# CityU-AIM-Group/HTD

Measured on AMD Instinct MI355X. Metric: images/sec (1333x800) HTD-R50 train step, higher is better.
Workload: dtype f32; 1 GPU; HTD ResNet-50 FPN fp32 train step fwd+bwd+SGD, batch 4/GPU @ 1333x800 (padded 1344x800), random-init weights, 2000 RPN proposals/img, 512 RoIs/img/stage; global_batch=4, parallelism=dp1, stage2_positives=158, proposals=random-init RPN (few positives: the regression branch is nearly idle)

## Files before the change

### htd_amd/csrc/conv_wgrad.hip

```cpp
#include <algorithm>

#include "common.h"

namespace {

using f32x16 = __attribute__((ext_vector_type(16))) float;

__device__ __forceinline__ float4 keep4(bool ok, float4 v)
{
    return make_float4(ok ? v.x : 0.f, ok ? v.y : 0.f, ok ? v.z : 0.f, ok ? v.w : 0.f);
}

struct WgradParams {
    const float *x, *gy;
    float *out;
    float *bias_out;
    int B, H, W, Ci, Co, kh, kw, stride, pad, dil, Ho, Wo;
    int64_t K;
    int Ntot;
    int mt, nt, splits;
    int64_t slices_per_split;
    const float *amax_x, *amax_g;
};

constexpr int BKW = 32;

enum : int {
    PIX_POINTWISE = 0,
    PIX_WIDE = 1,
    PIX_GENERAL = 2
};

template <int WGM, int WGN, int TM, int TN, int PIX, bool COVEC>
__global__ __launch_bounds__(256, 3) void conv_wgrad_kernel(WgradParams p)
{
    static_assert(WGM * WGN == 4, "4 waves per block");
    constexpr int BM = WGM * TM * 32, BN = WGN * TN * 32;
    constexpr int SA = BM + 4, SB = BN + 4;
    constexpr int VA = BM / 4, VB = BN / 4;
    constexpr int PA = (BKW * VA + 255) / 256, PB = (BKW * VB + 255) / 256;
    __shared__ __attribute__((aligned(16))) float lds[1][BKW * (SA + SB)];

    int tile, split;
    {
        const int tiles = p.mt * p.nt, L = blockIdx.x;
        if (p.splits % 8 == 0) {
            const int xcd = L % 8, idx = L / 8;
            tile = idx % tiles;
            split = (idx / tiles) * 8 + xcd;
        } else {
            tile = L % tiles;
            split = L / tiles;
        }
    }
    const int tile_m = tile % p.mt, tile_n = tile / p.mt;
    const int m0 = tile_m * BM, n0 = tile_n * BN;
    const int tid = threadIdx.x, lane = tid & 63, wave = tid >> 6;
    const int wm = wave / WGN, wn = wave % WGN;

    int a_col[PA], a_row[PA];
    bool a_cok[PA];
#pragma unroll
    for (int i = 0; i < PA; ++i) {
        const int v = tid + i * 256;
        a_row[i] = v / VA;
        a_col[i] = (v % VA) * 4;
        a_cok[i] = (v < BKW * VA) && (m0 + a_col[i] < p.Co);
    }
    int b_col[PB], b_row[PB], b_dy[PB], b_dx[PB], b_ci[PB];
    bool b_cok[PB];
#pragma unroll
    for (int i = 0; i < PB; ++i) {
        const int v = tid + i * 256;
        b_row[i] = v / VB;
        b_col[i] = (v % VB) * 4;
        const int n = n0 + b_col[i];
        b_cok[i] = (v < BKW * VB) && (n < p.Ntot);
        const int tap = b_cok[i] ? n / p.Ci : 0;
        b_ci[i] = b_cok[i] ? n - tap * p.Ci : 0;
        b_dy[i] = (tap / p.kw) * p.dil - p.pad;
        b_dx[i] = (tap % p.kw) * p.dil - p.pad;
    }

    const int64_t total_slices = (p.K + BKW - 1) / BKW;
    const int64_t s_begin = (int64_t)split * p.slices_per_split;
    const int64_t s_end = min(total_slices, s_begin + p.slices_per_split);

    unsigned a_k[PA];
#pragma unroll
    for (int i = 0; i < PA; ++i) a_k[i] = (unsigned)(s_begin * BKW) + a_row[i];
    unsigned b_k[PB];
    int b_b[PB], b_ho[PB], b_wo[PB];
    auto decode = [&](int i) {
        const unsigned kk = b_k[i] < (unsigned)p.K ? b_k[i] : 0u;
        b_wo[i] = (int)(kk % (unsigned)p.Wo);
        const unsigned t = kk / (unsigned)p.Wo;
        b_ho[i] = (int)(t % (unsigned)p.Ho);
        b_b[i] = (int)(t / (unsigned)p.Ho);
    };
#pragma unroll
    for (int i = 0; i < PB; ++i) {
        b_k[i] = (unsigned)(s_begin * BKW) + b_row[i];
        if constexpr (PIX != PIX_POINTWISE) decode(i);
    }

    float4 ra[PA], rb[PB];
    unsigned ra_ok = 0u, rb_ok = 0u;
    auto load_slice = [&]() {
#pragma unroll
        for (int i = 0; i < PA; ++i) {
            const bool ok = a_cok[i] && a_k[i] < (unsigned)p.K;
            const unsigned off = ok ? a_k[i] * (unsigned)p.Co + m0 + a_col[i] : 0u;
            if constexpr (COVEC) {
                ra[i] = *reinterpret_cast<const float4 *>(p.gy + off);
            } else {
                const int rem = ok ? p.Co - (m0 + a_col[i]) : 1;
                const float *g = p.gy + off;
                ra[i] = make_float4(g[0], g[rem > 1 ? 1 : 0], g[rem > 2 ? 2 : 0], g[rem > 3 ? 3 : 0]);
                ra[i].y = rem > 1 ? ra[i].y : 0.f;
                ra[i].z = rem > 2 ? ra[i].z : 0.f;
                ra[i].w = rem > 3 ? ra[i].w : 0.f;
            }
            ra_ok = ok ? (ra_ok | (1u << i)) : (ra_ok & ~(1u << i));
            a_k[i] += BKW;
        }
#pragma unroll
        for (int i = 0; i < PB; ++i) {
            bool ok = b_cok[i] && b_k[i] < (unsigned)p.K;
            unsigned off;
            if constexpr (PIX == PIX_POINTWISE) {
                off = b_k[i] * (unsigned)p.Ci + b_ci[i];
            } else {
                const int hi = b_ho[i] * p.stride + b_dy[i], wi = b_wo[i] * p.stride + b_dx[i];
                ok = ok && (unsigned)hi < (unsigned)p.H && (unsigned)wi < (unsigned)p.W;
                off = (((unsigned)b_b[i] * p.H + hi) * p.W + wi) * (unsigned)p.Ci + b_ci[i];
            }
            rb[i] = *reinterpret_cast<const float4 *>(p.x + (ok ? off : 0u));
            rb_ok = ok ? (rb_ok | (1u << i)) : (rb_ok & ~(1u << i));
            b_k[i] += BKW;
            if constexpr (PIX == PIX_WIDE) {
                const int wo = b_wo[i] + BKW;
                const bool c1 = wo >= p.Wo;
                b_wo[i] = c1 ? wo - p.Wo : wo;
                const int ho = b_ho[i] + (c1 ? 1 : 0);
                const bool c2 = ho == p.Ho;
                b_ho[i] = c2 ? 0 : ho;
                b_b[i] += c2 ? 1 : 0;
            } else if constexpr (PIX == PIX_GENERAL) {
                decode(i);
            }
        }
    };
    const bool do_bias = p.bias_out != nullptr && tile_n == 0;
    float4 bsum = make_float4(0.f, 0.f, 0.f, 0.f);
    auto store_slice = [&](int buf) {
        float *la = lds[buf], *lb = lds[buf] + BKW * SA;
#pragma unroll
        for (int i = 0; i < PA; ++i)
            if ((BKW * VA) % 256 == 0 || tid + i * 256 < BKW * VA) {
                const float4 v = keep4((ra_ok >> i) & 1u, ra[i]);
                *reinterpret_cast<float4 *>(la + a_row[i] * SA + a_col[i]) = v;
                if (do_bias) { bsum.x += v.x; bsum.y += v.y; bsum.z += v.z; bsum.w += v.w; }
            }
#pragma unroll
        for (int i = 0; i < PB; ++i)
            if ((BKW * VB) % 256 == 0 || tid + i * 256 < BKW * VB) *reinterpret_cast<float4 *>(lb + b_row[i] * SB + b_col[i]) = keep4((rb_ok >> i) & 1u, rb[i]);
    };

    f32x16 acc[TM][TN];
#pragma unroll
    for (int i = 0; i < TM; ++i)
#pragma unroll
        for (int j = 0; j < TN; ++j)
#pragma unroll
            for (int r = 0; r < 16; ++r) acc[i][j][r] = 0.f;
// ... 647 lines not shown
        if (v < 0) { x = Wv - 1; y = -1; }
    };
#pragma unroll
    for (int i = 0; i < 4; ++i) decode(s_begin * XH_KS + a_row0 + 8 * i, ax[i], ay[i], ab[i]);
#pragma unroll
    for (int i = 0; i < 3; ++i) decode(s_begin * XH_KS - 1 + b_row0 + 16 * i, bx[i], by[i], bb[i]);
    auto advance = [&](int &x, int &y, int &b) {
        if constexpr (WIDE) {
            x += XH_KS;
            const bool c1 = x >= Wv;
            x = c1 ? x - Wv : x;
            y += c1 ? 1 : 0;
            const bool c2 = y >= p.H;
            y = c2 ? y - p.H : y;
            b += c2 ? 1 : 0;
        } else {
            const int64_t v = ((int64_t)b * p.H + y) * Wv + x + XH_KS;
            x = (int)(v % Wv);
            const int64_t t = v / Wv;
            y = (int)(t % p.H);
            b = (int)(t / p.H);
        }
    };

    float4 ra[4], rb[3];
    unsigned ok_a = 0u, ok_b = 0u;
    auto load_slice = [&]() {
#pragma unroll
        for (int i = 0; i < 4; ++i) {
            const bool ok = a_cok && ab[i] < p.B && ax[i] < p.W;
            const unsigned off = (((unsigned)ab[i] * p.H + ay[i]) * (unsigned)p.W + ax[i]) * (unsigned)p.Co + m0 + a_col;
            ra[i] = *reinterpret_cast<const float4 *>(p.gy + (ok ? off : 0u));
            ok_a = ok ? (ok_a | (1u << i)) : (ok_a & ~(1u << i));
            advance(ax[i], ay[i], ab[i]);
        }
#pragma unroll
        for (int i = 0; i < 3; ++i) {
            const int yy = by[i] + dy;
            const bool ok = b_cok && (i < 2 || b_row0 < 2) && bb[i] < p.B && bx[i] < p.W && (unsigned)yy < (unsigned)p.H;
            const unsigned off = (((unsigned)bb[i] * p.H + yy) * (unsigned)p.W + bx[i]) * (unsigned)p.Ci + ci0 + b_col;
            rb[i] = *reinterpret_cast<const float4 *>(p.x + (ok ? off : 0u));
            ok_b = ok ? (ok_b | (1u << i)) : (ok_b & ~(1u << i));
            advance(bx[i], by[i], bb[i]);
        }
    };
    const bool do_bias = p.bias_out != nullptr && tile_nc == 0 && ky == 1;
    float4 bsum = make_float4(0.f, 0.f, 0.f, 0.f);
    auto put = [&](unsigned short *img, int plane, int rowpitch, int row, int col, float4 v) {
        unsigned h0, m0_, l0, h1, m1, l1;
        split3x2w(v.x, v.y, h0, m0_, l0);
        split3x2w(v.z, v.w, h1, m1, l1);
        unsigned short *d = img + row * rowpitch + col;
        *reinterpret_cast<uint2 *>(d) = make_uint2(h0, h1);
        *reinterpret_cast<uint2 *>(d + plane) = make_uint2(m0_, m1);
        *reinterpret_cast<uint2 *>(d + 2 * plane) = make_uint2(l0, l1);
    };
    auto store_slice = [&]() {
#pragma unroll
        for (int i = 0; i < 4; ++i) {
            const float4 v = keep4((ok_a >> i) & 1u, ra[i]);
            put(la, XH_PLANE_A, X3_ROW, a_row0 + 8 * i, a_col, v);
            if (do_bias) { bsum.x += v.x; bsum.y += v.y; bsum.z += v.z; bsum.w += v.w; }
        }
#pragma unroll
        for (int i = 0; i < 3; ++i)
            if (i < 2 || b_row0 < 2) put(lb, XH_PLANE_B, XH_ROWB, b_row0 + 16 * i, b_col, keep4((ok_b >> i) & 1u, rb[i]));
    };

    f32x16 acc[3][2];
#pragma unroll
    for (int t = 0; t < 3; ++t)
#pragma unroll
        for (int i = 0; i < 2; ++i)
#pragma unroll
            for (int r = 0; r < 16; ++r) acc[t][i][r] = 0.f;

    if (s_begin < s_end) {
        load_slice();
        store_slice();
    }
    __syncthreads();
    for (int64_t s = s_begin; s < s_end; ++s) {
        if (s + 1 < s_end) load_slice();
#pragma unroll
        for (int kk = 0; kk < XH_KS / 16; ++kk) {
            bf16x8w fa[2][3];
#pragma unroll
            for (int i = 0; i < 2; ++i)
#pragma unroll
                for (int q = 0; q < 3; ++q) fa[i][q] = tr_frag_row<X3_ROW>(la + q * XH_PLANE_A, kk * 16, wm * 64 + i * 32, lane);
#pragma unroll
            for (int t = 0; t < 3; ++t) {
                bf16x8w fb[3];
#pragma unroll
                for (int q = 0; q < 3; ++q) fb[q] = tr_frag_row<XH_ROWB>(lb + q * XH_PLANE_B, kk * 16 + t, wn * 32, lane);
#pragma unroll
                for (int i = 0; i < 2; ++i) {
                    acc[t][i] = __builtin_amdgcn_mfma_f32_32x32x16_bf16(fa[i][2], fb[0], acc[t][i], 0, 0, 0);
                    acc[t][i] = __builtin_amdgcn_mfma_f32_32x32x16_bf16(fa[i][0], fb[2], acc[t][i], 0, 0, 0);
                    acc[t][i] = __builtin_amdgcn_mfma_f32_32x32x16_bf16(fa[i][1], fb[1], acc[t][i], 0, 0, 0);
                    acc[t][i] = __builtin_amdgcn_mfma_f32_32x32x16_bf16(fa[i][1], fb[0], acc[t][i], 0, 0, 0);
                    acc[t][i] = __builtin_amdgcn_mfma_f32_32x32x16_bf16(fa[i][0], fb[1], acc[t][i], 0, 0, 0);
                    acc[t][i] = __builtin_amdgcn_mfma_f32_32x32x16_bf16(fa[i][0], fb[0], acc[t][i], 0, 0, 0);
                }
            }
        }
        if (s + 1 < s_end) {
            __syncthreads();
            store_slice();
        }
        __syncthreads();
    }

    if (do_bias) {
        float4 *red = reinterpret_cast<float4 *>(lds);
        red[tid] = bsum;
        __syncthreads();
        if (tid < 32) {
            float4 t = red[tid];
            for (int r = 1; r < 8; ++r) {
                const float4 v = red[r * 32 + tid];
                t.x += v.x; t.y += v.y; t.z += v.z; t.w += v.w;
            }
            float *dst = p.bias_out + (int64_t)split * p.Co;
            const int m = m0 + tid * 4;
            if (m < p.Co) dst[m] = t.x;
            if (m + 1 < p.Co) dst[m + 1] = t.y;
            if (m + 2 < p.Co) dst[m + 2] = t.z;
            if (m + 3 < p.Co) dst[m + 3] = t.w;
        }
    }
    float *out = p.out + (int64_t)split * p.Co * p.Ntot;
    const int fcol = lane & 31, fhalf = lane >> 5;
    const int ci = ci0 + wn * 32 + fcol;
    if (ci < p.Ci) {
#pragma unroll
        for (int t = 0; t < 3; ++t) {
            const int n = (ky * 3 + t) * p.Ci + ci;
#pragma unroll
            for (int i = 0; i < 2; ++i)
#pragma unroll
                for (int r = 0; r < 16; ++r) {
                    const int m = m0 + wm * 64 + i * 32 + (r & 3) + 8 * (r >> 2) + 4 * fhalf;
                    if (m < p.Co) out[(int64_t)m * p.Ntot + n] = acc[t][i][r];
                }
        }
    }
}

constexpr int XHD_KS = 16;
constexpr int XHD_RUN = XHD_KS + 2;
constexpr int XHD_PLANE_A = XHD_KS * X3_ROW, XHD_PLANE_B = XHD_RUN * XH_ROWB;
constexpr int XHD_BUF = 3 * XHD_PLANE_A + 3 * XHD_PLANE_B;
template <int TM, bool H2 = false>
__global__ __launch_bounds__(256, 2) void conv_wgrad_x3hd_kernel(WgradParams p)
{
    float sg = 1.f, sx = 1.f, sg_inv = 1.f, sx_inv = 1.f;
    if constexpr (H2) {
        const H2ScaleW a = h2w_scale(p.amax_g), b = h2w_scale(p.amax_x);
        sg = a.s; sg_inv = a.inv; sx = b.s; sx_inv = b.inv;
    }
    constexpr int BM = 2 * TM * 32, BNC = 64;
    constexpr int VA = BM / 4, RA = 256 / VA, PA = XHD_KS / RA;
    __shared__ __attribute__((aligned(16))) unsigned short lds[2 * XHD_BUF];
    const int ntc = (p.Ci + BNC - 1) / BNC;
    const int tiles = p.mt * ntc * 3;
    int tile, split;
    {
        const int L = blockIdx.x;
        if (p.splits % 8 == 0) {
            const int xcd = L % 8, idx = L / 8;
            tile = idx % tiles;
            split = (idx / tiles) * 8 + xcd;
        } else {
            tile = L % tiles;
            split = L / tiles;
        }
    }
    const int tile_m = tile % p.mt, rest = tile / p.mt;
    const int tile_nc = rest % ntc, ky = rest / ntc;
    const int m0 = tile_m * BM, ci0 = tile_nc * BNC, dy = ky - 1;
    const int tid = threadIdx.x, lane = tid & 63, wave = tid >> 6;
    const int wm = wave >> 1, wn = wave & 1;

    const int Wv = p.W + 1;
    const int64_t V = (int64_t)p.B * p.H * Wv;
    const int64_t v_begin = (int64_t)split * p.slices_per_split * XH_KS;
    const int64_t v_end = min((V + XH_KS - 1) / XH_KS * XH_KS, v_begin + p.slices_per_split * XH_KS);
    const int n_slices = v_begin < v_end ? (int)((v_end - v_begin) / XHD_KS) : 0;

    constexpr unsigned OOB = 0x80000000u;
    const int64_t px_end = min((int64_t)p.B * p.H * p.W, v_end - v_end / Wv);
    const __amdgpu_buffer_rsrc_t gy_desc = __builtin_amdgcn_make_buffer_rsrc(
        const_cast<float *>(p.gy), 0, (int)((unsigned)px_end * (unsigned)p.Co * 4u), 0x00020000);
    const __amdgpu_buffer_rsrc_t x_desc = __builtin_amdgcn_make_buffer_rsrc(
        const_cast<float *>(p.x), 0, (int)((unsigned)p.B * p.H * p.W * p.Ci * 4u), 0x00020000);

    const int a_col = (tid % VA) * 4, a_row0 = tid / VA;
    const int b_col = (tid & 15) * 4, b_row0 = tid >> 4;
    const bool a_cok = m0 + a_col < p.Co, b_cok = ci0 + b_col < p.Ci;
    const bool ragged = tid < 32;
    auto decode = [&](int64_t v, int &x, int &y, int64_t &real) {
        const int64_t vv = v < 0 ? 0 : v;
        x = (int)(vv % Wv);
        const int64_t t = vv / Wv;
        y = (int)(t % p.H);
        real = vv - t;
        if (v < 0) { x = Wv - 1; y = -1; real = 0; }
    };
    int ax[PA], bx[2], by[2];
    unsigned a_off[PA], b_off[2];
    const unsigned a_px = a_cok ? (unsigned)p.Co * 4u : 0u, b_px = b_cok ? (unsigned)p.Ci * 4u : 0u;
#pragma unroll
    for (int i = 0; i < PA; ++i) {
        int y;
        int64_t real;
        decode(v_begin + a_row0 + RA * i, ax[i], y, real);
        a_off[i] = a_cok ? (unsigned)(real * p.Co + m0 + a_col) * 4u : OOB;
    }
#pragma unroll
    for (int i = 0; i < 2; ++i) {
        int64_t real;
        decode(v_begin - 1 + b_row0 + 16 * i, bx[i], by[i], real);
        b_off[i] = b_cok && (i == 0 || ragged) ? (unsigned)((real + (int64_t)dy * p.W) * p.Ci + ci0 + b_col) * 4u : OOB;
    }
    const unsigned b_px1 = ragged ? b_px : 0u;
    const int adv_rows = XHD_KS / Wv, adv_x = XHD_KS - adv_rows * Wv;

    using u32x4w = __attribute__((ext_vector_type(4))) unsigned;
    auto load16 = [&](__amdgpu_buffer_rsrc_t d, unsigned off) {
        union { u32x4w u; float4 f; } c;
        c.u = __builtin_amdgcn_raw_buffer_load_b128(d, (int)off, 0, 0);
        return c.f;
    };
    float4 ra[2][PA], rb[2][2];
    auto load_slice = [&](float4 (&qa)[PA], float4 (&qb)[2]) {
#pragma unroll
        for (int i = 0; i < PA; ++i) {
            qa[i] = load16(gy_desc, ax[i] < p.W ? a_off[i] : OOB);
            ax[i] += adv_x;
            const bool c1 = ax[i] >= Wv;
            ax[i] -= c1 ? Wv : 0;
            a_off[i] += XHD_KS * a_px - (unsigned)(adv_rows + (c1 ? 1 : 0)) * a_px;
        }
#pragma unroll
        for (int i = 0; i < 2; ++i) {
            const unsigned px = i == 0 ? b_px : b_px1;
            qb[i] = load16(x_desc, bx[i] < p.W && (unsigned)(by[i] + dy) < (unsigned)p.H ? b_off[i] : OOB);
            bx[i] += adv_x;
            const bool c1 = bx[i] >= Wv;
            bx[i] -= c1 ? Wv : 0;
            const int rows = adv_rows + (c1 ? 1 : 0);
            by[i] += rows;
            by[i] -= by[i] >= p.H ? p.H : 0;
            b_off[i] += XHD_KS * px - (unsigned)rows * px;
        }
    };
    const bool do_bias = p.bias_out != nullptr && tile_nc == 0 && ky == 1;
    float4 bsum = make_float4(0.f, 0.f, 0.f, 0.f);
    auto put = [&](unsigned short *d, int plane, float4 v, float sc) {
        if constexpr (H2) {
            unsigned h0, l0, h1, l1;
            split2w(v.x * sc, v.y * sc, h0, l0);
            split2w(v.z * sc, v.w * sc, h1, l1);
            *reinterpret_cast<uint2 *>(d) = make_uint2(h0, h1);
            *reinterpret_cast<uint2 *>(d + plane) = make_uint2(l0, l1);
        } else {
            unsigned h0, m0_, l0, h1, m1, l1;
            split3x2w(v.x, v.y, h0, m0_, l0);
            split3x2w(v.z, v.w, h1, m1, l1);
            *reinterpret_cast<uint2 *>(d) = make_uint2(h0, h1);
            *reinterpret_cast<uint2 *>(d + plane) = make_uint2(m0_, m1);
            *reinterpret_cast<uint2 *>(d + 2 * plane) = make_uint2(l0, l1);
        }
    };
    const int a_lds0 = a_row0 * X3_ROW + a_col, a_lds1 = (a_row0 + RA) * X3_ROW + a_col;
    const int b_lds0 = 3 * XHD_PLANE_A + b_row0 * XH_ROWB + b_col, b_lds1 = 3 * XHD_PLANE_A + (16 + b_row0) * XH_ROWB + b_col;

    f32x16 acc[3][TM];
#pragma unroll
    for (int t = 0; t < 3; ++t)
#pragma unroll
        for (int i = 0; i < TM; ++i)
#pragma unroll
            for (int r = 0; r < 16; ++r) acc[t][i][r] = 0.f;

    auto half = [&](const unsigned short *rd, unsigned short *wr, float4 (&qa)[PA], float4 (&qb)[2]) {
        constexpr int NPL = H2 ? 2 : 3;
        bf16x8w fa[TM][3], fb[3][3];
#pragma unroll
        for (int i = 0; i < TM; ++i)
#pragma unroll
            for (int q = 0; q < NPL; ++q) fa[i][q] = tr_frag_row<X3_ROW>(rd + q * XHD_PLANE_A, 0, wm * TM * 32 + i * 32, lane);
#pragma unroll
        for (int t = 0; t < 3; ++t)
#pragma unroll
            for (int q = 0; q < NPL; ++q) fb[t][q] = tr_frag_row<XH_ROWB>(rd + 3 * XHD_PLANE_A + q * XHD_PLANE_B, t, wn * 32, lane);
        __builtin_amdgcn_sched_barrier(0);
        constexpr int QA[6] = {H2 ? 1 : 2, 0, H2 ? 0 : 1, 1, 0, 0}, QB[6] = {0, H2 ? 1 : 2, H2 ? 0 : 1, 0, 1, 0};
        unsigned h[2], m[2], l[2];
        constexpr int NC = 2 * (PA + 1), NM = (H2 ? 9 : 18) * TM;
#pragma unroll
        for (int c = 0; c < NC; ++c) {
            const int u = c >> 1;
            const float4 v = u < PA ? qa[u < PA ? u : 0] : qb[0];
            const float sc = u < PA ? sg : sx;
            if ((c & 1) == 0) {
                if constexpr (H2) split2w(v.x * sc, v.y * sc, h[0], l[0]);
                else split3x2w(v.x, v.y, h[0], m[0], l[0]);
            } else {
                if constexpr (H2) split2w(v.z * sc, v.w * sc, h[1], l[1]);
                else split3x2w(v.z, v.w, h[1], m[1], l[1]);
                unsigned short *d = wr + (u >= PA ? b_lds0 : u == 0 ? a_lds0 : a_lds1);
                const int plane = u < PA ? XHD_PLANE_A : XHD_PLANE_B;
                *reinterpret_cast<uint2 *>(d) = make_uint2(h[0], h[1]);
                if constexpr (H2) {
                    *reinterpret_cast<uint2 *>(d + plane) = make_uint2(l[0], l[1]);
                } else {
                    *reinterpret_cast<uint2 *>(d + plane) = make_uint2(m[0], m[1]);
                    *reinterpret_cast<uint2 *>(d + 2 * plane) = make_uint2(l[0], l[1]);
                }
                if (u < PA) { bsum.x += v.x; bsum.y += v.y; bsum.z += v.z; bsum.w += v.w; }
            }
#pragma unroll
            for (int e = c * NM / NC; e < (c + 1) * NM / NC; ++e) {
                const int q = e / (3 * TM), t = (e % (3 * TM)) / TM, i = e % TM;
                acc[t][i] = mfma_x3w<H2>(fa[i][QA[q]], fb[t][QB[q]], acc[t][i]);
            }
            __builtin_amdgcn_sched_barrier(0);
        }
        if (__builtin_amdgcn_readfirstlane(wave) == 0) {
            if (ragged) put(wr + b_lds1, XHD_PLANE_B, qb[1], sx);
        }
        load_slice(qa, qb);
        __syncthreads();
    };
    auto store_slice = [&](unsigned short *wr, const float4 (&qa)[PA], const float4 (&qb)[2]) {
        put(wr + a_lds0, XHD_PLANE_A, qa[0], sg);
        if constexpr (PA > 1) put(wr + a_lds1, XHD_PLANE_A, qa[PA - 1], sg);
#pragma unroll
        for (int i = 0; i < PA; ++i) { bsum.x += qa[i].x; bsum.y += qa[i].y; bsum.z += qa[i].z; bsum.w += qa[i].w; }
        put(wr + b_lds0, XHD_PLANE_B, qb[0], sx);
        if (ragged) put(wr + b_lds1, XHD_PLANE_B, qb[1], sx);
    };

    unsigned short *buf0 = lds, *buf1 = lds + XHD_BUF;
    load_slice(ra[0], rb[0]);
    load_slice(ra[1], rb[1]);
    store_slice(buf0, ra[0], rb[0]);
    load_slice(ra[0], rb[0]);
    __syncthreads();
    for (int s = 0; s < n_slices; s += 2) {
        half(buf0, buf1, ra[1], rb[1]);
        half(buf1, buf0, ra[0], rb[0]);
    }

    if (do_bias) {
        float4 *red = reinterpret_cast<float4 *>(lds);
        __syncthreads();
        red[tid] = bsum;
        __syncthreads();
        if (tid < VA) {
            float4 t = red[tid];
            for (int r = 1; r < RA; ++r) {
                const float4 v = red[r * VA + tid];
                t.x += v.x; t.y += v.y; t.z += v.z; t.w += v.w;
            }
            float *dst = p.bias_out + (int64_t)split * p.Co;
            const int m = m0 + tid * 4;
            if (m < p.Co) dst[m] = t.x;
            if (m + 1 < p.Co) dst[m + 1] = t.y;
            if (m + 2 < p.Co) dst[m + 2] = t.z;
            if (m + 3 < p.Co) dst[m + 3] = t.w;
        }
    }
    float *out = p.out + (int64_t)split * p.Co * p.Ntot;
    const int fcol = lane & 31, fhalf = lane >> 5;
    const int ci = ci0 + wn * 32 + fcol;
    if (ci < p.Ci) {
#pragma unroll
        for (int t = 0; t < 3; ++t) {
            const int n = (ky * 3 + t) * p.Ci + ci;
#pragma unroll
            for (int i = 0; i < TM; ++i)
#pragma unroll
                for (int r = 0; r < 16; ++r) {
                    const int m = m0 + wm * TM * 32 + i * 32 + (r & 3) + 8 * (r >> 2) + 4 * fhalf;
                    if (m < p.Co) out[(int64_t)m * p.Ntot + n] = H2 ? acc[t][i][r] * sg_inv * sx_inv : acc[t][i][r];
                }
        }
    }
}

__global__ __launch_bounds__(256) void splitk_reduce_kernel(const float *__restrict__ ws, float *__restrict__ out,
                                                            int64_t n, int splits, const float *__restrict__ ws2 = nullptr,
                                                            float *__restrict__ out2 = nullptr, int n2 = 0, int acc = 0)
{
    const int extra = out2 ? (n2 + 255) / 256 : 0;
    if ((int)blockIdx.x >= (int)gridDim.x - extra) {
        const int i = ((int)blockIdx.x - ((int)gridDim.x - extra)) * 256 + threadIdx.x;
        if (i < n2) {
            float s = acc ? out2[i] : 0.f;
            int k = 0;
            for (; k + 3 < splits; k += 4) {
                const float a = ws2[(int64_t)k * n2 + i], b = ws2[(int64_t)(k + 1) * n2 + i];
                const float c = ws2[(int64_t)(k + 2) * n2 + i], d = ws2[(int64_t)(k + 3) * n2 + i];
                s += a; s += b; s += c; s += d;
            }
            for (; k < splits; ++k) s += ws2[(int64_t)k * n2 + i];
            out2[i] = s;
        }
        return;
    }
    const unsigned main_blocks = gridDim.x - extra;
    const int64_t n4 = (n & 3) == 0 ? (n >> 2) : 0;
    for (int64_t i = (int64_t)blockIdx.x * blockDim.x + threadIdx.x; i < n4; i += (int64_t)main_blocks * blockDim.x) {
        float4 s = acc ? *reinterpret_cast<const float4 *>(out + i * 4) : make_float4(0.f, 0.f, 0.f, 0.f);
        int k = 0;
        for (; k + 3 < splits; k += 4) {
            float4 v[4];
#pragma unroll
            for (int u = 0; u < 4; ++u) v[u] = *reinterpret_cast<const float4 *>(ws + (int64_t)(k + u) * n + i * 4);
#pragma unroll
            for (int u = 0; u < 4; ++u) { s.x += v[u].x; s.y += v[u].y; s.z += v[u].z; s.w += v[u].w; }
        }
        for (; k < splits; ++k) {
            const float4 v = *reinterpret_cast<const float4 *>(ws + (int64_t)k * n + i * 4);
            s.x += v.x; s.y += v.y; s.z += v.z; s.w += v.w;
        }
        *reinterpret_cast<float4 *>(out + i * 4) = s;
    }
    if (blockIdx.x == 0)
        for (int64_t i = n4 * 4 + threadIdx.x; i < n; i += blockDim.x) {
            float s = acc ? out[i] : 0.f;
            for (int k = 0; k < splits; ++k) s += ws[(int64_t)k * n + i];
            out[i] = s;
        }
}

__global__ __launch_bounds__(256) void reduce_rows_kernel(const float *__restrict__ ws, float *__restrict__ out, int n,
                                                          int rows)
{
    __shared__ float red[16][17];
    const int col = threadIdx.x & 15, grp = threadIdx.x >> 4;
    const int c = blockIdx.x * 16 + col;
    float s = 0.f;
    if (c < n)
        for (int k = grp; k < rows; k += 16) s += ws[(int64_t)k * n + c];
    red[grp][col] = s;
    __syncthreads();
    if (grp == 0 && c < n) {
        float t = red[0][col];
#pragma unroll
        for (int g = 1; g < 16; ++g) t += red[g][col];
        out[c] = t;
    }
}

using htd::mag_bits;
using htd::wave_mag_out;

__global__ __launch_bounds__(256) void colsum_mask_kernel(const float *__restrict__ g, const float *__restrict__ y,
                                                          float *__restrict__ gm, float *__restrict__ partial,
                                                          int64_t rows, int C, int64_t rows_per_block, float *__restrict__ amax_out)
{
    const int c = blockIdx.y * 256 + threadIdx.x;
    const int64_t r0 = (int64_t)blockIdx.x * rows_per_block, r1 = min(rows, r0 + rows_per_block);
    float s = 0.f;
    unsigned mx = 0u;
    if (c < C)
        for (int64_t r = r0; r < r1; ++r) {
            float v = g[r * C + c];
            if (y) {
                v = y[r * C + c] > 0.f ? v : 0.f;
                gm[r * C + c] = v;
            }
            mx = max(mx, mag_bits(v));
            s += v;
        }
    if (amax_out) wave_mag_out(mx, amax_out);
    if (partial && c < C) partial[(int64_t)blockIdx.x * C + c] = s;
}

__global__ __launch_bounds__(256) void colsum_mask_vec_kernel(const float *__restrict__ g, const float *__restrict__ y,
                                                              float *__restrict__ gm, float *__restrict__ partial,
                                                              int64_t rows, int C, int64_t rows_per_block,
                                                              float *__restrict__ amax_out)
{
    __shared__ float4 red[256];
    unsigned mx = 0u;
    const int C4 = C >> 2;
    const int cbase = blockIdx.y * 256;
    const int cw = min(256, C4 - cbase);
    const int R = 256 / cw;
    const int c4 = threadIdx.x % cw, rsub = threadIdx.x / cw;
    const int64_t r0 = (int64_t)blockIdx.x * rows_per_block, r1 = min(rows, r0 + rows_per_block);
    float4 s = make_float4(0.f, 0.f, 0.f, 0.f);
    if (rsub < R) {
        int64_t r = r0 + rsub;
        for (; r + 3 * (int64_t)R < r1; r += 4 * (int64_t)R) {
            float4 v[4], yv[4];
#pragma unroll
            for (int u = 0; u < 4; ++u) {
                const int64_t o = (r + u * (int64_t)R) * C + (int64_t)(cbase + c4) * 4;
                v[u] = *reinterpret_cast<const float4 *>(g + o);
                if (y) yv[u] = *reinterpret_cast<const float4 *>(y + o);
            }
#pragma unroll
            for (int u = 0; u < 4; ++u) {
                if (y) {
                    const int64_t o = (r + u * (int64_t)R) * C + (int64_t)(cbase + c4) * 4;
                    v[u].x = yv[u].x > 0.f ? v[u].x : 0.f; v[u].y = yv[u].y > 0.f ? v[u].y : 0.f;
                    v[u].z = yv[u].z > 0.f ? v[u].z : 0.f; v[u].w = yv[u].w > 0.f ? v[u].w : 0.f;
                    *reinterpret_cast<float4 *>(gm + o) = v[u];
                }
                mx = htd::mag_bits4(mx, v[u]);
                s.x += v[u].x; s.y += v[u].y; s.z += v[u].z; s.w += v[u].w;
            }
        }
        for (; r < r1; r += R) {
            const int64_t o = r * C + (int64_t)(cbase + c4) * 4;
            float4 v = *reinterpret_cast<const float4 *>(g + o);
            if (y) {
                const float4 yv = *reinterpret_cast<const float4 *>(y + o);
                v.x = yv.x > 0.f ? v.x : 0.f; v.y = yv.y > 0.f ? v.y : 0.f;
                v.z = yv.z > 0.f ? v.z : 0.f; v.w = yv.w > 0.f ? v.w : 0.f;
                *reinterpret_cast<float4 *>(gm + o) = v;
            }
            mx = htd::mag_bits4(mx, v);
            s.x += v.x; s.y += v.y; s.z += v.z; s.w += v.w;
        }
    }
    if (amax_out) wave_mag_out(mx, amax_out);
    if (!partial) return;
    red[threadIdx.x] = s;
    __syncthreads();
    if (rsub == 0) {
        for (int k = 1; k < R; ++k) {
            const float4 t = red[k * cw + c4];
            s.x += t.x; s.y += t.y; s.z += t.z; s.w += t.w;
        }
        *reinterpret_cast<float4 *>(partial + (int64_t)blockIdx.x * C + (int64_t)(cbase + c4) * 4) = s;
    }
}

struct Cfg { int splits; int mt, nt; int bm, bn; };

template <int WGM, int WGN, int TM, int TN>
void launch_wgrad(int pix, bool covec, dim3 grid, hipStream_t s, const WgradParams &p)
{
#define HTD_WGRAD_CASE(PIX, CV)                                                                                   \
    if (pix == PIX && covec == CV) {                                                                               \
        hipLaunchKernelGGL((conv_wgrad_kernel<WGM, WGN, TM, TN, PIX, CV>), grid, dim3(256), 0, s, p);             \
        return;                                                                                                    \
    }
    HTD_WGRAD_CASE(PIX_POINTWISE, true) HTD_WGRAD_CASE(PIX_WIDE, true) HTD_WGRAD_CASE(PIX_GENERAL, true)
    HTD_WGRAD_CASE(PIX_POINTWISE, false) HTD_WGRAD_CASE(PIX_WIDE, false) HTD_WGRAD_CASE(PIX_GENERAL, false)
#undef HTD_WGRAD_CASE
}

Cfg choose(int Co, int Ntot, int64_t K)
{
    Cfg c;
    c.bm = Co <= 32 ? 32 : 128;
    c.bn = 128;
    c.mt = (int)htd::ceil_div(Co, c.bm);
    c.nt = (int)htd::ceil_div(Ntot, c.bn);
    const int64_t slices = htd::ceil_div(K, BKW);
    static const int units = getenv("HTD_WGRAD_UNITS") ? atoi(getenv("HTD_WGRAD_UNITS")) : 1536;
    int64_t want = htd::ceil_div(units, (int64_t)c.mt * c.nt);
    const int64_t tiles = (int64_t)c.mt * c.nt;
    int64_t cap = std::max<int64_t>(1, slices / 20);
    if (tiles * cap < 256)
        cap = std::max(cap, std::min<int64_t>(htd::ceil_div(256, tiles), std::max<int64_t>(1, slices / 5)));
    want = std::min<int64_t>(want, cap);
    c.splits = (int)std::max<int64_t>(1, std::min<int64_t>(want, 192));
    if (c.splits >= 6) c.splits = (c.splits + 7) / 8 * 8;
    static const int forced = getenv("HTD_WGRAD_SPLITS") ? atoi(getenv("HTD_WGRAD_SPLITS")) : 0;
    if (forced > 0) c.splits = (int)std::min<int64_t>(forced, slices);
    return c;
}

static const bool g_wgrad_x3h_off = getenv("HTD_WGRAD_X3H") != nullptr && atoi(getenv("HTD_WGRAD_X3H")) == 0;
bool x3h_takes(int Ci, int Co, int kh, int kw, int stride, int pad, int dil)
{
    return !g_wgrad_x3h_off && kh == 3 && kw == 3 && stride == 1 && pad == 1 && dil == 1 && Co >= 64 && (Co & 3) == 0 &&
           Ci >= 32 && (Ci & 3) == 0;
}
int x3h_splits(int B, int H, int W, int Ci, int Co)
{
    const int64_t tiles = htd::ceil_div(Co, 128) * htd::ceil_div(Ci, 64) * 3;
    const int64_t slices = htd::ceil_div((int64_t)B * H * (W + 1), XH_KS);
    static const int target = getenv("HTD_WGRAD_X3H_UNITS") ? atoi(getenv("HTD_WGRAD_X3H_UNITS")) : 768;
    int64_t want = htd::ceil_div(target, tiles);
    int64_t cap = std::max<int64_t>(1, slices / 8);
    if (tiles * cap < 256) cap = std::max(cap, std::min<int64_t>(htd::ceil_div(256, tiles), std::max<int64_t>(1, slices / 4)));
    want = std::min<int64_t>(want, cap);
    int splits = (int)std::max<int64_t>(1, std::min<int64_t>(want, 128));
    if (splits >= 6) splits = (splits + 7) / 8 * 8;
    static const int forced = getenv("HTD_WGRAD_X3H_SPLITS") ? atoi(getenv("HTD_WGRAD_X3H_SPLITS")) : 0;
    if (forced > 0) splits = (int)std::min<int64_t>(forced, std::max<int64_t>(1, slices / 2));
    return splits;
}

}

int g_wgrad_math = -1;

extern "C" int64_t htd_conv2d_wgrad_workspace_bytes(int B, int H, int W, int Ci, int Co, int kh, int kw, int stride,
                                                    int pad, int dil)
{
    const int Ho = (H + 2 * pad - (dil * (kh - 1) + 1)) / stride + 1;
    const int Wo = (W + 2 * pad - (dil * (kw - 1) + 1)) / stride + 1;
    const Cfg c = choose(Co, kh * kw * Ci, (int64_t)B * Ho * Wo);
    int splits = c.splits;
    if (x3h_takes(Ci, Co, kh, kw, stride, pad, dil)) splits = std::max(splits, x3h_splits(B, H, W, Ci, Co));
    return (int64_t)splits * Co * (kh * kw * Ci + 1) * 4 + 256;
}

static int bwd_weight_impl(const float *x, const float *gy, float *gw, float *gbias, int B, int H, int W, int Ci, int Co, int kh,
                           int kw, int stride, int pad, int dil, void *workspace, void *stream, int accumulate,
                           const float *amax_x = nullptr, const float *amax_g = nullptr)
{
    HTD_REQUIRE(B > 0 && H > 0 && W > 0 && Ci > 0 && Co > 0 && kh > 0 && kw > 0 && stride > 0 && dil > 0 && pad >= 0,
                "conv2d_bwd_weight: bad sizes");
    HTD_REQUIRE(Ci % 4 == 0, "conv2d_bwd_weight: Ci=%d must be a multiple of 4", Ci);
    HTD_REQUIRE(x && gy && gw && workspace, "conv2d_bwd_weight: null pointer");
    WgradParams p{};
    p.x = x; p.gy = gy;
    p.amax_x = amax_x; p.amax_g = amax_g;
    const bool h2 = amax_x != nullptr && amax_g != nullptr;
    p.B = B; p.H = H; p.W = W; p.Ci = Ci; p.Co = Co; p.kh = kh; p.kw = kw; p.stride = stride; p.pad = pad; p.dil = dil;
    p.Ho = (H + 2 * pad - (dil * (kh - 1) + 1)) / stride + 1;
    p.Wo = (W + 2 * pad - (dil * (kw - 1) + 1)) / stride + 1;
    HTD_REQUIRE(p.Ho > 0 && p.Wo > 0, "conv2d_bwd_weight: empty output");
    p.K = (int64_t)B * p.Ho * p.Wo;
    HTD_REQUIRE((int64_t)B * H * W * Ci < (1ll << 31) && p.K * Co < (1ll << 31),
                "conv2d_bwd_weight: operand larger than 2^31 elements (32-bit element offsets)");
    p.Ntot = kh * kw * Ci;
    static const int math_env0 = getenv("HTD_CONV_MATH") ? atoi(getenv("HTD_CONV_MATH")) : 1;
    if ((g_wgrad_math < 0 ? math_env0 : g_wgrad_math) == 1 && x3h_takes(Ci, Co, kh, kw, stride, pad, dil)) {
        p.mt = (int)htd::ceil_div(Co, 128);
        p.nt = (int)htd::ceil_div(Ci, 64);
        p.splits = x3h_splits(B, H, W, Ci, Co);
        const int64_t slices = htd::ceil_div((int64_t)B * H * (W + 1), XH_KS);
        p.slices_per_split = htd::ceil_div(slices, p.splits);
        p.splits = (int)htd::ceil_div(slices, p.slices_per_split);
        const bool direct = p.splits == 1 && !accumulate;
        p.out = direct ? gw : (float *)workspace;
        float *bias_part = (float *)workspace + (int64_t)p.splits * Co * p.Ntot;
        p.bias_out = !gbias ? nullptr : (direct ? gbias : bias_part);
        hipStream_t s = (hipStream_t)stream;
        const dim3 grid((unsigned)(p.mt * p.nt * 3 * p.splits));
        static const bool x3hd_on = !(getenv("HTD_WGRAD_X3D") && atoi(getenv("HTD_WGRAD_X3D")) == 0);
        if (x3hd_on && XHD_KS / (W + 1) + 1 <= H && (int64_t)B * H * W * Ci * 4 < (1ll << 31) &&
            (int64_t)B * H * W * Co * 4 < (1ll << 31))
        {
            static const bool tile64 = !(getenv("HTD_WGRAD_TILE64") && atoi(getenv("HTD_WGRAD_TILE64")) == 0);
            if (tile64 && Co <= 64) {
                p.mt = (int)htd::ceil_div(Co, 64);
                const dim3 g64((unsigned)(p.mt * p.nt * 3 * p.splits));
                if (h2) hipLaunchKernelGGL((conv_wgrad_x3hd_kernel<1, true>), g64, dim3(256), 0, s, p);
                else hipLaunchKernelGGL((conv_wgrad_x3hd_kernel<1, false>), g64, dim3(256), 0, s, p);
            } else if (h2) {
                hipLaunchKernelGGL((conv_wgrad_x3hd_kernel<2, true>), grid, dim3(256), 0, s, p);
            } else {
                hipLaunchKernelGGL((conv_wgrad_x3hd_kernel<2, false>), grid, dim3(256), 0, s, p);
            }
        }
        else {
            HTD_REQUIRE(!h2, "conv2d_bwd_weight_h2: this 3x3 layer is not taken by the H2 kernels (htd_conv2d_bwd_weight_h2_supported)");
            if (W + 1 >= XH_KS) hipLaunchKernelGGL(conv_wgrad_x3h_kernel<true>, grid, dim3(256), 0, s, p);
            else hipLaunchKernelGGL(conv_wgrad_x3h_kernel<false>, grid, dim3(256), 0, s, p);
        }
        if (!direct) {
            const int64_t n = (int64_t)Co * p.Ntot;
            const unsigned blocks = (unsigned)std::min<int64_t>(htd::ceil_div(n, 256), 2048);
            const unsigned extra = gbias ? (unsigned)htd::ceil_div(Co, 256) : 0u;
            hipLaunchKernelGGL(splitk_reduce_kernel, dim3(blocks + extra), dim3(256), 0, s, (const float *)workspace, gw, n,
                               p.splits, (const float *)(gbias ? bias_part : nullptr), gbias, Co, accumulate);
        }
        return htd::check_launch("conv2d_bwd_weight");
    }
    const Cfg c = choose(Co, p.Ntot, p.K);
    p.mt = c.mt; p.nt = c.nt; p.splits = c.splits;
    p.slices_per_split = htd::ceil_div(htd::ceil_div(p.K, BKW), c.splits);
    const bool direct = c.splits == 1 && !accumulate;
    p.out = direct ? gw : (float *)workspace;
    float *bias_partial = (float *)workspace + (int64_t)c.splits * Co * p.Ntot;
    p.bias_out = !gbias ? nullptr : (direct ? gbias : bias_partial);
    hipStream_t s = (hipStream_t)stream;
    p.slices_per_split = htd::ceil_div(htd::ceil_div(p.K, BKW), c.splits);
    dim3 grid((unsigned)(c.mt * c.nt * c.splits));
    const int pix = (kh == 1 && kw == 1 && stride == 1 && pad == 0) ? PIX_POINTWISE : (p.Wo >= BKW ? PIX_WIDE : PIX_GENERAL);
    const bool covec = (Co & 3) == 0;
    static const int math_env = getenv("HTD_CONV_MATH") ? atoi(getenv("HTD_CONV_MATH")) : 1;
    const bool x3 = (g_wgrad_math < 0 ? math_env : g_wgrad_math) == 1 && c.bm == 128 && covec && (Ci & 3) == 0;
    if (x3) {
        static const bool x3d_on = !(getenv("HTD_WGRAD_X3D") && atoi(getenv("HTD_WGRAD_X3D")) == 0);
        const bool x3d = x3d_on && (int64_t)B * H * W * Ci * 4 < (1ll << 31) && p.K * Co * 4 < (1ll << 31);
        if (x3d) {
            static const bool tile64 = !(getenv("HTD_WGRAD_TILE64") && atoi(getenv("HTD_WGRAD_TILE64")) == 0);
            const bool m64 = tile64 && Co <= 64 && pix != PIX_GENERAL, n64 = tile64 && !m64 && p.Ntot <= 64 && pix == PIX_POINTWISE;
            p.mt = (int)htd::ceil_div(Co, m64 ? 64 : 128);
            p.nt = (int)htd::ceil_div(p.Ntot, n64 ? 64 : 128);
            const dim3 gd = c.splits % 8 == 0 ? dim3((unsigned)(p.mt * p.nt * c.splits))
                                              : dim3((unsigned)(8 * htd::ceil_div(p.nt * c.splits, 8) * p.mt));
            if (h2) {
                if (m64 && pix == PIX_POINTWISE) hipLaunchKernelGGL((conv_wgrad_x3d_kernel<PIX_POINTWISE, 1, 2, true>), gd, dim3(256), 0, s, p);
                else if (m64) hipLaunchKernelGGL((conv_wgrad_x3d_kernel<PIX_WIDE, 1, 2, true>), gd, dim3(256), 0, s, p);
                else if (n64) hipLaunchKernelGGL((conv_wgrad_x3d_kernel<PIX_POINTWISE, 2, 1, true>), gd, dim3(256), 0, s, p);
                else if (pix == PIX_POINTWISE) hipLaunchKernelGGL((conv_wgrad_x3d_kernel<PIX_POINTWISE, 2, 2, true>), gd, dim3(256), 0, s, p);
                else if (pix == PIX_WIDE) hipLaunchKernelGGL((conv_wgrad_x3d_kernel<PIX_WIDE, 2, 2, true>), gd, dim3(256), 0, s, p);
                else hipLaunchKernelGGL((conv_wgrad_x3d_kernel<PIX_GENERAL, 2, 2, true>), gd, dim3(256), 0, s, p);
            }
            else if (m64 && pix == PIX_POINTWISE) hipLaunchKernelGGL((conv_wgrad_x3d_kernel<PIX_POINTWISE, 1, 2>), gd, dim3(256), 0, s, p);
            else if (m64) hipLaunchKernelGGL((conv_wgrad_x3d_kernel<PIX_WIDE, 1, 2>), gd, dim3(256), 0, s, p);
            else if (n64) hipLaunchKernelGGL((conv_wgrad_x3d_kernel<PIX_POINTWISE, 2, 1>), gd, dim3(256), 0, s, p);
            else if (pix == PIX_POINTWISE) hipLaunchKernelGGL((conv_wgrad_x3d_kernel<PIX_POINTWISE, 2, 2>), gd, dim3(256), 0, s, p);
            else if (pix == PIX_WIDE) hipLaunchKernelGGL((conv_wgrad_x3d_kernel<PIX_WIDE, 2, 2>), gd, dim3(256), 0, s, p);
            else hipLaunchKernelGGL((conv_wgrad_x3d_kernel<PIX_GENERAL, 2, 2>), gd, dim3(256), 0, s, p);
        } else if (h2) {
            HTD_REQUIRE(false, "conv2d_bwd_weight_h2: operands too large for the H2 kernels (htd_conv2d_bwd_weight_h2_supported)");
        } else if (pix == PIX_POINTWISE) hipLaunchKernelGGL(conv_wgrad_x3_kernel<PIX_POINTWISE>, grid, dim3(256), 0, s, p);
        else if (pix == PIX_WIDE) hipLaunchKernelGGL(conv_wgrad_x3_kernel<PIX_WIDE>, grid, dim3(256), 0, s, p);
        else hipLaunchKernelGGL(conv_wgrad_x3_kernel<PIX_GENERAL>, grid, dim3(256), 0, s, p);
    } else if (h2) {
        HTD_REQUIRE(false, "conv2d_bwd_weight_h2: layer not taken by the H2 kernels (htd_conv2d_bwd_weight_h2_supported)");
    } else if (c.bm == 32)
        launch_wgrad<1, 4, 1, 1>(pix, covec, grid, s, p);
    else
        launch_wgrad<2, 2, 2, 2>(pix, covec, grid, s, p);
    if (!direct) {
        const int64_t n = (int64_t)Co * p.Ntot;
        const unsigned blocks = (unsigned)std::min<int64_t>(htd::ceil_div(n, 256), 2048);
        const unsigned extra = gbias ? (unsigned)htd::ceil_div(Co, 256) : 0u;
        hipLaunchKernelGGL(splitk_reduce_kernel, dim3(blocks + extra), dim3(256), 0, s, (const float *)workspace, gw, n,
                           c.splits, (const float *)(gbias ? bias_partial : nullptr), gbias, Co, accumulate);
    }
    return htd::check_launch("conv2d_bwd_weight");
}

extern "C" int htd_conv2d_bwd_weight(const float *x, const float *gy, float *gw, float *gbias, int B, int H, int W,
                                     int Ci, int Co, int kh, int kw, int stride, int pad, int dil, void *workspace,
                                     void *stream)
{
    return bwd_weight_impl(x, gy, gw, gbias, B, H, W, Ci, Co, kh, kw, stride, pad, dil, workspace, stream, 0);
}

extern "C" int htd_conv2d_bwd_weight_acc(const float *x, const float *gy, float *gw, float *gbias, int B, int H, int W,
                                         int Ci, int Co, int kh, int kw, int stride, int pad, int dil, void *workspace,
                                         void *stream)
{
    return bwd_weight_impl(x, gy, gw, gbias, B, H, W, Ci, Co, kh, kw, stride, pad, dil, workspace, stream, 1);
}

extern "C" int htd_conv2d_bwd_weight_h2_supported(int B, int H, int W, int Ci, int Co, int kh, int kw, int stride, int pad, int dil)
{
    static const int math_env = getenv("HTD_CONV_MATH") ? atoi(getenv("HTD_CONV_MATH")) : 1;
    if (htd_conv2d_set_h2(-1) != 1 || (g_wgrad_math < 0 ? math_env : g_wgrad_math) != 1) return 0;
    if (B <= 0 || H <= 0 || W <= 0 || Ci <= 0 || Co <= 0 || (Ci & 3) != 0 || stride <= 0 || dil <= 0 || pad < 0) return 0;
    const int Ho = (H + 2 * pad - (dil * (kh - 1) + 1)) / stride + 1, Wo = (W + 2 * pad - (dil * (kw - 1) + 1)) / stride + 1;
    if (Ho <= 0 || Wo <= 0) return 0;
    const int64_t K = (int64_t)B * Ho * Wo;
    static const bool d_on = !(getenv("HTD_WGRAD_X3D") && atoi(getenv("HTD_WGRAD_X3D")) == 0);
    if (!d_on || (int64_t)B * H * W * Ci * 4 >= (1ll << 31) || K * Co * 4 >= (1ll << 31)) return 0;
    if (x3h_takes(Ci, Co, kh, kw, stride, pad, dil)) return XHD_KS / (W + 1) + 1 <= H ? 1 : 0;
    const Cfg c = choose(Co, kh * kw * Ci, K);
    return (c.bm == 128 && (Co & 3) == 0) ? 1 : 0;
}

extern "C" int htd_conv2d_bwd_weight_h2(const float *x, const float *gy, const float *amax_x, const float *amax_g, float *gw,
                                        float *gbias, int B, int H, int W, int Ci, int Co, int kh, int kw, int stride, int pad,
                                        int dil, int accumulate, void *workspace, void *stream)
{
    HTD_REQUIRE(amax_x && amax_g, "conv2d_bwd_weight_h2: null maximum");
    HTD_REQUIRE(htd_conv2d_bwd_weight_h2_supported(B, H, W, Ci, Co, kh, kw, stride, pad, dil) == 1,
                "conv2d_bwd_weight_h2: layer not taken by the H2 kernels");
    return bwd_weight_impl(x, gy, gw, gbias, B, H, W, Ci, Co, kh, kw, stride, pad, dil, workspace, stream, accumulate ? 1 : 0, amax_x,
                           amax_g);
}

static int bias_grad_relu_mask_impl(const float *g, const float *y, float *gm, float *gbias, int64_t rows, int C, void *workspace,
                                    float *amax_out, void *stream)
{
    HTD_REQUIRE(rows >= 0 && C > 0, "bias_grad: bad sizes");
    HTD_REQUIRE(g && (gbias || y) && (!gbias || workspace) && (!y || gm), "bias_grad: null pointer");
    hipStream_t s = (hipStream_t)stream;
    const int nb = (int)std::max<int64_t>(1, std::min<int64_t>(1024, htd::ceil_div(rows, 8)));
    const int64_t rpb = htd::ceil_div(std::max<int64_t>(rows, 1), nb);
    float *partial = gbias ? (float *)workspace : nullptr;
    if ((C & 3) == 0 && (((uintptr_t)g | (uintptr_t)y | (uintptr_t)gm | (uintptr_t)partial) & 15) == 0)
        hipLaunchKernelGGL(colsum_mask_vec_kernel, dim3(nb, (unsigned)htd::ceil_div(C / 4, 256)), dim3(256), 0, s, g, y,
                           gm, partial, rows, C, rpb, amax_out);
    else
        hipLaunchKernelGGL(colsum_mask_kernel, dim3(nb, (unsigned)htd::ceil_div(C, 256)), dim3(256), 0, s, g, y, gm,
                           partial, rows, C, rpb, amax_out);
    if (gbias)
        hipLaunchKernelGGL(reduce_rows_kernel, dim3((unsigned)htd::ceil_div(C, 16)), dim3(256), 0, s,
                           (const float *)partial, gbias, C, nb);
    return htd::check_launch("bias_grad");
}

extern "C" int htd_bias_grad_relu_mask(const float *g, const float *y, float *gm, float *gbias, int64_t rows, int C,
                                       void *workspace, void *stream)
{
    return bias_grad_relu_mask_impl(g, y, gm, gbias, rows, C, workspace, nullptr, stream);
}

extern "C" int htd_bias_grad_relu_mask_amax(const float *g, const float *y, float *gm, float *gbias, int64_t rows, int C,
                                            void *workspace, float *amax_out, void *stream)
{
    HTD_REQUIRE(amax_out, "bias_grad: null maximum");
    return bias_grad_relu_mask_impl(g, y, gm, gbias, rows, C, workspace, amax_out, stream);
}
```

### htd_amd/csrc/conv_x3.hip

```cpp
#include <algorithm>
#include <mutex>
#include <type_traits>
#include <unordered_map>

#include <stdlib.h>

#include "common.h"

namespace {

using f32x16 = __attribute__((ext_vector_type(16))) float;
using bf16x8 = __attribute__((ext_vector_type(8))) __bf16;
using bf16x2 = __attribute__((ext_vector_type(2))) __bf16;
using f32x2 = __attribute__((ext_vector_type(2))) float;
using f32x4 = __attribute__((ext_vector_type(4))) float;

using f16x8 = __attribute__((ext_vector_type(8))) _Float16;
using f16x2 = __attribute__((ext_vector_type(2))) _Float16;

constexpr int XK = 16;
constexpr int NCH = 6;

struct H2Scale { float s, inv; };
__device__ __forceinline__ H2Scale h2_scale(const float *amax)
{
    const unsigned E = (__float_as_uint(*amax) >> 23) & 0xffu;
    int e = E == 0u ? 126 : (E == 255u ? 0 : 141 - (int)E);
    e = e > 126 ? 126 : e;
    return H2Scale{__uint_as_float((unsigned)(127 + e) << 23), __uint_as_float((unsigned)(127 - e) << 23)};
}
__device__ __forceinline__ void split2hx2(float a, float b, unsigned &h, unsigned &l)
{
    union { f16x2 v; unsigned u; } c;
    c.v = __builtin_convertvector(f32x2{a, b}, f16x2);
    h = c.u;
    const f32x2 back = __builtin_convertvector(c.v, f32x2);
    c.v = __builtin_convertvector(f32x2{a - back[0], b - back[1]}, f16x2);
    l = c.u;
}

__device__ __forceinline__ void split3x2(float a, float b, unsigned &h, unsigned &m, unsigned &l)
{
    union { bf16x2 v; unsigned u; } c;
    c.v = __builtin_convertvector(f32x2{a, b}, bf16x2);
    h = c.u;
    const float ra = a - __uint_as_float(h << 16), rb = b - __uint_as_float(h & 0xffff0000u);
    c.v = __builtin_convertvector(f32x2{ra, rb}, bf16x2);
    m = c.u;
    c.v = __builtin_convertvector(f32x2{ra - __uint_as_float(m << 16), rb - __uint_as_float(m & 0xffff0000u)}, bf16x2);
    l = c.u;
}

#ifndef HTD_X3P_EARLY
#define HTD_X3P_EARLY 1
#endif
#ifndef HTD_X3H_NB
#define HTD_X3H_NB 2
#endif
#ifndef HTD_X3H_FRAG_FIRST
#define HTD_X3H_FRAG_FIRST 1
#endif
#ifndef HTD_X3H_OCC4
#define HTD_X3H_OCC4 0
#endif

template <int N>
__device__ __forceinline__ void wait_vm()
{
    asm volatile("s_waitcnt vmcnt(%0)" ::"n"(N) : "memory");
}
__device__ __forceinline__ void landed(f32x4 &a) { asm volatile("" : "+v"(a)::"memory"); }

__device__ __forceinline__ void lds_dma16(const void *src, unsigned lds_dst)
{
    unsigned keep;
    asm volatile("s_mov_b32 %0, m0\n\ts_mov_b32 m0, %2\n\ts_nop 0\n\tglobal_load_lds_dwordx4 %1, off\n\ts_mov_b32 m0, %0"
                 : "=&s"(keep)
                 : "v"(src), "s"(lds_dst)
                 : "memory");
}

using u32x2 = __attribute__((ext_vector_type(2))) unsigned;
template <int OFF>
__device__ __forceinline__ void lds_store8(unsigned addr, unsigned lo, unsigned hi)
{
    const u32x2 v = {lo, hi};
    asm volatile("ds_write_b64 %0, %1 offset:%2" ::"v"(addr), "v"(v), "n"(OFF) : "memory");
}

struct X3Params {
    const float *x;
    const uint4 *wp;
    const float *bias, *residual, *mask_src;
    float *y;
    int Hx, Wx;
    int Ho, Wo;
    int Ci, Co, Cop;
    int kh;
    int stride;
    int ntl;
    int tl_dy[9], tl_dx[9], tl_w[9];
    int o_step, o_h0, o_w0, oH, oW;
    int relu;
    int res_H, res_W;
    float res_sh, res_sw;
    int64_t M;
    int mt, nt;
    int ncs;
    int tiles_a, splits_a, sps_a, splits_b, sps_b;
    int64_t m_rem0;
    float *partial;
    const uint4 *xp;
    uint4 *yp;
    int64_t xp_rows, yp_rows;
    const float *amax, *wscale;
    float *amax_out;
};

__device__ __forceinline__ void block_absmax_out(float mx, float *out, float *red, unsigned seen)
{
    unsigned bits = (mx != mx) ? 0x7fc00000u : __float_as_uint(mx);
    for (int o = 32; o > 0; o >>= 1) bits = max(bits, (unsigned)__shfl_xor((int)bits, o));
    __syncthreads();
    if ((threadIdx.x & 63) == 0) reinterpret_cast<unsigned *>(red)[threadIdx.x >> 6] = bits;
    __syncthreads();
    if (threadIdx.x == 0) {
        const unsigned *r = reinterpret_cast<const unsigned *>(red);
        bits = max(max(r[0], r[1]), max(r[2], r[3]));
        if (bits > seen) __hip_atomic_fetch_max(reinterpret_cast<unsigned *>(out), bits, __ATOMIC_RELAXED, __HIP_MEMORY_SCOPE_AGENT);
    }
}
__device__ __forceinline__ void wave_absmax_out(float mx, float *out, unsigned seen)
{
    unsigned bits = (mx != mx) ? 0x7fc00000u : __float_as_uint(mx);
    for (int o = 32; o > 0; o >>= 1) bits = max(bits, (unsigned)__shfl_xor((int)bits, o));
    if ((threadIdx.x & 63) == 0 && bits > seen)
        __hip_atomic_fetch_max(reinterpret_cast<unsigned *>(out), bits, __ATOMIC_RELAXED, __HIP_MEMORY_SCOPE_AGENT);
}
__device__ __forceinline__ float absmax4(float mx, float4 v)
{
    const float m = fmaxf(fmaxf(fabsf(v.x), fabsf(v.y)), fmaxf(fabsf(v.z), fabsf(v.w)));
    const bool nan = (v.x != v.x) | (v.y != v.y) | (v.z != v.z) | (v.w != v.w);
    return nan ? __uint_as_float(0x7fc00000u) : ((mx != mx) ? mx : fmaxf(mx, m));
}

__device__ __forceinline__ void emit_planes4(uint4 *yp, int64_t rows, int64_t m, int n, float4 v)
{
    unsigned h0, m0, l0, h1, m1, l1;
    split3x2(v.x, v.y, h0, m0, l0);
    split3x2(v.z, v.w, h1, m1, l1);
    char *d = reinterpret_cast<char *>(yp + ((int64_t)(n >> 4) * NCH + ((n >> 3) & 1)) * rows + m) + ((n >> 2) & 1) * 8;
    *reinterpret_cast<uint2 *>(d) = make_uint2(h0, h1);
    *reinterpret_cast<uint2 *>(d + 2 * rows * 16) = make_uint2(m0, m1);
    *reinterpret_cast<uint2 *>(d + 4 * rows * 16) = make_uint2(l0, l1);
}

template <int BM, int KW>
struct Geo {
    static constexpr int RUN = BM + KW - 1;
    static constexpr int PITCH = ((RUN + 1 + 3) / 8) * 8 + 4;
    static constexpr int PASSES = (RUN + 63) / 64;
};

__device__ __forceinline__ int64_t x3_out_off(const X3Params &p, int64_t m, int n)
{
    if (p.o_step == 0) return m * p.Co + n;
    const unsigned mm = (unsigned)m, wo = mm % (unsigned)p.Wo, t = mm / (unsigned)p.Wo;
    const unsigned ho = t % (unsigned)p.Ho, b = t / (unsigned)p.Ho;
    return (((int64_t)b * p.oH + p.o_h0 + p.o_step * (int)ho) * p.oW + p.o_w0 + p.o_step * (int)wo) * p.Co + n;
}

template <int WGM, int WGN, int TM, int TN, bool MF16, typename Acc>
__device__ __forceinline__ void x3_epilogue(const X3Params &p, Acc &acc, uint4 *lds, int64_t m0, int n0, bool part, bool region_b,
                                            int split)
{
    constexpr int BN = WGN * TN * 32;
    constexpr int EPI_STRIDE = BN + 4, EPI_ROWS = WGM * 32;
    constexpr int RBLK = MF16 ? 16 : 32;
    constexpr int CB = TN * 32 / RBLK;
    const int tid = threadIdx.x, lane = tid & 63, wave = tid >> 6;
    const int wm = wave / WGN, wn = wave % WGN;
    const int frow = lane & 31, fhalf = lane >> 5;
    const int lrow = MF16 ? (lane & 15) : frow;
    const int kg = lane >> 4;
    float *le = reinterpret_cast<float *>(lds);
    const bool vec_ok = (p.Co & 3) == 0;
    constexpr int V = BN / 4, RPP = 256 / V;
    float omax = 0.f;
    const unsigned oseen = (p.amax_out != nullptr && !part) ? *reinterpret_cast<const volatile unsigned *>(p.amax_out) : 0u;
    const bool scaled = p.wscale != nullptr;
    float4 cscale = make_float4(1.f, 1.f, 1.f, 1.f);
    if (scaled) {
        const float ia = h2_scale(p.amax).inv;
        const float4 w4 = *reinterpret_cast<const float4 *>(p.wscale + n0 + (tid % V) * 4);
        cscale = make_float4(w4.x * ia, w4.y * ia, w4.z * ia, w4.w * ia);
    }
#pragma unroll
    for (int i = 0; i < TM; ++i) {
        if constexpr (MF16) {
#pragma unroll
            for (int ib = 0; ib < 2; ++ib)
#pragma unroll
                for (int j = 0; j < CB; ++j)
#pragma unroll
                    for (int r = 0; r < 4; ++r)
                        le[(wm * 32 + ib * 16 + 4 * kg + r) * EPI_STRIDE + wn * TN * 32 + j * 16 + lrow] = acc[2 * i + ib][j][r];
        } else {
#pragma unroll
            for (int j = 0; j < TN; ++j)
#pragma unroll
                for (int r = 0; r < 16; ++r) {
                    const int row = wm * 32 + (r & 3) + 8 * (r >> 2) + 4 * fhalf;
                    le[row * EPI_STRIDE + (wn * TN + j) * 32 + frow] = acc[i][j][r];
                }
        }
        __syncthreads();
        const int c4 = tid % V;
        const int n = n0 + c4 * 4;
        constexpr int NPASS = EPI_ROWS / RPP;
        if (vec_ok && !part && p.res_H == 0) {
            const bool col_ok = n < p.Co;
            float4 bv = make_float4(0.f, 0.f, 0.f, 0.f);
            if (p.bias != nullptr && col_ok) bv = *reinterpret_cast<const float4 *>(p.bias + n);
            constexpr int UB = NPASS < 4 ? NPASS : 4;
#pragma unroll
            for (int pass0 = 0; pass0 < NPASS; pass0 += UB) {
                float4 v[UB], rv[UB], mv[UB];
                int64_t o[UB];
                bool ok[UB];
#pragma unroll
                for (int u = 0; u < UB; ++u) {
                    const int row = tid / V + (pass0 + u) * RPP;
                    const int64_t m = m0 + ((row >> 5) * TM + i) * 32 + (row & 31);
                    ok[u] = m < p.M && col_ok;
                    o[u] = x3_out_off(p, ok[u] ? m : 0, n) & -(int64_t)ok[u];
                    v[u] = *reinterpret_cast<const float4 *>(le + row * EPI_STRIDE + c4 * 4);
                    if (scaled) { v[u].x *= cscale.x; v[u].y *= cscale.y; v[u].z *= cscale.z; v[u].w *= cscale.w; }
                }
                if (p.residual != nullptr) {
#pragma unroll
                    for (int u = 0; u < UB; ++u) rv[u] = *reinterpret_cast<const float4 *>(p.residual + o[u]);
                }
                if (p.mask_src != nullptr) {
#pragma unroll
                    for (int u = 0; u < UB; ++u) mv[u] = *reinterpret_cast<const float4 *>(p.mask_src + o[u]);
                }
#pragma unroll
                for (int u = 0; u < UB; ++u) { v[u].x += bv.x; v[u].y += bv.y; v[u].z += bv.z; v[u].w += bv.w; }
                if (p.residual != nullptr) {
#pragma unroll
                    for (int u = 0; u < UB; ++u) { v[u].x += rv[u].x; v[u].y += rv[u].y; v[u].z += rv[u].z; v[u].w += rv[u].w; }
                }
                if (p.relu) {
#pragma unroll
                    for (int u = 0; u < UB; ++u) {
                        v[u].x = fmaxf(v[u].x, 0.f); v[u].y = fmaxf(v[u].y, 0.f); v[u].z = fmaxf(v[u].z, 0.f); v[u].w = fmaxf(v[u].w, 0.f);
                    }
                }
                if (p.mask_src != nullptr) {
#pragma unroll
                    for (int u = 0; u < UB; ++u) {
                        v[u].x = mv[u].x > 0.f ? v[u].x : 0.f; v[u].y = mv[u].y > 0.f ? v[u].y : 0.f;
                        v[u].z = mv[u].z > 0.f ? v[u].z : 0.f; v[u].w = mv[u].w > 0.f ? v[u].w : 0.f;
                    }
                }
#pragma unroll
                for (int u = 0; u < UB; ++u)
                    if (ok[u]) {
                        *reinterpret_cast<float4 *>(p.y + o[u]) = v[u];
                        omax = absmax4(omax, v[u]);
                    }
                if (p.yp != nullptr) {
#pragma unroll
                    for (int u = 0; u < UB; ++u) {
                        const int row = tid / V + (pass0 + u) * RPP;
                        if (ok[u]) emit_planes4(p.yp, p.yp_rows, m0 + ((row >> 5) * TM + i) * 32 + (row & 31), n, v[u]);
                    }
                }
            }
            if (i + 1 < TM) __syncthreads();
            continue;
        }
#pragma unroll
        for (int pass = 0; pass < NPASS; ++pass) {
            const int row = tid / V + pass * RPP;
            const int64_t m = m0 + ((row >> 5) * TM + i) * 32 + (row & 31);
            if (m >= p.M || n >= p.Co) continue;
            float4 v = *reinterpret_cast<const float4 *>(le + row * EPI_STRIDE + c4 * 4);
            if (scaled) { v.x *= cscale.x; v.y *= cscale.y; v.z *= cscale.z; v.w *= cscale.w; }
            const int64_t o = x3_out_off(p, m, n);
            if (part) {
                float *dst = region_b ? p.partial + (p.splits_a > 1 ? (int64_t)p.splits_a * p.m_rem0 * p.Co : 0) +
                                            ((int64_t)split * (p.M - p.m_rem0) + (m - p.m_rem0)) * p.Co + n
                                      : p.partial + ((int64_t)split * p.m_rem0 + m) * p.Co + n;
                if (vec_ok) *reinterpret_cast<float4 *>(dst) = v;
                else {
                    dst[0] = v.x;
                    if (n + 1 < p.Co) dst[1] = v.y;
                    if (n + 2 < p.Co) dst[2] = v.z;
                    if (n + 3 < p.Co) dst[3] = v.w;
                }
                continue;
            }
            if (vec_ok) {
                if (p.bias) {
                    const float4 bv = *reinterpret_cast<const float4 *>(p.bias + n);
                    v.x += bv.x; v.y += bv.y; v.z += bv.z; v.w += bv.w;
                }
                if (p.residual) {
                    int64_t ro = o;
                    if (p.res_H > 0) {
                        const unsigned mm = (unsigned)m, wo = mm % (unsigned)p.Wo, t = mm / (unsigned)p.Wo;
                        const unsigned ho = t % (unsigned)p.Ho, b = t / (unsigned)p.Ho;
                        const int rh = min((int)floorf(ho * p.res_sh), p.res_H - 1);
                        const int rw = min((int)floorf(wo * p.res_sw), p.res_W - 1);
                        ro = (((int64_t)b * p.res_H + rh) * p.res_W + rw) * p.Co + n;
                    }
                    const float4 rv = *reinterpret_cast<const float4 *>(p.residual + ro);
                    v.x += rv.x; v.y += rv.y; v.z += rv.z; v.w += rv.w;
                }
                if (p.relu) { v.x = fmaxf(v.x, 0.f); v.y = fmaxf(v.y, 0.f); v.z = fmaxf(v.z, 0.f); v.w = fmaxf(v.w, 0.f); }
                if (p.mask_src) {
                    const float4 mv = *reinterpret_cast<const float4 *>(p.mask_src + o);
                    v.x = mv.x > 0.f ? v.x : 0.f; v.y = mv.y > 0.f ? v.y : 0.f;
                    v.z = mv.z > 0.f ? v.z : 0.f; v.w = mv.w > 0.f ? v.w : 0.f;
                }
                *reinterpret_cast<float4 *>(p.y + o) = v;
                omax = absmax4(omax, v);
                if (p.yp != nullptr) emit_planes4(p.yp, p.yp_rows, m, n, v);
            } else {
                auto put = [&](int e, float t) {
                    if (n + e >= p.Co) return;
                    t += p.bias ? p.bias[n + e] : 0.f;
                    if (p.residual) t += p.residual[o + e];
                    if (p.relu) t = fmaxf(t, 0.f);
                    if (p.mask_src) t = p.mask_src[o + e] > 0.f ? t : 0.f;
                    p.y[o + e] = t;
                    omax = absmax4(omax, make_float4(t, 0.f, 0.f, 0.f));
                };
                put(0, v.x); put(1, v.y); put(2, v.z); put(3, v.w);
            }
        }
        if (i + 1 < TM) __syncthreads();
    }
    if (p.amax_out != nullptr && !part) block_absmax_out(omax, p.amax_out, le, oseen);
}

template <int WGM, int WGN, int TM, int TN, int KW, int NB, bool H2 = false>
constexpr int x3p_occupancy()
{
    constexpr int BM = WGM * TM * 32, BN = WGN * TN * 32;
    constexpr int NCHL = H2 ? 4 : NCH;
    constexpr int main_bytes = (2 * NCHL * Geo<BM, KW>::PITCH + NB * NCHL * BN) * 16;
    constexpr int epi_bytes = WGM * 32 * (BN + 4) * 4;
    constexpr int by_lds = 163840 / (main_bytes > epi_bytes ? main_bytes : epi_bytes);
    constexpr int by_regs = TM * TN >= 4 ? (H2 && HTD_X3H_OCC4 ? 4 : 3) : 4;
    return by_lds < by_regs ? by_lds : by_regs;
}

template <int WGM, int WGN, int TM, int TN, int KW, bool MF16, int NB, bool H2 = false>
__global__ __launch_bounds__(256, (x3p_occupancy<WGM, WGN, TM, TN, KW, NB, H2>())) void conv_x3p_kernel(X3Params p)
{
    static_assert(!(H2 && MF16), "H2: 32x32x16 form only");
    constexpr int NCHL = H2 ? 4 : NCH;
    constexpr int BM = WGM * TM * 32, BN = WGN * TN * 32;
    using G = Geo<BM, KW>;
    constexpr int PADX = (KW - 1) / 2;
    constexpr int A_VEC = NCHL * G::PITCH;
    constexpr int B_VEC = NCHL * BN;
    constexpr int MAIN_VEC = 2 * A_VEC + NB * B_VEC;
    constexpr int EPI_STRIDE = BN + 4, EPI_ROWS = WGM * 32;
    constexpr int EPI_VEC = EPI_ROWS * EPI_STRIDE / 4;
    constexpr int LDS_VEC = MAIN_VEC > EPI_VEC ? MAIN_VEC : EPI_VEC;
    __shared__ uint4 lds[LDS_VEC];
    uint4 *const lA = lds, *const lB = lds + 2 * A_VEC;
    const unsigned lds_a0 = (unsigned)(size_t)(__attribute__((address_space(3))) void *)lA;

    int bid = blockIdx.x, split = 0, sps = 0;
    bool part = false;
    const bool region_b = bid >= p.tiles_a * p.splits_a;
    if (region_b) {
        const int r = bid - p.tiles_a * p.splits_a;
        bid = p.tiles_a + r / p.splits_b;
        split = r % p.splits_b;
        part = p.splits_b > 1;
        sps = p.sps_b;
    } else if (p.splits_a > 1) {
        split = bid % p.splits_a;
        bid = bid / p.splits_a;
        part = true;
        sps = p.sps_a;
    } else {
        const int q = p.tiles_a / 8, r = p.tiles_a % 8, xcd = bid % 8, idx = bid / 8;
        bid = (xcd < r ? xcd * (q + 1) : r * (q + 1) + (xcd - r) * q) + idx;
    }
    const int tile_m = bid / p.nt, tile_n = bid % p.nt;
    const int64_t m0 = (int64_t)tile_m * BM;
    const int n0 = tile_n * BN;

    const int tid = threadIdx.x, lane = tid & 63, wave = tid >> 6;
    const int wm = wave / WGN, wn = wave % WGN;
    const int frow = lane & 31, fhalf = lane >> 5;
    const int PADY = (p.kh - 1) / 2;

    const int vcol = tid & 3, vrow = tid >> 2;
    const int a_g0 = (int)m0 + vrow - PADX;
    unsigned a_off[KW > 1 ? 1 : G::PASSES];
    bool a_in[KW > 1 ? 1 : G::PASSES];
    unsigned a_tm[KW > 1 ? 1 : G::PASSES];
    if constexpr (KW > 1) {
        a_off[0] = (unsigned)a_g0 * (unsigned)p.Ci + vcol * 4;
        a_in[0] = true;
        a_tm[0] = 0u;
    } else {
#pragma unroll
        for (int i = 0; i < G::PASSES; ++i) {
            const int64_t m = m0 + vrow + 64 * i;
            a_in[i] = vrow + 64 * i < G::RUN && m < p.M;
            const unsigned mm = a_in[i] ? (unsigned)m : 0u;
            const unsigned wo = mm % (unsigned)p.Wo, t = mm / (unsigned)p.Wo;
            const unsigned ho = t % (unsigned)p.Ho, b = t / (unsigned)p.Ho;
            a_off[i] = ((b * (unsigned)p.Hx + ho * (unsigned)p.stride) * (unsigned)p.Wx + wo * (unsigned)p.stride) *
                           (unsigned)p.Ci + vcol * 4;
            unsigned tm = 0x1ffu;
            if (p.ntl > 0) {
                tm = 0u;
                const int hb = (int)(ho * (unsigned)p.stride), wb = (int)(wo * (unsigned)p.stride);
                for (int q = 0; q < p.ntl; ++q)
                    tm |= ((unsigned)(hb + p.tl_dy[q]) < (unsigned)p.Hx && (unsigned)(wb + p.tl_dx[q]) < (unsigned)p.Wx) ? (1u << q) : 0u;
            }
            a_tm[i] = tm;
        }
    }

    constexpr int RBLK = MF16 ? 16 : 32;
    constexpr int RB = TM * 32 / RBLK, CB = TN * 32 / RBLK;
    const int lrow = MF16 ? (lane & 15) : frow;
    const int kg = lane >> 4;
    unsigned vmask[RB];
    const int a_frag0 = (wm * TM * 32 + lrow) * 16;
#pragma unroll
    for (int i = 0; i < RB; ++i) {
        const int r = wm * TM * 32 + i * RBLK + lrow;
        vmask[i] = 0xffffffffu;
        if constexpr (KW > 1) {
            const int64_t m = m0 + r;
            const unsigned mm = m < p.M ? (unsigned)m : 0u;
            const int xx = (int)(mm % (unsigned)p.Wx), yy = (int)((mm / (unsigned)p.Wx) % (unsigned)p.Hx);
            unsigned v = 0u;
            for (int ky = 0; ky < p.kh; ++ky)
#pragma unroll
                for (int kx = 0; kx < KW; ++kx) {
                    const bool ok = m < p.M && (unsigned)(yy + ky - PADY) < (unsigned)p.Hx &&
                                    (unsigned)(xx + kx - PADX) < (unsigned)p.Wx;
                    v |= ok ? (1u << (ky * KW + kx)) : 0u;
                }
            vmask[i] = v;
        }
    }
    const int zero_frag = G::RUN * 16;
    const int a_c0 = MF16 ? kg * G::PITCH * 16 : fhalf * G::PITCH * 16;
    const int a_c1 = MF16 ? ((kg >> 1) * 4 + (kg & 1)) * G::PITCH * 16 : 0;
    const int b_row = (wn * TN * 32 + lrow) * 16;
    const int b_c0 = (MF16 ? kg * BN * 16 : fhalf * BN * 16) + b_row;
    const int b_c1 = MF16 ? ((1 - (kg >> 1)) * 2 + (kg & 1)) * BN * 16 + b_row : 0;
    const int b_c2 = MF16 ? (((kg >> 1) ? 0 : 4) + (kg & 1)) * BN * 16 + b_row : 0;

    const int total_steps = p.ncs * p.kh;
    const int s_begin = part ? split * sps : 0;
    const int s_end = part ? min(total_steps, s_begin + sps) : total_steps;

    if (tid < 2 * NCHL) lA[(tid / NCHL) * A_VEC + (tid % NCHL) * G::PITCH + G::RUN] = make_uint4(0u, 0u, 0u, 0u);

    constexpr int NP = G::PASSES;
    constexpr int NPT = KW > 1 ? 1 : NP;
    constexpr bool EARLY = HTD_X3P_EARLY && TM * TN >= 4;
    static_assert(KW == 1 || NP <= KW, "one pass per tap");
    f32x4 ra[2 * NPT];
#pragma unroll
    for (int i = 0; i < 2 * NPT; ++i) ra[i] = f32x4{0.f, 0.f, 0.f, 0.f};
    unsigned ra_ok = 0u;
    float h2s = 1.f;
    if constexpr (H2) h2s = h2_scale(p.amax).s;
    auto load_pass = [&](int shift, int koff, int i, int slot, bool live) __attribute__((always_inline)) {
        bool ok;
        unsigned off;
        if constexpr (KW > 1) {
            const int g = a_g0 + 64 * i + shift;
            ok = live && vrow + 64 * i < G::RUN && g >= 0 && (int64_t)g < p.M;
            off = a_off[0] + (unsigned)(64 * i) * (unsigned)p.Ci + (unsigned)koff;
            ra_ok = ok ? (ra_ok | (1u << i)) : (ra_ok & ~(1u << i));
        } else {
            ok = live && a_in[i] && ((a_tm[i] >> shift) & 1u);
            off = a_off[i] + (unsigned)koff;
            ra_ok = ok ? (ra_ok | (1u << slot)) : (ra_ok & ~(1u << slot));
        }
        asm volatile("global_load_dwordx4 %0, %1, off" : "+v"(ra[slot]) : "v"(p.x + (off & (0u - (unsigned)ok))) : "memory");
    };
    auto store_pass = [&](int buf, int i, int slot) __attribute__((always_inline)) {
        int j = vrow + 64 * i;
        if constexpr (EARLY) {
            static_assert(G::PITCH >= G::RUN + 2, "a spare row behind the zero row");
            j = (G::RUN % 64 == 0 || j < G::RUN) ? j : G::RUN + 1;
        } else {
            if (G::RUN % 64 != 0 && j >= G::RUN) return;
        }
        bool ok;
        if constexpr (KW > 1) ok = (ra_ok >> i) & 1u;
        else ok = (ra_ok >> slot) & 1u;
        const float4 v = make_float4(ok ? ra[slot][0] : 0.f, ok ? ra[slot][1] : 0.f, ok ? ra[slot][2] : 0.f, ok ? ra[slot][3] : 0.f);
        const unsigned d = lds_a0 + (unsigned)(buf * A_VEC * 16 + ((vcol >> 1) * G::PITCH + j) * 16 + (vcol & 1) * 8);
        if constexpr (H2) {
            unsigned h0, l0, h1, l1;
            split2hx2(v.x * h2s, v.y * h2s, h0, l0);
            split2hx2(v.z * h2s, v.w * h2s, h1, l1);
            lds_store8<0>(d, h0, h1);
            lds_store8<2 * G::PITCH * 16>(d, l0, l1);
        } else {
            unsigned h0, m0_, l0, h1, m1, l1;
            split3x2(v.x, v.y, h0, m0_, l0);
            split3x2(v.z, v.w, h1, m1, l1);
            lds_store8<0>(d, h0, h1);
            lds_store8<2 * G::PITCH * 16>(d, m0_, m1);
            lds_store8<4 * G::PITCH * 16>(d, l0, l1);
        }
    };
    constexpr int NI = (H2 ? 4 : NCH) * BN / 64;
    const uint4 *bsrc[(NI + 3) / 4];
#pragma unroll
    for (int k = 0; k < (NI + 3) / 4; ++k) {
        const int idx = (wave + 4 * k) % NI;
        bsrc[k] = p.wp + (int64_t)(idx / (BN / 64)) * p.Cop + (idx % (BN / 64)) * 64 + n0 + lane;
    }
    const unsigned lds_b0 = (unsigned)(size_t)(__attribute__((address_space(3))) void *)lB;
    const int wave_u = __builtin_amdgcn_readfirstlane(wave);
    auto load_b = [&](unsigned tile_off, int buf) {
#pragma unroll
        for (int k = 0; k < (NI + 3) / 4; ++k) {
            const int idx = wave_u + 4 * k;
            if (NI % 4 != 0 && idx >= NI) continue;
            lds_dma16(bsrc[k] + tile_off, lds_b0 + (unsigned)((buf * B_VEC + idx * 64) * 16));
        }
    };

    auto lds_barrier = [&]() {
        asm volatile("s_waitcnt lgkmcnt(0)" ::: "memory");
        __builtin_amdgcn_s_barrier();
        asm volatile("" ::: "memory");
    };
    constexpr int DIST = NB - 1;
    constexpr int NI_MIN = NI / 4;
    static_assert(NI_MIN >= 1, "every wave issues at least one LDS-DMA per B tile");
    auto wait_tap = [&](bool b_issued) __attribute__((always_inline)) {
        if (DIST >= 2 && b_issued) wait_vm<NPT + NI_MIN>();
        else wait_vm<NPT>();
    };
    const int ntap = p.kh * KW;
    const unsigned tile_stride = (unsigned)(NCH * p.Cop);
    int ps = s_begin, pbuf = 0;
    int pcs = s_begin / p.kh, ptap = (s_begin - pcs * p.kh) * KW;
    const bool tap_list = KW == 1 && p.ntl > 0;
    unsigned poff = (unsigned)((tap_list ? p.tl_w[ptap] : ptap) * p.ncs + pcs) * tile_stride;
    auto issue_b = [&]() -> bool {
        const bool any = ps < s_end;
        if (any) load_b(poff, pbuf);
        pbuf = pbuf + 1 == NB ? 0 : pbuf + 1;
        ++ptap;
        poff += (unsigned)p.ncs * tile_stride;
        if (ptap % KW == 0) ++ps;
        if (ptap == ntap) { ptap = 0; ++pcs; poff = (unsigned)pcs * tile_stride; }
        if constexpr (KW == 1)
            if (tap_list) poff = (unsigned)(p.tl_w[ptap] * p.ncs + pcs) * tile_stride;
        return any;
    };
    auto tap_koff = [&](int t, int c) -> int {
        if constexpr (KW == 1)
            if (tap_list) return (p.tl_dy[t] * p.Wx + p.tl_dx[t]) * p.Ci + c * XK;
        return (t - PADY) * p.Wx * p.Ci + c * XK;
    };

    using acc_t = typename std::conditional<MF16, f32x4, f32x16>::type;
    acc_t acc[RB][CB];
#pragma unroll
    for (int i = 0; i < RB; ++i)
#pragma unroll
        for (int j = 0; j < CB; ++j)
#pragma unroll
            for (int r = 0; r < (MF16 ? 4 : 16); ++r) acc[i][j][r] = 0.f;

    f16x8 hfa[RB][2], hfb[CB][2];
    auto mma_tap = [&](int abuf, int bbuf, int kx, int tap0, int phase = 2) __attribute__((always_inline)) {
        const char *la = reinterpret_cast<const char *>(lA + abuf * A_VEC);
        const char *lb = reinterpret_cast<const char *>(lB + bbuf * B_VEC);
        int arow[RB];
#pragma unroll
        for (int i = 0; i < RB; ++i) {
            arow[i] = a_frag0 + (i * RBLK + kx) * 16;
            if constexpr (KW > 1) arow[i] = ((vmask[i] >> (tap0 + kx)) & 1u) ? arow[i] : zero_frag;
        }
        if constexpr (MF16) {
            bf16x8 fa01[RB], fa02[RB];
#pragma unroll
            for (int i = 0; i < RB; ++i) {
                fa01[i] = *reinterpret_cast<const bf16x8 *>(la + arow[i] + a_c0);
                fa02[i] = *reinterpret_cast<const bf16x8 *>(la + arow[i] + a_c1);
            }
#pragma unroll
            for (int j = 0; j < CB; ++j) {
                const bf16x8 fb01 = *reinterpret_cast<const bf16x8 *>(lb + b_c0 + j * 16 * 16);
                const bf16x8 fb10 = *reinterpret_cast<const bf16x8 *>(lb + b_c1 + j * 16 * 16);
                const bf16x8 fb20 = *reinterpret_cast<const bf16x8 *>(lb + b_c2 + j * 16 * 16);
#pragma unroll
                for (int i = 0; i < RB; ++i) {
                    acc[i][j] = __builtin_amdgcn_mfma_f32_16x16x32_bf16(fa02[i], fb20, acc[i][j], 0, 0, 0);
                    acc[i][j] = __builtin_amdgcn_mfma_f32_16x16x32_bf16(fa01[i], fb10, acc[i][j], 0, 0, 0);
                    acc[i][j] = __builtin_amdgcn_mfma_f32_16x16x32_bf16(fa01[i], fb01, acc[i][j], 0, 0, 0);
                }
            }
        } else if constexpr (H2) {
            if (phase != 1) {
#pragma unroll
                for (int i = 0; i < RB; ++i)
#pragma unroll
                    for (int q = 0; q < 2; ++q)
                        hfa[i][q] = *reinterpret_cast<const f16x8 *>(la + arow[i] + a_c0 + q * 2 * G::PITCH * 16);
#pragma unroll
                for (int j = 0; j < CB; ++j)
#pragma unroll
                    for (int q = 0; q < 2; ++q)
                        hfb[j][q] = *reinterpret_cast<const f16x8 *>(lb + b_c0 + j * 32 * 16 + q * 2 * BN * 16);
            }
            if (phase != 0) {
#pragma unroll
                for (int i = 0; i < RB; ++i)
#pragma unroll
                    for (int j = 0; j < CB; ++j) {
                        acc[i][j] = __builtin_amdgcn_mfma_f32_32x32x16_f16(hfa[i][1], hfb[j][0], acc[i][j], 0, 0, 0);
                        acc[i][j] = __builtin_amdgcn_mfma_f32_32x32x16_f16(hfa[i][0], hfb[j][1], acc[i][j], 0, 0, 0);
                        acc[i][j] = __builtin_amdgcn_mfma_f32_32x32x16_f16(hfa[i][0], hfb[j][0], acc[i][j], 0, 0, 0);
                    }
            }
        } else {
            bf16x8 fa[RB][3], fb[CB][3];
#pragma unroll
            for (int i = 0; i < RB; ++i)
#pragma unroll
                for (int q = 0; q < 3; ++q)
                    fa[i][q] = *reinterpret_cast<const bf16x8 *>(la + arow[i] + a_c0 + q * 2 * G::PITCH * 16);
#pragma unroll
            for (int j = 0; j < CB; ++j)
#pragma unroll
                for (int q = 0; q < 3; ++q)
                    fb[j][q] = *reinterpret_cast<const bf16x8 *>(lb + b_c0 + j * 32 * 16 + q * 2 * BN * 16);
#pragma unroll
            for (int i = 0; i < RB; ++i)
#pragma unroll
                for (int j = 0; j < CB; ++j) {
                    acc[i][j] = __builtin_amdgcn_mfma_f32_32x32x16_bf16(fa[i][2], fb[j][0], acc[i][j], 0, 0, 0);
                    acc[i][j] = __builtin_amdgcn_mfma_f32_32x32x16_bf16(fa[i][0], fb[j][2], acc[i][j], 0, 0, 0);
                    acc[i][j] = __builtin_amdgcn_mfma_f32_32x32x16_bf16(fa[i][1], fb[j][1], acc[i][j], 0, 0, 0);
                    acc[i][j] = __builtin_amdgcn_mfma_f32_32x32x16_bf16(fa[i][1], fb[j][0], acc[i][j], 0, 0, 0);
                    acc[i][j] = __builtin_amdgcn_mfma_f32_32x32x16_bf16(fa[i][0], fb[j][1], acc[i][j], 0, 0, 0);
                    acc[i][j] = __builtin_amdgcn_mfma_f32_32x32x16_bf16(fa[i][0], fb[j][0], acc[i][j], 0, 0, 0);
                }
        }
    };

    int s = s_begin;
    int cs = s_begin / p.kh, ky = s_begin - cs * p.kh;
    int cs1 = cs, ky1 = ky;
    if (++ky1 == p.kh) { ky1 = 0; ++cs1; }
    int cs2 = cs1, ky2 = ky1;
    if (++ky2 == p.kh) { ky2 = 0; ++cs2; }
#pragma unroll
    for (int d = 0; d < DIST; ++d) issue_b();
    {
        const int shift0 = (ky - PADY) * p.Wx, koff0 = tap_koff(ky, cs);
        if constexpr (KW == 1) {
#pragma unroll
            for (int i = 0; i < NP; ++i) load_pass(ky, koff0, i, i, true);
            wait_vm<0>();
#pragma unroll
            for (int i = 0; i < NP; ++i) landed(ra[i]);
#pragma unroll
            for (int i = 0; i < NP; ++i) store_pass(0, i, i);
#pragma unroll
            for (int i = 0; i < NP; ++i) load_pass(ky1, tap_koff(ky1, cs1), i, NP + i, s_begin + 1 < s_end);
        } else {
            load_pass(shift0, koff0, 0, 0, true);
            load_pass(shift0, koff0, 1, 1, true);
            wait_vm<0>();
            landed(ra[0]);
            landed(ra[1]);
            store_pass(0, 0, 0);
            store_pass(0, 1, 1);
            if constexpr (NP > 2) {
                load_pass(shift0, koff0, 2, 0, true);
                wait_vm<0>();
                landed(ra[0]);
                store_pass(0, 2, 0);
            }
            const int sh = (ky1 - PADY) * p.Wx;
            load_pass(sh, sh * p.Ci + cs1 * XK, 0, 1, s_begin + 1 < s_end);
        }
    }
    lds_barrier();

    int bbuf = 0, abuf = 0, kx = 0;
    int n1shift = (ky1 - PADY) * p.Wx, n1koff = tap_koff(ky1, cs1);
    int n2shift = (ky2 - PADY) * p.Wx, n2koff = tap_koff(ky2, cs2);
    auto tap = [&](int P, bool TAIL) __attribute__((always_inline)) {
        const bool more = s + 1 < s_end, more2 = s + 2 < s_end;
        if constexpr (H2 && HTD_X3H_FRAG_FIRST) mma_tap(abuf, bbuf, kx, ky * KW, 0);
        const bool issued = issue_b();
        if (!TAIL) {
            if constexpr (KW == 1) {
#pragma unroll
                for (int i = 0; i < NP; ++i) load_pass(ky2, n2koff, i, P * NP + i, more2);
            } else {
                const bool last = kx == KW - 1;
                load_pass(last ? n2shift : n1shift, last ? n2koff : n1koff, last ? 0 : kx + 1, P, last ? more2 : more);
            }
        }
        if constexpr (EARLY) {
            if (TAIL) wait_vm<0>();
            else if (issued) wait_vm<NPT + NI_MIN>();
            else wait_vm<NPT>();
#pragma unroll
            for (int i = 0; i < NPT; ++i) landed(ra[(P ^ 1) * NPT + i]);
            mma_tap(abuf, bbuf, kx, ky * KW, (H2 && HTD_X3H_FRAG_FIRST) ? 1 : 2);
            if constexpr (KW == 1) {
#pragma unroll
                for (int i = 0; i < NP; ++i) store_pass(abuf ^ 1, i, (P ^ 1) * NP + i);
            } else {
                store_pass(abuf ^ 1, kx, P ^ 1);
            }
            constexpr int NM = RB * CB * ((MF16 || H2) ? 3 : 6);
            constexpr int PER = (NPT * 36 + NM - 1) / NM;
            __builtin_amdgcn_sched_group_barrier(0x002, 4, 0);
#pragma unroll
            for (int e = 0; e < NM; ++e) {
                __builtin_amdgcn_sched_group_barrier(0x008, 1, 0);
                __builtin_amdgcn_sched_group_barrier(0x002, PER, 0);
            }
            if (!TAIL) {
                if (DIST >= 2 && issued) wait_vm<NPT + NI_MIN>();
                else wait_vm<NPT>();
            }
        } else {
            mma_tap(abuf, bbuf, kx, ky * KW, (H2 && HTD_X3H_FRAG_FIRST) ? 1 : 2);
            if (TAIL) wait_vm<0>();
            else wait_tap(issued);
#pragma unroll
            for (int i = 0; i < NPT; ++i) landed(ra[(P ^ 1) * NPT + i]);
            if (more) {
                if constexpr (KW == 1) {
#pragma unroll
                    for (int i = 0; i < NP; ++i) store_pass(abuf ^ 1, i, (P ^ 1) * NP + i);
                } else {
                    store_pass(abuf ^ 1, kx, P ^ 1);
                }
            }
        }
        lds_barrier();
        bbuf = bbuf + 1 == NB ? 0 : bbuf + 1;
        if (++kx == KW) {
            kx = 0;
            ++s;
            abuf ^= 1;
            cs = cs1; ky = ky1;
            cs1 = cs2; ky1 = ky2;
            if (++ky2 == p.kh) { ky2 = 0; ++cs2; }
            n1shift = n2shift; n1koff = n2koff;
            n2shift = (ky2 - PADY) * p.Wx;
            n2koff = tap_koff(ky2, cs2);
        }
    };
    const int taps_total = (s_end - s_begin) * KW;
    int t = 0;
#pragma unroll 1
    for (; t + 1 < taps_total; t += 2) {
        tap(0, false);
        tap(1, false);
    }
    if (t < taps_total) tap(0, true);
    wait_vm<0>();
#pragma unroll
    for (int i = 0; i < 2 * NPT; ++i) landed(ra[i]);

    x3_epilogue<WGM, WGN, TM, TN, MF16>(p, acc, lds, m0, n0, part, region_b, split);
}

template <int WGM, int WGN, int TM, int TN, int NS>
constexpr int x3q_occupancy()
{
    constexpr int BM = WGM * TM * 32, BN = WGN * TN * 32;
    constexpr int main_bytes = NS * NCH * (BM + BN) * 16;
    constexpr int epi_bytes = WGM * 32 * (BN + 4) * 4;
    constexpr int by_lds = 163840 / (main_bytes > epi_bytes ? main_bytes : epi_bytes);
    constexpr int by_regs = TM * TN >= 4 ? 3 : 4;
    return by_lds < by_regs ? by_lds : by_regs;
}

template <int WGM, int WGN, int TM, int TN, bool MF16, int NS>
__global__ __launch_bounds__(256, (x3q_occupancy<WGM, WGN, TM, TN, NS>())) void conv_x3q_kernel(X3Params p)
{
    constexpr int BM = WGM * TM * 32, BN = WGN * TN * 32;
    constexpr int A_VEC = NCH * BM, B_VEC = NCH * BN;
    constexpr int MAIN_VEC = NS * (A_VEC + B_VEC);
    constexpr int EPI_VEC = WGM * 32 * (BN + 4) / 4;
    constexpr int LDS_VEC = MAIN_VEC > EPI_VEC ? MAIN_VEC : EPI_VEC;
    __shared__ uint4 lds[LDS_VEC];
    uint4 *const lA = lds, *const lB = lds + NS * A_VEC;
    const unsigned lds_a0 = (unsigned)(size_t)(__attribute__((address_space(3))) void *)lA;
    const unsigned lds_b0 = (unsigned)(size_t)(__attribute__((address_space(3))) void *)lB;

    int bid = blockIdx.x, split = 0, sps = 0;
    bool part = false;
    const bool region_b = bid >= p.tiles_a * p.splits_a;
    if (region_b) {
        const int r = bid - p.tiles_a * p.splits_a;
        bid = p.tiles_a + r / p.splits_b;
        split = r % p.splits_b;
        part = p.splits_b > 1;
        sps = p.sps_b;
    } else if (p.splits_a > 1) {
        split = bid % p.splits_a;
        bid = bid / p.splits_a;
        part = true;
        sps = p.sps_a;
    } else {
        const int q = p.tiles_a / 8, r = p.tiles_a % 8, xcd = bid % 8, idx = bid / 8;
        bid = (xcd < r ? xcd * (q + 1) : r * (q + 1) + (xcd - r) * q) + idx;
    }
    const int tile_m = bid / p.nt, tile_n = bid % p.nt;
    const int64_t m0 = (int64_t)tile_m * BM;
    const int n0 = tile_n * BN;

    const int tid = threadIdx.x, lane = tid & 63, wave = tid >> 6;
    const int wm = wave / WGN, wn = wave % WGN;
    const int frow = lane & 31, fhalf = lane >> 5;
    constexpr int RBLK = MF16 ? 16 : 32;
    constexpr int RB = TM * 32 / RBLK, CB = TN * 32 / RBLK;
    const int lrow = MF16 ? (lane & 15) : frow;
    const int kg = lane >> 4;
    const int a_row = (wm * TM * 32 + lrow) * 16;
    const int a_c0 = (MF16 ? kg * BM * 16 : fhalf * BM * 16) + a_row;
    const int a_c1 = MF16 ? ((kg >> 1) * 4 + (kg & 1)) * BM * 16 + a_row : 0;
    const int b_row = (wn * TN * 32 + lrow) * 16;
    const int b_c0 = (MF16 ? kg * BN * 16 : fhalf * BN * 16) + b_row;
    const int b_c1 = MF16 ? ((1 - (kg >> 1)) * 2 + (kg & 1)) * BN * 16 + b_row : 0;
    const int b_c2 = MF16 ? (((kg >> 1) ? 0 : 4) + (kg & 1)) * BN * 16 + b_row : 0;

    const int total_steps = p.ncs;
    const int s_begin = part ? split * sps : 0;
    const int s_end = part ? min(total_steps, s_begin + sps) : total_steps;

    constexpr int NIA = NCH * BM / 64, NIB = NCH * BN / 64, NI = NIA + NIB, NIW = (NI + 3) / 4;
    const int wave_u = __builtin_amdgcn_readfirstlane(wave);
    const uint4 *src[NIW];
    unsigned dst[NIW], adv[NIW];
#pragma unroll
    for (int k = 0; k < NIW; ++k) {
        const int idx = wave_u + 4 * k;
        if (idx < NIA) {
            const int chunk = idx / (BM / 64), half = idx % (BM / 64);
            src[k] = p.xp + (int64_t)chunk * p.xp_rows + m0 + half * 64 + lane;
            dst[k] = lds_a0 + (unsigned)((chunk * BM + half * 64) * 16);
            adv[k] = (unsigned)(NCH * p.xp_rows);
        } else {
            const int j = (idx < NI ? idx : NIA) - NIA, chunk = j / (BN / 64), half = j % (BN / 64);
            src[k] = p.wp + (int64_t)chunk * p.Cop + n0 + half * 64 + lane;
            dst[k] = lds_b0 + (unsigned)((chunk * BN + half * 64) * 16);
            adv[k] = (unsigned)(NCH * p.Cop);
        }
    }
    auto issue = [&](int s, int stage) __attribute__((always_inline)) {
#pragma unroll
        for (int k = 0; k < NIW; ++k) {
            const int idx = wave_u + 4 * k;
            if (NI % 4 != 0 && idx >= NI) continue;
            const unsigned st = (unsigned)stage * (unsigned)((idx < NIA ? A_VEC : B_VEC) * 16);
            lds_dma16(src[k] + (int64_t)s * adv[k], dst[k] + st);
        }
    };
    auto lds_barrier = [&]() {
        asm volatile("s_waitcnt lgkmcnt(0)" ::: "memory");
        __builtin_amdgcn_s_barrier();
        asm volatile("" ::: "memory");
    };

    using acc_t = typename std::conditional<MF16, f32x4, f32x16>::type;
    acc_t acc[RB][CB];
#pragma unroll
    for (int i = 0; i < RB; ++i)
#pragma unroll
        for (int j = 0; j < CB; ++j)
#pragma unroll
            for (int r = 0; r < (MF16 ? 4 : 16); ++r) acc[i][j][r] = 0.f;

    auto mma = [&](int stage) __attribute__((always_inline)) {
        const char *la = reinterpret_cast<const char *>(lA + stage * A_VEC);
        const char *lb = reinterpret_cast<const char *>(lB + stage * B_VEC);
        if constexpr (MF16) {
            bf16x8 fa01[RB], fa02[RB];
#pragma unroll
            for (int i = 0; i < RB; ++i) {
                fa01[i] = *reinterpret_cast<const bf16x8 *>(la + a_c0 + i * 16 * 16);
                fa02[i] = *reinterpret_cast<const bf16x8 *>(la + a_c1 + i * 16 * 16);
            }
#pragma unroll
            for (int j = 0; j < CB; ++j) {
                const bf16x8 fb01 = *reinterpret_cast<const bf16x8 *>(lb + b_c0 + j * 16 * 16);
                const bf16x8 fb10 = *reinterpret_cast<const bf16x8 *>(lb + b_c1 + j * 16 * 16);
                const bf16x8 fb20 = *reinterpret_cast<const bf16x8 *>(lb + b_c2 + j * 16 * 16);
#pragma unroll
                for (int i = 0; i < RB; ++i) {
                    acc[i][j] = __builtin_amdgcn_mfma_f32_16x16x32_bf16(fa02[i], fb20, acc[i][j], 0, 0, 0);
                    acc[i][j] = __builtin_amdgcn_mfma_f32_16x16x32_bf16(fa01[i], fb10, acc[i][j], 0, 0, 0);
                    acc[i][j] = __builtin_amdgcn_mfma_f32_16x16x32_bf16(fa01[i], fb01, acc[i][j], 0, 0, 0);
                }
            }
        } else {
            bf16x8 fa[RB][3], fb[CB][3];
#pragma unroll
            for (int i = 0; i < RB; ++i)
#pragma unroll
                for (int q = 0; q < 3; ++q) fa[i][q] = *reinterpret_cast<const bf16x8 *>(la + a_c0 + i * 32 * 16 + q * 2 * BM * 16);
#pragma unroll
            for (int j = 0; j < CB; ++j)
#pragma unroll
                for (int q = 0; q < 3; ++q) fb[j][q] = *reinterpret_cast<const bf16x8 *>(lb + b_c0 + j * 32 * 16 + q * 2 * BN * 16);
#pragma unroll
            for (int i = 0; i < RB; ++i)
#pragma unroll
                for (int j = 0; j < CB; ++j) {
                    acc[i][j] = __builtin_amdgcn_mfma_f32_32x32x16_bf16(fa[i][2], fb[j][0], acc[i][j], 0, 0, 0);
                    acc[i][j] = __builtin_amdgcn_mfma_f32_32x32x16_bf16(fa[i][0], fb[j][2], acc[i][j], 0, 0, 0);
                    acc[i][j] = __builtin_amdgcn_mfma_f32_32x32x16_bf16(fa[i][1], fb[j][1], acc[i][j], 0, 0, 0);
                    acc[i][j] = __builtin_amdgcn_mfma_f32_32x32x16_bf16(fa[i][1], fb[j][0], acc[i][j], 0, 0, 0);
                    acc[i][j] = __builtin_amdgcn_mfma_f32_32x32x16_bf16(fa[i][0], fb[j][1], acc[i][j], 0, 0, 0);
// ... 764 lines not shown
                       (const PlanesDescH *)desc, n);
    hipLaunchKernelGGL(x3h_planes_many_kernel, dim3((unsigned)total_blocks), dim3(256), 0, (hipStream_t)stream,
                       (const PlanesDescH *)desc, n);
    return htd::check_launch("x3h_planes_many");
}

extern "C" int htd_absmax(const float *x, int64_t n, float *amax, void *stream)
{
    HTD_REQUIRE(x && amax && n > 0 && ((uintptr_t)x & 15) == 0, "absmax: bad arguments");
    const unsigned blocks = (unsigned)std::min<int64_t>(htd::ceil_div(n >> 2, (int64_t)256 * 8) + 1, 2048);
    hipLaunchKernelGGL(absmax_kernel, dim3(blocks), dim3(256), 0, (hipStream_t)stream, x, n, (unsigned *)amax);
    return htd::check_launch("absmax");
}

extern "C" int htd_conv2d_x3_planes_many(const void *desc, int n, int64_t total_blocks, void *stream)
{
    static_assert(sizeof(PlanesDesc) == 40, "PlanesDesc layout is part of the ABI");
    HTD_REQUIRE(desc && n > 0 && total_blocks > 0 && total_blocks < (1ll << 31), "x3_planes_many: bad arguments");
    hipLaunchKernelGGL(x3_planes_many_kernel, dim3((unsigned)total_blocks), dim3(256), 0, (hipStream_t)stream,
                       (const PlanesDesc *)desc, n);
    return htd::check_launch("x3_planes_many");
}

extern "C" int64_t htd_conv2d_x3p_workspace_bytes(int64_t M, int Co, int Ci, int kh, int kw)
{
    int64_t need = 0;
    for (int cfg = 0; cfg < 4; ++cfg) need = std::max(need, plan_x3p(cfg, M, Co, (Ci / XK) * kh, kw, true).partial_floats * 4);
    return need;
}

extern "C" int64_t htd_act_planes_rows(int64_t M) { return M > 0 ? act_rows(M) : 0; }

extern "C" int64_t htd_act_planes_bytes(int64_t M, int C)
{
    if (M <= 0 || C <= 0 || C % XK != 0) return 0;
    return (int64_t)(C / XK) * NCH * act_rows(M) * 16;
}

extern "C" int htd_act_planes(const float *x, void *planes, int64_t M, int C, void *stream)
{
    HTD_REQUIRE(x && planes && M > 0 && C > 0 && C % XK == 0, "act_planes: bad arguments (C %% 16)");
    const unsigned blocks = (unsigned)std::min<int64_t>(htd::ceil_div(M * (C >> 3), (int64_t)256), 65536);
    hipLaunchKernelGGL(act_planes_kernel, dim3(blocks), dim3(256), 0, (hipStream_t)stream, x, (uint4 *)planes, M, C, act_rows(M));
    return htd::check_launch("act_planes");
}

extern "C" int htd_conv2d_fwd_x3q(const float *x, const void *xplanes, const void *wplanes, const float *bias,
                                  const float *residual, int res_h, int res_w, float *y, void *yplanes, float *amax_out, int B, int H,
                                  int W, int Ci, int Co, int kh, int kw, int stride, int pad, int relu, void *workspace, void *stream)
{
    HTD_REQUIRE((x || xplanes) && wplanes && y && B > 0 && H > 0 && W > 0, "conv2d_fwd_x3q: bad arguments");
    HTD_REQUIRE(x3p_shape_ok(Ci, Co, kh, kw, stride, pad, 1), "conv2d_fwd_x3q: unsupported layer Ci=%d Co=%d k=%dx%d s=%d p=%d", Ci,
                Co, kh, kw, stride, pad);
    HTD_REQUIRE(!xplanes || (kh == 1 && stride == 1), "conv2d_fwd_x3q: input planes serve 1x1 / stride-1 layers only");
    HTD_REQUIRE(!yplanes || Co % XK == 0, "conv2d_fwd_x3q: output planes need Co %% 16 == 0 (Co=%d)", Co);
    HTD_REQUIRE((res_h > 0) == (res_w > 0) && res_h >= 0 && (res_h == 0 || ((Co & 3) == 0 && residual)),
                "conv2d_fwd_x3q: bad residual up-sampling arguments");
    X3Params p{};
    p.x = x; p.wp = (const uint4 *)wplanes; p.bias = bias; p.residual = residual; p.y = y;
    p.Hx = H; p.Wx = W;
    p.Ho = (H + 2 * pad - kh) / stride + 1;
    p.Wo = (W + 2 * pad - kw) / stride + 1;
    p.Ci = Ci; p.Co = Co; p.Cop = planes_np(Co); p.kh = kh; p.stride = stride; p.relu = relu;
    p.M = (int64_t)B * p.Ho * p.Wo;
    p.ncs = Ci / XK;
    p.xp = (const uint4 *)xplanes; p.xp_rows = act_rows(p.M);
    p.yp = (uint4 *)yplanes; p.yp_rows = act_rows(p.M);
    p.amax_out = amax_out;
    HTD_REQUIRE((int64_t)B * H * W * Ci < (1ll << 31) && p.M * Co < (1ll << 40), "conv2d_fwd_x3q: operand too large");
    if (res_h > 0) {
        p.res_H = res_h; p.res_W = res_w;
        p.res_sh = (float)res_h / (float)p.Ho; p.res_sw = (float)res_w / (float)p.Wo;
    }
    return launch_x3p(p, kw, (hipStream_t)stream, workspace);
}

extern "C" int htd_conv2d_fwd_x3p(const float *x, const void *wplanes, const float *bias, const float *residual, int res_h,
                                  int res_w, float *y, int B, int H, int W, int Ci, int Co, int kh, int kw, int stride, int pad,
                                  int relu, void *workspace, void *stream)
{
    HTD_REQUIRE(x, "conv2d_fwd_x3p: bad arguments");
    return htd_conv2d_fwd_x3q(x, nullptr, wplanes, bias, residual, res_h, res_w, y, nullptr, nullptr, B, H, W, Ci, Co, kh, kw, stride,
                              pad, relu, workspace, stream);
}

extern "C" int htd_conv2d_bwd_data_x3q(const float *gy, const void *gyplanes, const void *wplanesT, const float *mask_src,
                                       const float *accum, float *gx, void *gxplanes, float *amax_out, int B, int H, int W, int Ci,
                                       int Co, int kh, int kw, int pad, void *workspace, void *stream)
{
    HTD_REQUIRE((gy || gyplanes) && wplanesT && gx && B > 0 && H > 0 && W > 0, "conv2d_bwd_data_x3q: bad arguments");
    HTD_REQUIRE(x3p_shape_ok(Co, Ci, kh, kw, 1, pad, 1), "conv2d_bwd_data_x3q: unsupported layer Ci=%d Co=%d k=%dx%d p=%d", Ci, Co,
                kh, kw, pad);
    HTD_REQUIRE(!gyplanes || kh == 1, "conv2d_bwd_data_x3q: gradient planes serve 1x1 layers only");
    HTD_REQUIRE(!gxplanes || Ci % XK == 0, "conv2d_bwd_data_x3q: output planes need Ci %% 16 == 0 (Ci=%d)", Ci);
    X3Params p{};
    p.x = gy; p.wp = (const uint4 *)wplanesT; p.residual = accum; p.mask_src = mask_src; p.y = gx;
    p.Hx = H; p.Wx = W; p.Ho = H; p.Wo = W;
    p.Ci = Co; p.Co = Ci; p.Cop = planes_np(Ci); p.kh = kh; p.stride = 1;
    p.M = (int64_t)B * H * W;
    p.ncs = Co / XK;
    p.xp = (const uint4 *)gyplanes; p.xp_rows = act_rows(p.M);
    p.yp = (uint4 *)gxplanes; p.yp_rows = act_rows(p.M);
    p.amax_out = amax_out;
    HTD_REQUIRE((int64_t)B * H * W * Co < (1ll << 31), "conv2d_bwd_data_x3q: operand too large");
    return launch_x3p(p, kw, (hipStream_t)stream, workspace);
}

extern "C" int htd_conv2d_bwd_data_x3p(const float *gy, const void *wplanesT, const float *mask_src, const float *accum,
                                       float *gx, int B, int H, int W, int Ci, int Co, int kh, int kw, int pad, void *workspace,
                                       void *stream)
{
    HTD_REQUIRE(gy, "conv2d_bwd_data_x3p: bad arguments");
    return htd_conv2d_bwd_data_x3q(gy, nullptr, wplanesT, mask_src, accum, gx, nullptr, nullptr, B, H, W, Ci, Co, kh, kw, pad,
                                   workspace, stream);
}

extern "C" int htd_conv2d_fwd_x3h(const float *x, const float *amax, const void *wplanes, const float *bias, const float *residual,
                                  int res_h, int res_w, float *y, void *yplanes, float *amax_out, int B, int H, int W, int Ci,
                                  int Co, int kh, int kw, int stride, int pad, int relu, void *workspace, void *stream)
{
    HTD_REQUIRE(!yplanes || Co % XK == 0, "conv2d_fwd_x3h: output planes need Co %% 16 == 0 (Co=%d)", Co);
    HTD_REQUIRE(x && amax && wplanes && y && B > 0 && H > 0 && W > 0, "conv2d_fwd_x3h: bad arguments");
    const bool taps = x3h_strided_ok(Ci, Co, kh, kw, stride, pad);
    HTD_REQUIRE(taps || x3p_shape_ok(Ci, Co, kh, kw, stride, pad, 1), "conv2d_fwd_x3h: unsupported layer Ci=%d Co=%d k=%dx%d s=%d p=%d",
                Ci, Co, kh, kw, stride, pad);
    HTD_REQUIRE(!taps || (!yplanes && res_h == 0), "conv2d_fwd_x3h: strided 3x3 layers write no planes and take no up-sampled residual");
    HTD_REQUIRE((res_h > 0) == (res_w > 0) && res_h >= 0 && (res_h == 0 || ((Co & 3) == 0 && residual)),
                "conv2d_fwd_x3h: bad residual up-sampling arguments");
    X3Params p{};
    p.x = x; p.wp = (const uint4 *)wplanes; p.bias = bias; p.residual = residual; p.y = y;
    p.Hx = H; p.Wx = W;
    p.Ho = (H + 2 * pad - kh) / stride + 1;
    p.Wo = (W + 2 * pad - kw) / stride + 1;
    p.Ci = Ci; p.Co = Co; p.Cop = planes_np(Co); p.kh = kh; p.stride = stride; p.relu = relu;
    p.M = (int64_t)B * p.Ho * p.Wo;
    p.ncs = Ci / XK;
    p.amax = amax;
    p.wscale = reinterpret_cast<const float *>(p.wp + planes_vec(kh * kw, Ci, p.Cop));
    p.yp = (uint4 *)yplanes; p.yp_rows = act_rows(p.M);
    p.amax_out = amax_out;
    HTD_REQUIRE((int64_t)B * H * W * Ci < (1ll << 31) && p.M * Co < (1ll << 40), "conv2d_fwd_x3h: operand too large");
    if (res_h > 0) {
        p.res_H = res_h; p.res_W = res_w;
        p.res_sh = (float)res_h / (float)p.Ho; p.res_sw = (float)res_w / (float)p.Wo;
    }
    if (taps) {
        p.kh = p.ntl = kh * kw;
        for (int t = 0; t < p.ntl; ++t) { p.tl_dy[t] = t / kw - pad; p.tl_dx[t] = t % kw - pad; p.tl_w[t] = t; }
        return launch_x3p(p, 1, (hipStream_t)stream, workspace);
    }
    return launch_x3p(p, kw, (hipStream_t)stream, workspace);
}

extern "C" int htd_conv2d_bwd_data_x3h(const float *gy, const float *amax, const void *wplanesT, const float *mask_src,
                                       const float *accum, float *gx, void *gxplanes, float *amax_out, int B, int H, int W,
                                       int Ci, int Co, int kh, int kw, int pad, void *workspace, void *stream)
{
    HTD_REQUIRE(!gxplanes || Ci % XK == 0, "conv2d_bwd_data_x3h: output planes need Ci %% 16 == 0 (Ci=%d)", Ci);
    HTD_REQUIRE(gy && amax && wplanesT && gx && B > 0 && H > 0 && W > 0, "conv2d_bwd_data_x3h: bad arguments");
    HTD_REQUIRE(x3p_shape_ok(Co, Ci, kh, kw, 1, pad, 1), "conv2d_bwd_data_x3h: unsupported layer Ci=%d Co=%d k=%dx%d p=%d", Ci, Co, kh,
                kw, pad);
    X3Params p{};
    p.x = gy; p.wp = (const uint4 *)wplanesT; p.residual = accum; p.mask_src = mask_src; p.y = gx;
    p.Hx = H; p.Wx = W; p.Ho = H; p.Wo = W;
    p.Ci = Co; p.Co = Ci; p.Cop = planes_np(Ci); p.kh = kh; p.stride = 1;
    p.M = (int64_t)B * H * W;
    p.ncs = Co / XK;
    p.amax = amax;
    p.wscale = reinterpret_cast<const float *>(p.wp + planes_vec(kh * kw, Co, p.Cop));
    p.yp = (uint4 *)gxplanes; p.yp_rows = act_rows(p.M);
    p.amax_out = amax_out;
    HTD_REQUIRE((int64_t)B * H * W * Co < (1ll << 31), "conv2d_bwd_data_x3h: operand too large");
    return launch_x3p(p, kw, (hipStream_t)stream, workspace);
}

namespace {
struct StridedClass { int ntaps; int dy[9], dx[9], w[9]; int Ho, Wo; };
int strided_classes(int H, int W, int kh, int kw, int stride, int pad, StridedClass *cls)
{
    int n = 0;
    for (int c = 0; c < stride * stride; ++c) {
        const int ph = c / stride, pw = c % stride;
        StridedClass &q = cls[c];
        q.ntaps = 0;
        q.Ho = ph < H ? (H - ph + stride - 1) / stride : 0;
        q.Wo = pw < W ? (W - pw + stride - 1) / stride : 0;
        if (q.Ho == 0 || q.Wo == 0) continue;
        for (int ky = 0; ky < kh; ++ky) {
            const int ry = ph + pad - ky;
            if (((ry % stride) + stride) % stride != 0) continue;
            for (int kx = 0; kx < kw; ++kx) {
                const int rx = pw + pad - kx;
                if (((rx % stride) + stride) % stride != 0) continue;
                q.dy[q.ntaps] = ry >= 0 ? ry / stride : -((-ry) / stride);
                q.dx[q.ntaps] = rx >= 0 ? rx / stride : -((-rx) / stride);
                q.w[q.ntaps] = (kh - 1 - ky) * kw + (kw - 1 - kx);
                ++q.ntaps;
            }
        }
        n += q.ntaps > 0;
    }
    return n;
}
bool x3h_strided_dgrad_ok(int Ci, int Co, int kh, int kw, int stride, int pad)
{
    static const bool on = !(getenv("HTD_X3H_STRIDED") && atoi(getenv("HTD_X3H_STRIDED")) == 0);
    return on && Co % XK == 0 && Ci >= 33 && stride == 2 && ((kh == 3 && kw == 3 && pad == 1) || (kh == 1 && kw == 1 && pad == 0));
}
}

extern "C" int htd_conv2d_bwd_data_x3h_strided_supported(int Ci, int Co, int kh, int kw, int stride, int pad, int dil)
{
    return (g_conv_h2 == 1 && !x3p_off() && htd::conv_math() == 1 && dil == 1 && x3h_strided_dgrad_ok(Ci, Co, kh, kw, stride, pad)) ? 1 : 0;
}

extern "C" int64_t htd_conv2d_bwd_data_x3h_strided_workspace_bytes(int B, int H, int W, int Ci, int Co, int kh, int kw, int stride, int pad)
{
    if (!x3h_strided_dgrad_ok(Ci, Co, kh, kw, stride, pad) || B <= 0 || H <= 0 || W <= 0) return 0;
    StridedClass cls[4];
    strided_classes(H, W, kh, kw, stride, pad, cls);
    int64_t need = 0;
    for (int c = 0; c < stride * stride; ++c)
        if (cls[c].ntaps > 0)
            need = std::max(need, htd_conv2d_x3p_workspace_bytes((int64_t)B * cls[c].Ho * cls[c].Wo, Ci, Co, cls[c].ntaps, 1));
    return need;
}

extern "C" int htd_conv2d_bwd_data_x3h_strided(const float *gy, const float *amax, const void *wplanesT, const float *mask_src,
                                               float *gx, float *amax_out, int B, int H, int W, int Ci, int Co, int kh, int kw,
                                               int stride, int pad, void *workspace, void *stream)
{
    HTD_REQUIRE(gy && amax && wplanesT && gx && B > 0 && H > 0 && W > 0, "conv2d_bwd_data_x3h_strided: bad arguments");
    HTD_REQUIRE(x3h_strided_dgrad_ok(Ci, Co, kh, kw, stride, pad), "conv2d_bwd_data_x3h_strided: unsupported layer Ci=%d Co=%d k=%dx%d s=%d p=%d",
                Ci, Co, kh, kw, stride, pad);
    const int Ho = (H + 2 * pad - kh) / stride + 1, Wo = (W + 2 * pad - kw) / stride + 1;
    HTD_REQUIRE(Ho > 0 && Wo > 0 && (int64_t)B * Ho * Wo * Co < (1ll << 31) && (int64_t)B * H * W * Ci < (1ll << 40),
                "conv2d_bwd_data_x3h_strided: bad sizes");
    StridedClass cls[4];
    const int live = strided_classes(H, W, kh, kw, stride, pad, cls);
    if (live < stride * stride) {
        if (hipMemsetAsync(gx, 0, (size_t)B * H * W * Ci * 4, (hipStream_t)stream) != hipSuccess) {
            htd::set_error("conv2d_bwd_data_x3h_strided: memset failed");
            return HTD_ERR_LAUNCH;
        }
    }
    X3Params p{};
    p.x = gy; p.wp = (const uint4 *)wplanesT; p.mask_src = mask_src; p.y = gx;
    p.Hx = Ho; p.Wx = Wo;
    p.Ci = Co; p.Co = Ci; p.Cop = planes_np(Ci); p.stride = 1;
    p.ncs = Co / XK;
    p.amax = amax;
    p.wscale = reinterpret_cast<const float *>(p.wp + planes_vec(kh * kw, Co, p.Cop));
    p.amax_out = amax_out;
    p.o_step = stride; p.oH = H; p.oW = W;
    for (int c = 0; c < stride * stride; ++c) {
        const StridedClass &q = cls[c];
        if (q.ntaps == 0) continue;
        X3Params r = p;
        r.Ho = q.Ho; r.Wo = q.Wo;
        r.M = (int64_t)B * q.Ho * q.Wo;
        r.kh = r.ntl = q.ntaps;
        for (int t = 0; t < q.ntaps; ++t) { r.tl_dy[t] = q.dy[t]; r.tl_dx[t] = q.dx[t]; r.tl_w[t] = q.w[t]; }
        r.o_h0 = c / stride; r.o_w0 = c % stride;
        const int st = launch_x3p(r, 1, (hipStream_t)stream, workspace);
        if (st) return st;
    }
    return HTD_OK;
}
```

### htd_amd/dense.py

```python
import os

import torch
from torch.autograd import Function
from torch.autograd.function import once_differentiable
from torch.multiprocessing.reductions import StorageWeakRef as _StorageWeakRef

from . import capi
from .mmcv_ops import chain_outputs

CL = torch.channels_last
_P = capi.ptr
_S = capi.current_stream_ptr


def _out_hw(H, W, kh, kw, stride, pad, dil):
    return ((H + 2 * pad - (dil * (kh - 1) + 1)) // stride + 1, (W + 2 * pad - (dil * (kw - 1) + 1)) // stride + 1)


def _need_gpu(t, name):
    if not t.is_cuda:
        raise NotImplementedError(f'{name}: only GPU tensors are supported (libhtd_amd.so has no CPU path)')


def _splitk_ws(M, Co, Cred, kh, kw, device):
# ... 421 lines not shown
    return torch.empty(capi.lib().htd_act_planes_bytes(M, C) // 4, device=device, dtype=torch.int32)


def act_planes(x):
    x = x.contiguous(memory_format=CL)
    B, C, H, W = x.shape
    out = _act_planes_buf(B * H * W, C, x.device)
    capi.call('htd_act_planes', _P(x), _P(out), B * H * W, C, _S(), work=('byte', 10.0 * x.numel()))
    return out


def _planes_pay(w_consumer, transposed=False, rows=None):
    if not ACT_PLANES or w_consumer.dim() != 4 or w_consumer.dtype != torch.float32:
        return False
    if H2_1X1 and capi.lib().htd_conv2d_set_h2(-1) == 1:
        return False
    if rows is not None and rows < ACT_PLANES_MIN_ROWS:
        return False
    Co, Ci, kh, kw = w_consumer.shape
    cred, cout = (Co, Ci) if transposed else (Ci, Co)
    return kh == 1 and kw == 1 and cred % 16 == 0 and (cout + 127) // 128 >= ACT_PLANES_MIN_TILES and \
        bool(capi.lib().htd_conv2d_x3p_supported(cred, cout, 1, 1, 1, 0, 1))


def _fwd_raw(x, weight, bias, residual, stride, padding, dilation, relu, res_up=False, x_planes=None, emit=None):
    y = _fwd_raw_(x, weight, bias, residual, stride, padding, dilation, relu, res_up, x_planes, bool(emit))
    if emit is not None:
        return y if isinstance(y, tuple) else (y, None)
    return y


def _fwd_raw_(x, weight, bias, residual, stride, padding, dilation, relu, res_up, x_planes, emit):
    B, Ci, H, W = x.shape
    Co, Ci_w, kh, kw = weight.shape
    if Ci != Ci_w:
        raise ValueError(f'conv2d: input has {Ci} channels, weight expects {Ci_w}')
    Ho, Wo = _out_hw(H, W, kh, kw, stride, padding, dilation)
    y = torch.empty((B, Co, Ho, Wo), device=x.device, dtype=x.dtype, memory_format=CL)
    if y.numel() == 0:
        return y
    flops = 2.0 * B * Ho * Wo * Co * kh * kw * Ci
    rh, rw = (residual.size(2), residual.size(3)) if (res_up and residual is not None) else (0, 0)
    if _stem7_ok(x, weight, stride, padding, dilation, residual):
        ws = torch.empty(capi.lib().htd_conv2d_stem7_workspace_bytes() // 4, device=x.device, dtype=torch.float32)
        capi.call('htd_conv2d_stem7_fwd', _P(x), _P(weight), _P(bias), _P(y), B, H, W, int(bool(relu)), _P(ws), _S(),
                  work=('flop', flops, 4.0 * (x.numel() + weight.numel() + y.numel())))
        return y
    if _x3p_ok(Ci, Co, kh, kw, stride, padding, dilation, x.dtype):
        nb = capi.lib().htd_conv2d_x3p_workspace_bytes(B * Ho * Wo, Co, Ci, kh, kw)
        ws = torch.empty(nb // 4, device=x.device, dtype=torch.float32) if nb > 0 else None
        use_xp = x_planes is not None and kh == 1 and stride == 1
        yp = _act_planes_buf(B * Ho * Wo, Co, x.device) if (emit and Co % 16 == 0) else None
        work = ('flop', flops, 4.0 * (x.numel() + weight.numel() + y.numel() + (y.numel() if residual is not None else 0)))
        h2 = _x3h_ok(Ci, Co, kh, kw, stride, padding, dilation, x.dtype)
        out_slot = _amax_slot(x.device) if h2 else None
        if h2:
            am = carried_amax(x)
            if am is None:
                _h2_trace('fwd', x, weight)
            if am is None and kh * kw * Co >= H2_ABSMAX_MIN_WORK and x.numel() >= H2_ABSMAX_MIN_ELEMS:
                am = absmax(x)
            if am is not None:
                capi.call('htd_conv2d_fwd_x3h', _P(x), _P(am), _P(x3_planes(weight, False, True)), _P(bias), _P(residual), rh, rw,
                          _P(y), _P(yp), _P(out_slot), B, H, W, Ci, Co, kh, kw, stride, padding,
                          int(bool(relu)), _P(ws), _S(), work=work)
                tag_amax(y, out_slot)
                _h2_guard(am, out_slot)
                return (y, yp) if emit else y
        capi.call('htd_conv2d_fwd_x3q', _P(x), _P(x_planes) if use_xp else None, _P(x3_planes(weight, False, False)), _P(bias),
                  _P(residual), rh, rw, _P(y), _P(yp), _P(out_slot), B, H, W, Ci, Co, kh, kw, stride, padding, int(bool(relu)),
                  _P(ws), _S(), key='htd_conv2d_fwd_x3p', work=work)
        if out_slot is not None:
            tag_amax(y, out_slot)
        return (y, yp) if emit else y
    work = ('flop', flops, 4.0 * (x.numel() + weight.numel() + y.numel() + (y.numel() if residual is not None else 0)))
    if x.dtype == torch.float32 and rh == 0 and \
            capi.lib().htd_conv2d_x3h_strided_supported(Ci, Co, kh, kw, stride, padding, dilation):
        am = carried_amax(x)
        if am is None:
            _h2_trace('fwd', x, weight)
            if kh * kw * Co >= H2_ABSMAX_MIN_WORK and x.numel() >= H2_ABSMAX_MIN_ELEMS:
                am = absmax(x)
        if am is not None:
            nb = capi.lib().htd_conv2d_x3p_workspace_bytes(B * Ho * Wo, Co, Ci, kh * kw, 1)
            ws = torch.empty(nb // 4, device=x.device, dtype=torch.float32) if nb > 0 else None
            out_slot = _amax_slot(x.device)
            capi.call('htd_conv2d_fwd_x3h', _P(x), _P(am), _P(x3_planes(weight, False, True)), _P(bias), _P(residual), 0, 0, _P(y), None,
                      _P(out_slot), B, H, W, Ci, Co, kh, kw, stride, padding, int(bool(relu)), _P(ws), _S(), work=work)
            tag_amax(y, out_slot)
            _h2_guard(am, out_slot)
            return y
    if _igemm_emits(y, Co):
        slot = _amax_slot(x.device)
        capi.call('htd_conv2d_fwd_amax', _P(x), _P(weight), _P(bias), _P(residual), rh, rw, _P(y), _P(slot), B, H, W, Ci, Co, kh, kw,
                  stride, padding, dilation, int(bool(relu)), _P(_splitk_ws(B * Ho * Wo, Co, Ci, kh, kw, x.device)), _S(),
                  key='htd_conv2d_fwd', work=work)
        tag_amax(y, slot)
        return y
    capi.call('htd_conv2d_fwd', _P(x), _P(weight), _P(bias), _P(residual), rh, rw, _P(y), B, H, W, Ci, Co, kh, kw, stride,
              padding, dilation, int(bool(relu)), _P(_splitk_ws(B * Ho * Wo, Co, Ci, kh, kw, x.device)), _S(), work=work)
    return y


def _igemm_emits(y, C):
    return y.dtype == torch.float32 and C >= 64 and emits('igemm')


def _colsum_raw(g, y=None, bias=None):
    B, Co, Ho, Wo = g.shape
    gm = torch.empty_like(g, memory_format=CL) if y is not None else g
    gb = grad_out(bias) if bias is not None else torch.empty(Co, device=g.device, dtype=g.dtype)
    if g.numel() == 0:
        return gm, gb.zero_()
    ws = torch.empty(2048 * Co, device=g.device, dtype=g.dtype)
    work = ('byte', 4.0 * B * Ho * Wo * Co * (3 if y is not None else 1))
    if _mask_emits(g):
        slot = _amax_slot(g.device)
        capi.call('htd_bias_grad_relu_mask_amax', _P(g), _P(y), _P(gm) if y is not None else None, _P(gb), B * Ho * Wo, Co,
                  _P(ws), _P(slot), _S(), key='htd_bias_grad_relu_mask', work=work)
        tag_amax(gm, slot)
    else:
        capi.call('htd_bias_grad_relu_mask', _P(g), _P(y), _P(gm) if y is not None else None, _P(gb), B * Ho * Wo, Co,
                  _P(ws), _S(), work=work)
    return gm, gb


H2_EMIT_OFF = frozenset(v for v in os.environ.get('HTD_H2_EMIT_OFF', '').split(',') if v)


def emits(kind):
    return kind not in H2_EMIT_OFF and capi.lib().htd_conv2d_set_h2(-1) == 1


def _mask_emits(g):
    return g.dtype == torch.float32 and emits('mask')


def _mask_raw(g, y):
    B, Co, Ho, Wo = g.shape
    gm = torch.empty_like(g, memory_format=CL)
    if g.numel() == 0:
        return gm
    if _mask_emits(g):
        slot = _amax_slot(g.device)
        capi.call('htd_bias_grad_relu_mask_amax', _P(g), _P(y), _P(gm), None, B * Ho * Wo, Co, None, _P(slot), _S(),
                  key='htd_bias_grad_relu_mask', work=('byte', 12.0 * B * Ho * Wo * Co))
        tag_amax(gm, slot)
    else:
        capi.call('htd_bias_grad_relu_mask', _P(g), _P(y), _P(gm), None, B * Ho * Wo, Co, None, _S(),
                  work=('byte', 12.0 * B * Ho * Wo * Co))
    return gm


def _dgrad_raw(g, weight, x_shape, stride, padding, dilation, mask_src=None, accum=None, wT=None, g_planes=None, emit=None):
    gx = _dgrad_raw_(g, weight, x_shape, stride, padding, dilation, mask_src, accum, wT, g_planes, bool(emit))
    if emit is not None:
        return gx if isinstance(gx, tuple) else (gx, None)
    return gx


def _dgrad_raw_(g, weight, x_shape, stride, padding, dilation, mask_src, accum, wT, g_planes, emit):
    B, Ci, H, W = x_shape
    Co, _, kh, kw = weight.shape
    Ho, Wo = g.shape[2], g.shape[3]
    if B == 0:
        return torch.empty((0, Ci, H, W), device=g.device, dtype=g.dtype, memory_format=CL)
    if stride == 1 and _x3p_ok(Co, Ci, kh, kw, 1, padding, dilation, g.dtype):
        gx = torch.empty((B, Ci, H, W), device=g.device, dtype=g.dtype, memory_format=CL)
        nb = capi.lib().htd_conv2d_x3p_workspace_bytes(B * H * W, Ci, Co, kh, kw)
        ws = torch.empty(nb // 4, device=g.device, dtype=torch.float32) if nb > 0 else None
        use_gp = g_planes is not None and kh == 1
        gxp = _act_planes_buf(B * H * W, Ci, g.device) if (emit and Ci % 16 == 0) else None
        work = ('flop', 2.0 * B * Ho * Wo * Co * kh * kw * Ci,
                4.0 * (g.numel() + weight.numel() + gx.numel() * (1 + (mask_src is not None) + (accum is not None))))
        h2 = _x3h_ok(Co, Ci, kh, kw, 1, padding, dilation, g.dtype)
        out_slot = _amax_slot(g.device) if h2 else None
        if h2:
            am = carried_amax(g)
            if am is None:
                _h2_trace('dgrad', g, weight)
            if am is None and kh * kw * Ci >= H2_ABSMAX_MIN_WORK and g.numel() >= H2_ABSMAX_MIN_ELEMS:
                am = absmax(g)
            if am is not None:
                capi.call('htd_conv2d_bwd_data_x3h', _P(g), _P(am), _P(x3_planes(weight, True, True)), _P(mask_src), _P(accum), _P(gx),
                          _P(gxp), _P(out_slot), B, H, W, Ci, Co, kh, kw, padding, _P(ws), _S(), work=work)
                tag_amax(gx, out_slot)
                _h2_guard(am, out_slot)
                return (gx, gxp) if emit else gx
        capi.call('htd_conv2d_bwd_data_x3q', _P(g), _P(g_planes) if use_gp else None, _P(x3_planes(weight, True, False)), _P(mask_src),
                  _P(accum), _P(gx), _P(gxp), _P(out_slot), B, H, W, Ci, Co, kh, kw, padding, _P(ws), _S(),
                  key='htd_conv2d_bwd_data_x3p', work=work)
        if out_slot is not None:
            tag_amax(gx, out_slot)
        return (gx, gxp) if emit else gx
    if stride != 1 and accum is None and g.dtype == torch.float32 and \
            capi.lib().htd_conv2d_bwd_data_x3h_strided_supported(Ci, Co, kh, kw, stride, padding, dilation):
        am = carried_amax(g)
        if am is None:
            _h2_trace('dgrad', g, weight)
            if kh * kw * Ci >= H2_ABSMAX_MIN_WORK and g.numel() >= H2_ABSMAX_MIN_ELEMS:
                am = absmax(g)
        if am is not None:
            gx = torch.empty((B, Ci, H, W), device=g.device, dtype=g.dtype, memory_format=CL)
            nb = capi.lib().htd_conv2d_bwd_data_x3h_strided_workspace_bytes(B, H, W, Ci, Co, kh, kw, stride, padding)
            ws = torch.empty(nb // 4, device=g.device, dtype=torch.float32) if nb > 0 else None
            out_slot = _amax_slot(g.device)
            capi.call('htd_conv2d_bwd_data_x3h_strided', _P(g), _P(am), _P(x3_planes(weight, True, True)), _P(mask_src), _P(gx),
                      _P(out_slot), B, H, W, Ci, Co, kh, kw, stride, padding, _P(ws), _S(), key='htd_conv2d_bwd_data_x3h',
                      work=('flop', 2.0 * B * Ho * Wo * Co * kh * kw * Ci,
                            4.0 * (g.numel() + weight.numel() + gx.numel() * (1 + (mask_src is not None)))))
            tag_amax(gx, out_slot)
            _h2_guard(am, out_slot)
            return gx
    gd, Cod = g, Co
    if Co % 8 != 0:
        Cod = Co + (-Co) % 8
        gd = torch.empty((B, Cod, Ho, Wo), device=g.device, dtype=g.dtype, memory_format=CL)
        if gd.numel():
            capi.call('htd_pad_channels', _P(g), _P(gd), B * Ho * Wo, Co, Cod, _S())
    if wT is None or Cod != Co:
        key = _flip_key(weight)
        hit = _STEP_FLIPS.get(key) if Cod == Co else None
        wT = hit[1] if hit is not None else None
        if wT is None:
            wT = torch.empty(Ci * kh * kw * Cod, device=g.device, dtype=g.dtype)
            if Cod != Co:
                capi.call('htd_conv2d_flip_weights_padded', _P(weight), _P(wT), Co, Cod, kh, kw, Ci, _S())
            else:
                capi.call('htd_conv2d_flip_weights', _P(weight), _P(wT), Co, kh, kw, Ci, _S())
                _STEP_FLIPS[key] = (weight, wT)
    gx = torch.empty((B, Ci, H, W), device=g.device, dtype=g.dtype, memory_format=CL)
    work = ('flop', 2.0 * B * Ho * Wo * Co * kh * kw * Ci,
            4.0 * (g.numel() + weight.numel() + gx.numel() * (1 + (mask_src is not None) + (accum is not None))))
    if _igemm_emits(gx, Ci):
        slot = _amax_slot(g.device)
        capi.call('htd_conv2d_bwd_data_amax', _P(gd), _P(wT), _P(mask_src), _P(accum), _P(gx), _P(slot), B, H, W, Ci, Cod, kh, kw,
                  stride, padding, dilation, _P(_splitk_ws(B * H * W, Ci, Cod, kh, kw, g.device)), _S(),
                  key='htd_conv2d_bwd_data', work=work)
        tag_amax(gx, slot)
        return gx
    capi.call('htd_conv2d_bwd_data', _P(gd), _P(wT), _P(mask_src), _P(accum), _P(gx), B, H, W, Ci, Cod, kh, kw, stride,
              padding, dilation, _P(_splitk_ws(B * H * W, Ci, Cod, kh, kw, g.device)), _S(), work=work)
    return gx


SINK_ACCUMULATE = os.environ.get('HTD_SINK_ACC', '1') != '0'


H2_WGRAD = os.environ.get('HTD_H2_WGRAD', '1') != '0'


def _wgrad_amax(x, g, weight, stride, padding, dilation):
    if not H2_WGRAD or x.dtype != torch.float32:
        return None
    B, Ci, H, W = x.shape
    Co, _, kh, kw = weight.shape
    if B * g.size(2) * g.size(3) == 0 or \
            not capi.lib().htd_conv2d_bwd_weight_h2_supported(B, H, W, Ci, Co, kh, kw, stride, padding, dilation):
        return None
    ax, ag = carried_amax(x), carried_amax(g)
    if ax is None:
        _h2_trace('wgrad x', x, weight)
    if ag is None:
        _h2_trace('wgrad g', g, weight)
    if (ax is None and (kh * kw * Co < H2_ABSMAX_MIN_WORK or x.numel() < H2_ABSMAX_MIN_ELEMS)) or \
            (ag is None and (kh * kw * Ci < H2_ABSMAX_MIN_WORK or g.numel() < H2_ABSMAX_MIN_ELEMS)):
        return None
    return (ax if ax is not None else absmax(x)), (ag if ag is not None else absmax(g))


def _wgrad_launch(x, g, weight, stride, padding, dilation, bias, amax=None):
    B, Ci, H, W = x.shape
    Co, _, kh, kw = weight.shape
    Ho, Wo = g.shape[2], g.shape[3]
    aw = grad_sink_again(weight) if SINK_ACCUMULATE else None
    ab = grad_sink_again(bias) if (aw is not None and torch.is_tensor(bias)) else None
    if aw is not None and (bias is None or ab is not None) and B * Ho * Wo > 0:
        nbytes = capi.lib().htd_conv2d_wgrad_workspace_bytes(B, H, W, Ci, Co, kh, kw, stride, padding, dilation)
        ws = torch.empty(nbytes // 4 + 1, device=g.device, dtype=g.dtype)
        work = ('flop', 2.0 * B * Ho * Wo * Co * kh * kw * Ci, 4.0 * (x.numel() + g.numel() + aw.numel()))
        if amax is not None:
            capi.call('htd_conv2d_bwd_weight_h2', _P(x), _P(g), _P(amax[0]), _P(amax[1]), _P(aw), _P(ab), B, H, W, Ci, Co, kh, kw,
                      stride, padding, dilation, 1, _P(ws), _S(), work=work)
        else:
            capi.call('htd_conv2d_bwd_weight_acc', _P(x), _P(g), _P(aw), _P(ab), B, H, W, Ci, Co, kh, kw, stride, padding,
                      dilation, _P(ws), _S(), key='htd_conv2d_bwd_weight', work=work)
        ent = _GRAD_SINK.get(weight.data_ptr())
        return None, None, not (ent is not None and ent[2] is _TEMP_USED)
    gw, sink_w = grad_out2(weight)
    gb, sink_b = (None, True)
    if bias is not None:
        gb, sink_b = grad_out2(bias) if torch.is_tensor(bias) else (torch.empty(Co, device=g.device, dtype=g.dtype), False)
    if B * Ho * Wo == 0:
        gw.zero_()
        if gb is not None:
            gb.zero_()
        return gw, gb, sink_w and sink_b
    nbytes = capi.lib().htd_conv2d_wgrad_workspace_bytes(B, H, W, Ci, Co, kh, kw, stride, padding, dilation)
    ws = torch.empty(nbytes // 4 + 1, device=g.device, dtype=g.dtype)
    work = ('flop', 2.0 * B * Ho * Wo * Co * kh * kw * Ci, 4.0 * (x.numel() + g.numel() + gw.numel()))
    if amax is not None:
        capi.call('htd_conv2d_bwd_weight_h2', _P(x), _P(g), _P(amax[0]), _P(amax[1]), _P(gw), _P(gb), B, H, W, Ci, Co, kh, kw,
                  stride, padding, dilation, 0, _P(ws), _S(), work=work)
    else:
        capi.call('htd_conv2d_bwd_weight', _P(x), _P(g), _P(gw), _P(gb), B, H, W, Ci, Co, kh, kw, stride, padding,
                  dilation, _P(ws), _S(), work=work)
    return gw, gb, sink_w and sink_b


def _wgrad_raw(x, g, weight, stride, padding, dilation, bias=None, overlap=True):
    amax = _wgrad_amax(x, g, weight, stride, padding, dilation)
    if not overlap or not OVERLAP_WGRAD or (capi.profiling() and not _OVERLAP_IN_PROFILE):
        if OVERLAP_WGRAD and _SIDE and SINK_ACCUMULATE and grad_sink_again(weight) is not None:
            torch.cuda.current_stream().wait_stream(side_stream(g.device))
        return _wgrad_launch(x, g, weight, stride, padding, dilation, bias, amax)[:2]
    main, side = torch.cuda.current_stream(), side_stream(g.device)
    side.wait_stream(main)
    x.record_stream(side)
    g.record_stream(side)
    with torch.cuda.stream(side):
        gw, gb, sinks = _wgrad_launch(x, g, weight, stride, padding, dilation, bias, amax)
    if not sinks and weight.data_ptr() not in _SIDE_CONSUMED:
        if gw is not None:
            gw.record_stream(main)
        if gb is not None:
            gb.record_stream(main)
        main.wait_stream(side)
    return gw, gb


def _dgrad_joined(galias, g, weight, x_shape, stride, padding, dilation):
    fuse = galias is not None and stride == 1 and galias.dtype == g.dtype and tuple(galias.shape) == tuple(x_shape)
    gx = _dgrad_raw(g, weight, x_shape, stride, padding, dilation, accum=galias.contiguous(memory_format=CL) if fuse else None)
    return gx if (galias is None or fuse) else gx + galias


class Conv2dFunction(Function):
    @staticmethod
    def forward(ctx, x, weight, bias, residual, stride, padding, dilation, relu, res_up=False, chain=False):
        _need_gpu(x, 'conv2d')
        src = x
        x = x.contiguous(memory_format=CL)
        weight = weight.contiguous(memory_format=CL)
        res = residual.contiguous(memory_format=CL) if residual is not None else None
        b = bias.contiguous() if bias is not None else None
        y = _fwd_raw(x, weight, b, res, stride, padding, dilation, relu, res_up)
        ctx.save_for_backward(x, weight, y if relu else None)
        ctx.cfg = (stride, padding, dilation, bool(relu), bias is not None, residual is not None)
        ctx.res_up = tuple(res.shape) if (res_up and res is not None) else None
        ctx.bias_ref = b
        return chain_outputs(ctx, y, (src, ), chain)

    @staticmethod
    @once_differentiable
    def backward(ctx, g, galias=None):
        x, weight, y = ctx.saved_tensors
        stride, padding, dilation, relu, has_bias, has_res = ctx.cfg
        if g is None:
            return (galias, ) + (None, ) * 9
        g = g.contiguous(memory_format=CL)
        need_x, need_w, need_b, need_r = ctx.needs_input_grad[:4]
        gb = gw = None
        want_b = has_bias and need_b
        if relu:
            if want_b and not need_w:
                g, gb = _colsum_raw(g, y, ctx.bias_ref)
            else:
                g = _mask_raw(g, y)
        elif want_b and not need_w:
            gb = _colsum_raw(g, None, ctx.bias_ref)[1]
        gx = _dgrad_joined(galias, g, weight, x.shape, stride, padding, dilation) if need_x else None
        aliases_g = has_res and need_r and ctx.res_up is None
        if need_w:
            gw, gb = _wgrad_raw(x, g, weight, stride, padding, dilation, ctx.bias_ref if want_b else None,
                                overlap=not aliases_g)
        gr = None
        if has_res and need_r:
            gr = g
            if ctx.res_up is not None:
                rB, rC, rh, rw = ctx.res_up
                gr = torch.empty((rB, rC, rh, rw), device=g.device, dtype=g.dtype, memory_format=CL)
                capi.call('htd_upsample_nearest_bwd', _P(g), _P(gr), rB, g.size(2), g.size(3), rh, rw, rC, _S(),
                          work=('byte', 4.0 * (g.numel() + gr.numel())))
        return gx, gw, (gb if (has_bias and need_b) else None), gr, None, None, None, None, None, None


class ConvReluHeadFunction(Function):

    @staticmethod
    def forward(ctx, x, w1, b1, w2, b2, padding, chain):
        _need_gpu(x, 'conv_relu_head')
        src = x
        x = x.contiguous(memory_format=CL)
        w1, w2 = w1.contiguous(memory_format=CL), w2.contiguous(memory_format=CL)
        b1 = b1.contiguous() if b1 is not None else None
        b2 = b2.contiguous() if b2 is not None else None
        h = _fwd_raw(x, w1, b1, None, 1, padding, 1, True)
        y = _fwd_raw(h, w2, b2, None, 1, 0, 1, False)
        ctx.save_for_backward(x, w1, w2, h)
        ctx.cfg = (int(padding), b1, b2)
        return chain_outputs(ctx, y, (src, ), chain)

    @staticmethod
    @once_differentiable
    def backward(ctx, gy, galias=None):
        x, w1, w2, h = ctx.saved_tensors
        padding, b1, b2 = ctx.cfg
        if gy is None:
            return (galias, ) + (None, ) * 6
        need_x, need_w1, need_b1, need_w2, need_b2 = ctx.needs_input_grad[:5]
        gy = gy.contiguous(memory_format=CL)
        gw1 = gb1 = gw2 = gb2 = None
        if need_w2:
            gw2, gb2 = _wgrad_raw(h, gy, w2, 1, 0, 1, b2 if (need_b2 and b2 is not None) else None)
        elif need_b2 and b2 is not None:
            gb2 = _colsum_raw(gy, None, b2)[1]
        gh = _dgrad_raw(gy, w2, h.shape, 1, 0, 1, mask_src=h)
        if need_w1:
            gw1, gb1 = _wgrad_raw(x, gh, w1, 1, padding, 1, b1 if (need_b1 and b1 is not None) else None)
        elif need_b1 and b1 is not None:
            gb1 = _colsum_raw(gh, None, b1)[1]
        gx = _dgrad_joined(galias, gh, w1, x.shape, 1, padding, 1) if need_x else galias
        return gx, gw1, gb1, gw2, gb2, None, None


def conv_relu_head(x, w1, b1, w2, b2, padding=1, chain=False):
    return ConvReluHeadFunction.apply(x, w1, b1, w2, b2, int(padding), bool(chain))



def _gconv_pack(weight, groups, transpose):
    C, cg, kh, kw = weight.shape
    n = capi.lib().htd_gconv2d_packed_floats(C, groups, kh, kw)
    if n <= 0:
        raise ValueError(f'grouped conv2d: {C} channels in {groups} groups is unsupported')
    wp = torch.empty(n, device=weight.device, dtype=weight.dtype)
    capi.call('htd_gconv2d_pack_weights', _P(weight), _P(wp), C, groups, kh, kw, int(transpose), _S())
    return wp


def _gconv_fwd_raw(x, wp, bias, geom, relu, cols_shape=None):
    C, groups, kh, kw, stride, padding, dilation = geom
    B, H, W = cols_shape if cols_shape is not None else (x.size(0), x.size(2), x.size(3))
    Ho, Wo = _out_hw(H, W, kh, kw, stride, padding, dilation)
    y = torch.empty((B, C, Ho, Wo), device=x.device, dtype=x.dtype, memory_format=CL)
    capi.call('htd_gconv2d_fwd', _P(x), _P(wp), _P(bias), _P(y), B, H, W, C, groups, kh, kw, stride, padding, dilation,
              int(bool(relu)), int(cols_shape is not None), _S(),
              work=('flop', 2.0 * B * Ho * Wo * C * kh * kw * (C // groups), 4.0 * (x.numel() + y.numel())))
    return y


def _gconv_dgrad_raw(g, wpT, geom, x_shape, cols=False):
    C, groups, kh, kw, stride, padding, dilation = geom
    B, _, H, W = x_shape
    M = g.size(0) * g.size(2) * g.size(3)
    gx = torch.empty((M, kh * kw, C), device=g.device, dtype=g.dtype) if cols else \
        torch.empty((B, C, H, W), device=g.device, dtype=g.dtype, memory_format=CL)
    capi.call('htd_gconv2d_bwd_data', _P(g), _P(wpT), _P(gx), B, H, W, C, groups, kh, kw, stride, padding, dilation,
              int(cols), _S(), work=('flop', 2.0 * M * C * kh * kw * (C // groups), 4.0 * (g.numel() + gx.numel())))
    return gx


def _gconv_wgrad_raw(x, g, weight, geom, x_shape, cols=False):
    C, groups, kh, kw, stride, padding, dilation = geom
    B, _, H, W = x_shape
    gw = grad_out(weight)
    nbytes = capi.lib().htd_gconv2d_wgrad_workspace_bytes(B, H, W, C, groups, kh, kw, stride, padding, dilation)
    ws = torch.empty(nbytes // 4 + 1, device=g.device, dtype=g.dtype)
    M = g.size(0) * g.size(2) * g.size(3)
    capi.call('htd_gconv2d_bwd_weight', _P(x), _P(g), _P(gw), B, H, W, C, groups, kh, kw, stride, padding, dilation,
              int(cols), _P(ws), _S(), work=('flop', 2.0 * M * C * kh * kw * (C // groups), 4.0 * (x.numel() + g.numel())))
    return gw


class GroupedConv2dFunction(Function):

    @staticmethod
    def forward(ctx, x, weight, bias, stride, padding, dilation, groups, relu):
        _need_gpu(x, 'grouped conv2d')
        x = x.contiguous(memory_format=CL)
        weight = weight.contiguous(memory_format=CL)
        C, cg, kh, kw = weight.shape
        if x.size(1) != C or cg * groups != C:
            raise ValueError(f'grouped conv2d: input {tuple(x.shape)}, weight {tuple(weight.shape)}, groups {groups}')
        if x.dtype != torch.float32:
            raise TypeError('grouped conv2d runs in fp32')
        geom = (C, groups, kh, kw, stride, padding, dilation)
        b = bias.contiguous() if bias is not None else None
        y = _gconv_fwd_raw(x, _gconv_pack(weight, groups, False), b, geom, relu)
        ctx.save_for_backward(x, weight, y if relu else None)
        ctx.geom, ctx.relu, ctx.bias_ref = geom, bool(relu), b
        return y

    @staticmethod
    @once_differentiable
    def backward(ctx, g):
        x, weight, y = ctx.saved_tensors
        g = g.contiguous(memory_format=CL)
        need_x, need_w, need_b = ctx.needs_input_grad[:3]
        gb = None
        if ctx.bias_ref is not None and need_b:
            g, gb = _colsum_raw(g, y if ctx.relu else None, ctx.bias_ref)
        elif ctx.relu:
            g = _mask_raw(g, y)
        gx = _gconv_dgrad_raw(g, _gconv_pack(weight, ctx.geom[1], True), ctx.geom, x.shape) if need_x else None
        gw = _gconv_wgrad_raw(x, g, weight, ctx.geom, x.shape) if need_w else None
        return gx, gw, gb, None, None, None, None, None


def grouped_conv2d(x, weight, bias=None, stride=1, padding=0, dilation=1, groups=1, relu=False):
    return GroupedConv2dFunction.apply(x, weight, bias, int(stride), int(padding), int(dilation), int(groups), bool(relu))


class ResStageFunction(Function):

    @staticmethod
    def forward(ctx, x, strides, dilation, has_ds, *params):
        _need_gpu(x, 'res_stage')
        x = x.contiguous(memory_format=CL)
        params = [t.contiguous(memory_format=CL) if t.dim() == 4 else t.contiguous() for t in params]
        saved, k = [], 0
        for stride, ds in zip(strides, has_ds):
            w1, b1, w2, b2, w3, b3 = params[k:k + 6]
            k += 6
            h1 = _fwd_raw(x, w1, b1, None, 1, 0, 1, True)
            h2, h2p = _fwd_raw(h1, w2, b2, None, stride, dilation, dilation, True,
                               emit=_planes_pay(w3, rows=h1.size(0) * (h1.size(2) // stride) * (h1.size(3) // stride)))
            if ds:
                wd, bd = params[k:k + 2]
                k += 2
                idn = _fwd_raw(x, wd, bd, None, stride, 0, 1, False)
            else:
                idn = x
            out = _fwd_raw(h2, w3, b3, idn, 1, 0, 1, True, x_planes=h2p)
            saved += [x, h1, h2, out]
            x = out
        ctx.save_for_backward(*saved, *params)
        ctx.cfg = (strides, dilation, has_ds)
        ctx.flipped = [take_flipped(t) if t.dim() == 4 else None for t in params]
        return x

    @staticmethod
    @once_differentiable
    def backward(ctx, g):
        strides, dilation, has_ds = ctx.cfg
        nb = len(strides)
        saved, params = ctx.saved_tensors[:4 * nb], ctx.saved_tensors[4 * nb:]
        flipped = ctx.flipped
        offs, k = [], 0
        for ds in has_ds:
            offs.append(k)
            k += 8 if ds else 6
        need = ctx.needs_input_grad
        grads = [None] * len(params)
        g = g.contiguous(memory_format=CL)
        premasked = False
        for i in range(nb - 1, -1, -1):
            x, h1, h2, out = saved[4 * i:4 * i + 4]
            k, stride, ds = offs[i], strides[i], has_ds[i]
            w1, b1, w2, b2, w3, b3 = params[k:k + 6]
            pneed = need[4 + k:4 + k + (8 if ds else 6)]
            first = i == 0
            need_x = need[0] if first else True
            gm3 = g if premasked else _mask_raw(g, out)
            gb3 = None
            if pneed[4]:
                grads[k + 4], gb3 = _wgrad_raw(h2, gm3, w3, 1, 0, 1, True if (pneed[5] or (ds and pneed[7])) else None)
            elif pneed[5] or (ds and pneed[7]):
                gb3 = _colsum_raw(gm3)[1]
            grads[k + 5] = gb3 if pneed[5] else None
            gm2 = _dgrad_raw(gm3, w3, h2.shape, 1, 0, 1, mask_src=h2, wT=flipped[k + 4])
            if pneed[2]:
                grads[k + 2], gb2 = _wgrad_raw(h1, gm2, w2, stride, dilation, dilation, True if pneed[3] else None)
            else:
                gb2 = _colsum_raw(gm2)[1] if pneed[3] else None
# ... 450 lines not shown
```

### include/htd_amd.h

```cpp
#ifndef HTD_AMD_H
#define HTD_AMD_H

#include <stdint.h>

#ifdef __cplusplus
extern "C" {
#endif

#define HTD_OK 0
#define HTD_ERR_ARG 1
#define HTD_ERR_LAUNCH 2

const char *htd_last_error(void);
#define HTD_ABI_VERSION 7
int htd_abi_version(void);

int htd_roi_align_fwd(const float *feat, const float *rois, const int64_t *roi_level, int level,
                      float *out, int64_t n, int B, int C, int H, int W, int ph, int pw, float spatial_scale,
                      int sampling_ratio, int aligned, void *stream);
int htd_roi_align_bwd(const float *grad_out, const float *rois, const int64_t *roi_level, int level,
                      float *grad_feat, int64_t n, int B, int C, int H, int W, int ph, int pw,
                      float spatial_scale, int sampling_ratio, int aligned, void *stream);
int htd_roi_align_levels_fwd(const float *const *feats, const int *H, const int *W, const float *scales, int L,
                             const float *rois, const int64_t *roi_level, float *out, int64_t n, int B, int C, int ph, int pw,
                             int sampling_ratio, int aligned, void *stream);
int htd_roi_align_levels_fwd_amax(const float *const *feats, const int *H, const int *W, const float *scales, int L,
                                  const float *rois, const int64_t *roi_level, float *out, int64_t n, int B, int C, int ph,
                                  int pw, int sampling_ratio, int aligned, float *amax_out, void *stream);
int htd_roi_align_levels_bwd_gather(const float *grad_out, const float *rois, const int64_t *roi_level,
                                    float *const *grad_feats, const int *H, const int *W, const float *scales,
                                    const int *accumulate, int L, int64_t n, int B, int C, int ph, int pw,
                                    int sampling_ratio, int aligned, void *workspace, void *stream);
int htd_roi_align_all_levels_fwd(const float *const *feats, const int *H, const int *W, const float *scales, int L,
                                 const float *rois, float *const *outs, int64_t n, int B, int C, int ph, int pw,
                                 int sampling_ratio, int aligned, void *stream);
int htd_roi_align_all_levels_bwd_gather(const float *const *grad_outs, const float *rois, float *const *grad_feats,
                                        const int *H, const int *W, const float *scales, const int *accumulate, int L,
                                        int64_t n, int B, int C, int ph, int pw, int sampling_ratio, int aligned,
                                        void *workspace, void *stream);
int64_t htd_roi_align_fold_workspace_bytes(int64_t n, const int *H, int L, int pw, int C);
int htd_roi_align_levels_bwd_gather_folded(const float *grad_out, const float *rois, const int64_t *roi_level,
                                           float *const *grad_feats, const int *H, const int *W, const float *scales,
                                           const int *accumulate, int L, int64_t n, int B, int C, int ph, int pw,
                                           int sampling_ratio, int aligned, void *workspace, void *fold_ws, void *stream);
int htd_roi_align_all_levels_bwd_gather_folded(const float *const *grad_outs, const float *rois, float *const *grad_feats,
                                               const int *H, const int *W, const float *scales, const int *accumulate,
                                               int L, int64_t n, int B, int C, int ph, int pw, int sampling_ratio,
                                               int aligned, void *workspace, void *fold_ws, void *stream);
int64_t htd_roi_align_bwd_gather_workspace_bytes(int64_t n);
int htd_roi_align_bwd_gather(const float *grad_out, const float *rois, const int64_t *roi_level, int level,
                             float *grad_feat, int64_t n, int B, int C, int H, int W, int ph, int pw,
                             float spatial_scale, int sampling_ratio, int aligned, int accumulate, void *workspace,
                             void *stream);

int64_t htd_nms_workspace_bytes(int64_t n_total);
int htd_nms_sorted(const float *boxes, uint8_t *keep_mask, int64_t n, float iou_thr, int offset,
                   void *workspace, void *stream);
int htd_nms_sorted_batched(const float *boxes, const int64_t *seg_offsets, int segments,
                           int64_t n_total, int64_t max_seg, uint8_t *keep_mask, float iou_thr,
                           int offset, void *workspace, void *stream);

int htd_soft_nms_segments(const float *boxes, float *scores, const int64_t *seg_offsets, int segments,
                          int64_t n_total, int *rank, float iou_thr, float sigma, float min_score,
                          int method, int offset, void *stream);

int64_t htd_segmented_topk_workspace_bytes(int S, int64_t nchunks);
int htd_segmented_topk(const float *keys, const int64_t *segs, const int32_t *chunk_tab, int S, int64_t nchunks,
                       int64_t *out_idx, float *out_val, void *workspace, void *stream);
int64_t htd_random_sample_workspace_bytes(int B, int64_t A, int64_t nchunks);
int htd_random_sample(const int64_t *assigned, const float *keys, int B, int64_t A, int num, int max_pos, float neg_pos_ub,
                      const int64_t *segs, const int32_t *chunk_tab, int64_t nchunks, unsigned char *pos_mask,
                      unsigned char *neg_mask, int64_t *counts, int64_t *order, int slots, void *workspace, void *stream);

int htd_fuse_global_fwd(const float *roi_feats, const float *rois, const float *global_feat,
                        const float *extra, float alpha, float *out, int64_t n, int P, int C,
                        int B, void *stream);
int htd_plain_and_fused_fwd(const float *roi_feats, const float *rois, const float *global_feat, float *both,
                            int64_t n, int P, int C, int B, void *stream);
int htd_fuse_global_fwd_amax(const float *roi_feats, const float *rois, const float *global_feat, const float *extra,
                             float alpha, float *out, int64_t n, int P, int C, int B, float *amax_out, void *stream);
int htd_plain_and_fused_fwd_amax(const float *roi_feats, const float *rois, const float *global_feat, float *both,
                                 int64_t n, int P, int C, int B, float *amax_out, void *stream);
int htd_fuse_global_bwd_global(const float *grad, const float *rois, float *grad_global,
                               int64_t n, int P, int C, int B, void *stream);

int htd_ba_fuse_fwd(const float *const *lvl, int L, const float *border, const float *att,
                    float *out, int64_t n, int ph, int pw, int C, int edge, void *stream);
int htd_ba_fuse_bwd(const float *const *lvl, int L, const float *att, const float *grad_out,
                    float *const *grad_lvl, float *grad_border, float *grad_att, int64_t n, int ph,
                    int pw, int C, int edge, void *stream);

int64_t htd_conv2d_workspace_bytes(int64_t M, int Co, int Ci, int kh, int kw);
int htd_conv2d_set_math(int mode);
int htd_conv2d_tile_table_set(int64_t M, int Co, int Ci, int taps, int epi, int cfg);
int htd_conv2d_tile_table_clear(void);
int htd_conv2d_tile_query(int64_t M, int Co, int Ci, int taps, int epi);
int htd_conv2d_fwd(const float *x, const float *w, const float *bias, const float *residual, int res_h,
                   int res_w, float *y, int B, int H, int W, int Ci, int Co, int kh, int kw, int stride,
                   int pad, int dil, int relu, void *workspace, void *stream);
int htd_bgemm_nt(const float *a, const float *b, float *c, int G, int M, int N, int K, void *stream);
int htd_bgemm_nt_counts(const float *a, const float *b, float *c, int G, int M, int N, int K, const int64_t *counts, int limit,
                        void *stream);
int htd_conv2d_flip_weights(const float *w, float *wT, int Co, int kh, int kw, int Ci, void *stream);
int htd_conv2d_flip_weights_padded(const float *w, float *wT, int Co, int Co_padded, int kh, int kw, int Ci, void *stream);
int htd_pad_channels(const float *x, float *y, int64_t rows, int C, int C_padded, void *stream);
int htd_conv2d_bwd_data(const float *gy, const float *wT, const float *mask_src, const float *accum, float *gx,
                        int B, int H, int W, int Ci, int Co, int kh, int kw, int stride, int pad, int dil,
                        void *workspace, void *stream);
int htd_conv2d_fwd_amax(const float *x, const float *w, const float *bias, const float *residual, int res_h, int res_w,
                        float *y, float *amax_out, int B, int H, int W, int Ci, int Co, int kh, int kw, int stride, int pad,
                        int dil, int relu, void *workspace, void *stream);
int htd_conv2d_bwd_data_amax(const float *gy, const float *wT, const float *mask_src, const float *accum, float *gx,
                             float *amax_out, int B, int H, int W, int Ci, int Co, int kh, int kw, int stride, int pad,
                             int dil, void *workspace, void *stream);
int64_t htd_conv2d_wgrad_workspace_bytes(int B, int H, int W, int Ci, int Co, int kh, int kw,
                                         int stride, int pad, int dil);
int htd_conv2d_bwd_weight(const float *x, const float *gy, float *gw, float *gbias, int B, int H, int W,
                          int Ci, int Co, int kh, int kw, int stride, int pad, int dil, void *workspace,
                          void *stream);
int htd_conv2d_bwd_weight_acc(const float *x, const float *gy, float *gw, float *gbias, int B, int H, int W, int Ci,
                              int Co, int kh, int kw, int stride, int pad, int dil, void *workspace, void *stream);
int htd_bias_grad_relu_mask(const float *g, const float *y, float *gm, float *gbias, int64_t rows,
                            int C, void *workspace, void *stream);
int htd_bias_grad_relu_mask_amax(const float *g, const float *y, float *gm, float *gbias, int64_t rows, int C,
                                 void *workspace, float *amax_out, void *stream);
int64_t htd_conv2d_stem7_workspace_bytes(void);
int htd_conv2d_stem7_fwd(const float *x, const float *w, const float *bias, float *y, int B, int H, int W, int relu,
                         void *workspace, void *stream);
int htd_conv2d_x3p_supported(int Ci, int Co, int kh, int kw, int stride, int pad, int dil);
int htd_conv2d_x3p_tile_table_set(int64_t M, int Co, int Ci, int taps, int epi, int cfg);
int htd_conv2d_x3p_tile_table_clear(void);
int htd_conv2d_x3p_tile_query(int64_t M, int Co, int Ci, int taps, int epi);
int htd_conv2d_x3p_plan_query(int cfg, int64_t M, int Co, int Ci, int kh, int kw, int64_t *out);
int64_t htd_conv2d_x3_planes_bytes(int Co, int kh, int kw, int Ci, int transposed);
int htd_conv2d_x3_planes(const float *w, void *planes, int Co, int kh, int kw, int Ci, int transposed, void *stream);
int htd_conv2d_x3_planes_many(const void *desc, int n, int64_t total_blocks, void *stream);
int64_t htd_conv2d_x3p_workspace_bytes(int64_t M, int Co, int Ci, int kh, int kw);
int htd_conv2d_fwd_x3p(const float *x, const void *wplanes, const float *bias, const float *residual, int res_h,
                       int res_w, float *y, int B, int H, int W, int Ci, int Co, int kh, int kw, int stride, int pad,
                       int relu, void *workspace, void *stream);
int htd_conv2d_bwd_data_x3p(const float *gy, const void *wplanesT, const float *mask_src, const float *accum,
                            float *gx, int B, int H, int W, int Ci, int Co, int kh, int kw, int pad, void *workspace,
                            void *stream);
int64_t htd_act_planes_rows(int64_t M);
int64_t htd_act_planes_bytes(int64_t M, int C);
int htd_act_planes(const float *x, void *planes, int64_t M, int C, void *stream);
int htd_conv2d_fwd_x3q(const float *x, const void *xplanes, const void *wplanes, const float *bias, const float *residual,
                       int res_h, int res_w, float *y, void *yplanes, float *amax_out, int B, int H, int W, int Ci, int Co, int kh, int kw,
                       int stride, int pad, int relu, void *workspace, void *stream);
int htd_conv2d_bwd_data_x3q(const float *gy, const void *gyplanes, const void *wplanesT, const float *mask_src,
                            const float *accum, float *gx, void *gxplanes, float *amax_out, int B, int H, int W, int Ci, int Co, int kh, int kw,
                            int pad, void *workspace, void *stream);

int htd_conv2d_set_h2(int on);
int htd_conv2d_bwd_weight_h2_supported(int B, int H, int W, int Ci, int Co, int kh, int kw, int stride, int pad, int dil);
int htd_conv2d_bwd_weight_h2(const float *x, const float *gy, const float *amax_x, const float *amax_g, float *gw,
                             float *gbias, int B, int H, int W, int Ci, int Co, int kh, int kw, int stride, int pad,
                             int dil, int accumulate, void *workspace, void *stream);
int htd_conv2d_x3h_supported(int Ci, int Co, int kh, int kw, int stride, int pad, int dil);
int htd_conv2d_x3h_strided_supported(int Ci, int Co, int kh, int kw, int stride, int pad, int dil);
int htd_conv2d_bwd_data_x3h_strided_supported(int Ci, int Co, int kh, int kw, int stride, int pad, int dil);
int64_t htd_conv2d_bwd_data_x3h_strided_workspace_bytes(int B, int H, int W, int Ci, int Co, int kh, int kw, int stride, int pad);
int htd_conv2d_bwd_data_x3h_strided(const float *gy, const float *amax, const void *wplanesT, const float *mask_src, float *gx,
                                    float *amax_out, int B, int H, int W, int Ci, int Co, int kh, int kw, int stride, int pad,
                                    void *workspace, void *stream);
int htd_absmax(const float *x, int64_t n, float *amax, void *stream);
int htd_conv2d_x3h_planes(const float *w, void *planes, int Co, int kh, int kw, int Ci, int transposed, void *stream);
int htd_conv2d_x3h_planes_many(const void *desc, int n, int64_t total_blocks, int64_t total_rows, void *stream);
int htd_conv2d_fwd_x3h(const float *x, const float *amax, const void *wplanes, const float *bias, const float *residual,
                       int res_h, int res_w, float *y, void *yplanes, float *amax_out, int B, int H, int W, int Ci,
                       int Co, int kh, int kw, int stride, int pad, int relu, void *workspace, void *stream);
int htd_conv2d_bwd_data_x3h(const float *gy, const float *amax, const void *wplanesT, const float *mask_src,
                            const float *accum, float *gx, void *gxplanes, float *amax_out, int B, int H, int W,
                            int Ci, int Co, int kh, int kw, int pad, void *workspace, void *stream);

int64_t htd_deform_columns_bytes(int B, int H, int W, int C, int kh, int kw, int stride, int pad, int dil);
int htd_deform_im2col(const float *x, const float *offset, const float *mask, float *columns, int B,
                      int H, int W, int C, int kh, int kw, int stride, int pad, int dil,
                      int deform_groups, void *stream);
int htd_deform_col2im(const float *x, const float *offset, const float *mask, const float *gcolumns,
                      float *gx, float *goffset, float *gmask, int B, int H, int W, int C, int kh,
                      int kw, int stride, int pad, int dil, int deform_groups, void *stream);
int htd_deform_im2col_bf16(const void *x, const float *offset, const float *mask, void *columns, int B, int H, int W,
                           int C, int kh, int kw, int stride, int pad, int dil, int deform_groups, void *stream);
int htd_deform_col2im_bf16(const void *x, const float *offset, const float *mask, const void *gcolumns, float *gx,
                           float *goffset, float *gmask, int B, int H, int W, int C, int kh, int kw, int stride, int pad,
                           int dil, int deform_groups, void *stream);

int htd_global_avg_pool_fwd(const float *x, float *out, int64_t B, int P, int C, void *stream);
int htd_global_avg_pool_bwd(const float *g, float *gx, int64_t B, int P, int C, void *stream);
int htd_global_avg_pool_bwd_acc(const float *g, float *gx, int64_t B, int P, int C, void *stream);

int htd_group_norm_relu_fwd(const float *x, const float *gamma, const float *beta, float *y,
                            float *mean, float *rstd, int64_t n, int P, int C, int G, float eps,
                            int relu, void *stream);
int htd_group_norm_relu_bwd(const float *x, const float *y, const float *gamma, const float *mean,
                            const float *rstd, const float *gy, float *gx, float *ggamma,
                            float *gbeta, int64_t n, int P, int C, int G, int relu, void *stream);
int htd_group_norm_relu_bwd_ws(const float *x, const float *y, const float *gamma, const float *mean, const float *rstd,
                               const float *gy, float *gx, float *ggamma, float *gbeta, int64_t n, int P, int C, int G,
                               int relu, void *workspace, void *stream);
int htd_group_norm_relu_fwd_amax(const float *x, const float *gamma, const float *beta, float *y, float *mean, float *rstd,
                                 int64_t n, int P, int C, int G, float eps, int relu, float *amax_out, void *stream);
int htd_group_norm_bwd_amax_supported(int P, int C, int G);
int htd_group_norm_relu_bwd_amax(const float *x, const float *y, const float *gamma, const float *mean, const float *rstd,
                                 const float *gy, float *gx, float *ggamma, float *gbeta, int64_t n, int P, int C, int G,
                                 int relu, void *workspace, float *amax_out, void *stream);
int htd_fuse_global_bwd_global_ws(const float *grad, const float *rois, float *grad_global, int64_t n, int P, int C, int B,
                                  void *workspace, void *stream);

int htd_group_norm_map_slab(int P, int C);
int64_t htd_group_norm_map_workspace_bytes(int64_t n, int P, int C, int G);
int htd_group_norm_map_fwd(const float *x, const float *residual, const float *gamma, const float *beta, float *y, float *mean,
                           float *rstd, int64_t n, int P, int C, int G, float eps, int relu, void *workspace, float *amax_out,
                           void *stream);
int htd_group_norm_map_bwd(const float *x, const float *y, const float *gamma, const float *mean, const float *rstd,
                           const float *gy, float *gx, float *gres, float *ggamma, float *gbeta, int64_t n, int P, int C, int G,
                           int relu, void *workspace, float *amax_out, void *stream);

int htd_weight_standardize_fwd(const float *w, float *w_hat, float *mean, float *inv, int Co, int K, float eps, void *stream);
int htd_weight_standardize_bwd(const float *w, const float *mean, const float *inv, const float *g_hat, float *gw, int Co, int K,
                               float eps, void *stream);

int htd_bn_fold_fwd(const float *w, const float *gamma, const float *beta, const float *mean,
                    const float *var, float eps, float *w_folded, float *b_folded, int Co, int K,
                    void *stream);
int htd_bn_fold_bwd(const float *w, const float *gamma, const float *mean, const float *var, float eps,
                    const float *gw_folded, const float *gb_folded, float *gw, float *ggamma,
                    float *gbeta, int Co, int K, void *stream);
int htd_bn_fold_many_fwd(const void *desc, int n_layers, int total_tiles, float eps, void *stream);
int htd_bn_fold_many_bwd(const void *desc, int n_layers, int total_rows, float eps, void *stream);

int64_t htd_max_iou_assign_workspace_bytes(int B, int A, int K);
int htd_max_iou_assign(const float *boxes, int box_shared, const uint8_t *box_valid, const float *gts,
                       const uint8_t *gt_valid, int B, int A, int K, float pos_iou_thr, float neg_iou_thr,
                       float min_pos_iou, int match_low_quality, int64_t *assigned, float *max_overlaps,
                       void *workspace, void *stream);

int htd_roi_targets(const float *boxes, const float *gt_boxes, const int64_t *gt_labels, const uint8_t *is_pos,
                    const uint8_t *valid, int64_t n, int num_classes, const float *means4, const float *stds4,
                    int64_t *labels, float *label_weights, float *bbox_targets, float *bbox_weights, void *stream);
int htd_delta2bbox_clip(const float *rois, const float *deltas, const float *lim_wh, const uint8_t *keep, int64_t n,
                        int64_t rows_per_img, const float *means4, const float *stds4, float wh_ratio_clip,
                        float *out, void *stream);
int htd_map_roi_levels(const float *rois, int64_t *lvls, int64_t n, int num_levels, float finest_scale, void *stream);
int htd_rpn_heads_gather(const float *const *y, const int64_t *pix, int L, int B, int C, int na, float *cls, float *reg,
                         void *stream);
int htd_rpn_heads_scatter(const float *gcls, const float *greg, float *const *gy, const int64_t *pix, int L, int B, int C,
                          int na, void *stream);
int htd_static_samples_finish(const float *gts, const uint8_t *gvalid, const int64_t *glabels, const float *props,
                              const int64_t *assigned, const int64_t *order, const int64_t *counts, int B, int K, int P,
                              int A, int S, int add_gt, float *boxes, uint8_t *valid, uint8_t *is_pos,
                              float *pos_gt_boxes, int64_t *pos_gt_labels, uint8_t *pos_is_gt, void *stream);

int htd_roi_head_loss_partial_rows(void);
int htd_roi_head_loss(const float *cls_score, const int64_t *labels, const float *label_weights, const float *bbox_pred,
                      const float *bbox_targets, const float *bbox_weights, int64_t n, int NC, int num_fg, float beta,
                      float *partial, float *grad_cls, float *grad_box, void *stream);
int htd_roi_head_loss_decoded(const float *cls_score, const int64_t *labels, const float *label_weights, const float *rois,
                              const float *bbox_pred, const float *bbox_targets, const float *bbox_weights, int64_t n, int NC,
                              int num_fg, const double *means4, const double *stds4, double wh_ratio_clip, int kind, double eps,
                              double beta, float *partial, float *box_lo, float *grad_cls, float *grad_box, void *stream);
int htd_roi_head_loss_classes(const float *cls_score, const int64_t *labels, const float *label_weights, const float *bbox_pred,
                              const float *bbox_targets, const float *bbox_weights, int64_t n, int NC, int num_fg, int reg_classes,
                              int box_loss, float beta, float *partial, float *grad_cls, float *grad_box, void *stream);
int htd_rpn_loss_partial_rows(void);
int htd_rpn_loss(const float *cls, const float *reg, const float *anchors, const float *gts, const int64_t *assigned,
                 const uint8_t *pos, const uint8_t *neg, int B, int A, int K, const float *means4, const float *stds4,
                 float beta, float pos_weight, float *partial, float *grad_cls, float *grad_reg, void *stream);
int htd_rpn_loss_l1(const float *cls, const float *reg, const float *anchors, const float *gts, const int64_t *assigned,
                    const uint8_t *pos, const uint8_t *neg, int B, int A, int K, const float *means4, const float *stds4,
                    float pos_weight, float *partial, float *grad_cls, float *grad_reg, void *stream);

int htd_focal_loss_partial_rows(void);
int htd_sigmoid_focal_loss(const float *logits, const int64_t *labels, const float *weight, int64_t N, int C, float gamma,
                           float alpha, float *loss_out, float *partial, float *grad, void *stream);
int64_t htd_retina_avg_factor_workspace_bytes(int B);
int htd_retina_avg_factor(const int64_t *assigned, int B, int A, void *workspace, int *num_pos, float *avg_factor,
                          void *stream);
int htd_retina_loss(const float *const *cls, const int64_t *cls_stride, const float *const *reg, const int64_t *reg_stride,
                    const int64_t *pix, int L, int B, int na, int C, const float *anchors, const float *gts,
                    const int64_t *gt_labels, const int64_t *assigned, int A, int K, const float *means4,
                    const float *stds4, float gamma, float alpha, float pos_weight, int box_loss, float beta,
                    const float *avg_factor, float cls_weight, float box_weight, float *partial, float *const *grad_cls,
                    float *const *grad_reg, void *stream);
int htd_retina_grad_scale(float *const *grad_cls, const int64_t *cls_stride, float *const *grad_reg,
                          const int64_t *reg_stride, const int64_t *pix, int L, int B, int na, int C, const float *g_cls,
                          const float *g_box, void *stream);
int htd_retina_keys(const float *const *cls, const int64_t *cls_stride, const int64_t *pix, int L, int B, int na, int C,
                    float *keys, void *stream);

int64_t htd_ghm_workspace_bytes(int L);
int htd_ghmc_loss(const float *logits, const int64_t *labels, const float *weight, int64_t N, int C, const float *edges,
                  int bins, double momentum, float *acc_sum, float loss_weight, void *workspace, float *partial, float *grad,
                  void *stream);
int htd_ghm_head_loss(const float *const *cls, const int64_t *cls_stride, const float *const *reg, const int64_t *reg_stride,
                      const int64_t *pix, int L, int B, int na, int C, const float *anchors, const float *gts,
                      const int64_t *gt_labels, const int64_t *assigned, int A, int K, const float *means4,
                      const float *stds4, const float *edges_c, int bins_c, double momentum_c, float *acc_sum_c,
                      const float *edges_r, int bins_r, double momentum_r, float *acc_sum_r, float mu, float cls_weight,
                      float box_weight, void *workspace, float *partial, float *const *grad_cls, float *const *grad_reg,
                      void *stream);

int htd_ghm_head_loss_launches(const float *const *cls, const int64_t *cls_stride, const float *const *reg,
                               const int64_t *reg_stride, const int64_t *pix, int L, int B, int na, int C, const float *anchors,
                               const float *gts, const int64_t *gt_labels, const int64_t *assigned, int A, int K,
                               const float *means4, const float *stds4, const float *edges_c, int bins_c, double momentum_c,
                               float *acc_sum_c, const float *edges_r, int bins_r, double momentum_r, float *acc_sum_r, float mu,
                               float cls_weight, float box_weight, void *workspace, float *partial, float *const *grad_cls,
                               float *const *grad_reg, int launches, void *stream);

int64_t htd_fcos_targets_workspace_bytes(int B, int64_t P);
int htd_fcos_targets(const int64_t *hw, const int64_t *strides, const float *ranges, int L, const float *gts,
                     const uint8_t *gt_valid, int B, int K, int center_sampling, double radius, int norm_on_bbox,
                     int *assigned, float *bbox_targets, float *ctr_targets, void *workspace, int *num_pos, float *norm,
                     void *stream);
int htd_fcos_loss_partial_rows(void);
int htd_fcos_loss(const float *const *cls, const int64_t *cls_stride, const float *const *reg, const int64_t *reg_stride,
                  const float *const *ctr, const int64_t *ctr_stride, const int64_t *hw, const int64_t *strides, int L,
                  int B, int C, const int64_t *gt_labels, int K, const int *assigned, const float *bbox_targets,
                  const float *ctr_targets, const float *norm, int box_kind, double eps, float gamma, float alpha,
                  float cls_weight, float box_weight, float ctr_weight, float *partial, float *const *grad_cls,
                  float *const *grad_reg, float *const *grad_ctr, void *stream);
int htd_fcos_grad_scale(float *const *grad_cls, const int64_t *cls_stride, float *const *grad_reg,
                        const int64_t *reg_stride, float *const *grad_ctr, const int64_t *ctr_stride, const int64_t *hw,
                        const int64_t *strides, int L, int B, int C, const float *g_cls, const float *g_box,
                        const float *g_ctr, void *stream);
int htd_fcos_keys(const float *const *cls, const int64_t *cls_stride, const float *const *ctr, const int64_t *ctr_stride,
// ... 94 lines not shown
```

Measured before the change: 123.4 images/sec.

## Skip zero-gradient rows in RPN head conv backward via occupancy bitmap

Adds a row-occupancy kernel that marks which 16-pixel slices of the RPN head output gradient are nonzero. The 3x3 weight-gradient kernel then seeks only over occupied runs, and the H2 data-gradient kernel skips tiles whose whole neighbourhood is empty. This targets the sparse gradients produced by the RPN loss with few sampled anchors. In exchange it adds an extra pass over the gradient, plus per-slice bitmap scanning and more kernel template variants.

```diff
diff --git a/htd_amd/csrc/conv_wgrad.hip b/htd_amd/csrc/conv_wgrad.hip
--- a/htd_amd/csrc/conv_wgrad.hip
+++ b/htd_amd/csrc/conv_wgrad.hip
@@ -21,6 +21,7 @@
     int mt, nt, splits;
     int64_t slices_per_split;
     const float *amax_x, *amax_g;
+    const uint32_t *occ;
 };
 
 constexpr int BKW = 32;
@@ -974,7 +975,7 @@
 constexpr int XHD_RUN = XHD_KS + 2;
 constexpr int XHD_PLANE_A = XHD_KS * X3_ROW, XHD_PLANE_B = XHD_RUN * XH_ROWB;
 constexpr int XHD_BUF = 3 * XHD_PLANE_A + 3 * XHD_PLANE_B;
-template <int TM, bool H2 = false>
+template <int TM, bool H2 = false, bool OCC = false>
 __global__ __launch_bounds__(256, 2) void conv_wgrad_x3hd_kernel(WgradParams p)
 {
     float sg = 1.f, sx = 1.f, sg_inv = 1.f, sx_inv = 1.f;
@@ -1023,29 +1024,44 @@
     const bool a_cok = m0 + a_col < p.Co, b_cok = ci0 + b_col < p.Ci;
     const bool ragged = tid < 32;
     auto decode = [&](int64_t v, int &x, int &y, int64_t &real) {
-        const int64_t vv = v < 0 ? 0 : v;
-        x = (int)(vv % Wv);
-        const int64_t t = vv / Wv;
-        y = (int)(t % p.H);
-        real = vv - t;
+        if constexpr (OCC) {
+            const unsigned vv = v < 0 ? 0u : (unsigned)v;
+            x = (int)(vv % (unsigned)Wv);
+            const unsigned t = vv / (unsigned)Wv;
+            y = (int)(t % (unsigned)p.H);
+            real = (int64_t)(vv - t);
+        } else {
+            const int64_t vv = v < 0 ? 0 : v;
+            x = (int)(vv % Wv);
+            const int64_t t = vv / Wv;
+            y = (int)(t % p.H);
+            real = vv - t;
+        }
         if (v < 0) { x = Wv - 1; y = -1; real = 0; }
     };
     int ax[PA], bx[2], by[2];
     unsigned a_off[PA], b_off[2];
     const unsigned a_px = a_cok ? (unsigned)p.Co * 4u : 0u, b_px = b_cok ? (unsigned)p.Ci * 4u : 0u;
-#pragma unroll
-    for (int i = 0; i < PA; ++i) {
-        int y;
-        int64_t real;
-        decode(v_begin + a_row0 + RA * i, ax[i], y, real);
-        a_off[i] = a_cok ? (unsigned)(real * p.Co + m0 + a_col) * 4u : OOB;
-    }
-#pragma unroll
-    for (int i = 0; i < 2; ++i) {
-        int64_t real;
-        decode(v_begin - 1 + b_row0 + 16 * i, bx[i], by[i], real);
-        b_off[i] = b_cok && (i == 0 || ragged) ? (unsigned)((real + (int64_t)dy * p.W) * p.Ci + ci0 + b_col) * 4u : OOB;
-    }
+    auto seek = [&](int64_t v) {
+        int t = tid;
+        if constexpr (OCC) asm volatile("" : "+v"(t));
+        const int a_col_ = (t % VA) * 4, a_row0_ = t / VA, b_col_ = (t & 15) * 4, b_row0_ = t >> 4;
+        const bool a_cok_ = m0 + a_col_ < p.Co, b_cok_ = ci0 + b_col_ < p.Ci, ragged_ = t < 32;
+#pragma unroll
+        for (int i = 0; i < PA; ++i) {
+            int y;
+            int64_t real;
+            decode(v + a_row0_ + RA * i, ax[i], y, real);
+            a_off[i] = a_cok_ ? (unsigned)(real * p.Co + m0 + a_col_) * 4u : OOB;
+        }
+#pragma unroll
+        for (int i = 0; i < 2; ++i) {
+            int64_t real;
+            decode(v - 1 + b_row0_ + 16 * i, bx[i], by[i], real);
+            b_off[i] = b_cok_ && (i == 0 || ragged_) ? (unsigned)((real + (int64_t)dy * p.W) * p.Ci + ci0 + b_col_) * 4u : OOB;
+        }
+    };
+    if constexpr (!OCC) seek(v_begin);
     const unsigned b_px1 = ragged ? b_px : 0u;
     const int adv_rows = XHD_KS / Wv, adv_x = XHD_KS - adv_rows * Wv;
 
@@ -1077,6 +1093,39 @@
             by[i] -= by[i] >= p.H ? p.H : 0;
             b_off[i] += XHD_KS * px - (unsigned)rows * px;
         }
+    };
+    [[maybe_unused]] const int k_end = (int)(v_end / XH_KS);
+    [[maybe_unused]] int k = v_begin < v_end ? (int)(v_begin / XH_KS) : k_end, lrem = 0, issued = 0;
+    auto cue = [&]() {
+        if (lrem == 0) {
+            auto word = [&](int i) { return (unsigned)__builtin_amdgcn_readfirstlane((int)p.occ[i >> 5]) >> (i & 31); };
+            while (k < k_end) {
+                const unsigned w = word(k);
+                if (w != 0u) { k += __builtin_ctz(w); break; }
+                k = (k | 31) + 1;
+            }
+            if (k < k_end) {
+                int e = k;
+                for (;;) {
+                    const int room = 32 - (e & 31);
+                    const unsigned z = ~word(e);
+                    const int n = z != 0u ? min((int)__builtin_ctz(z), room) : room;
+                    e += n;
+                    if (n < room || e >= k_end) break;
+                }
+                e = min(e, k_end);
+                seek((int64_t)k * XH_KS);
+                lrem = (e - k) * (XH_KS / XHD_KS);
+                issued += lrem;
+                k = e;
+            } else {
+#pragma unroll
+                for (int i = 0; i < PA; ++i) a_off[i] = OOB;
+                b_off[0] = b_off[1] = OOB;
+                lrem = 1 << 30;
+            }
+        }
+        --lrem;
     };
     const bool do_bias = p.bias_out != nullptr && tile_nc == 0 && ky == 1;
     float4 bsum = make_float4(0.f, 0.f, 0.f, 0.f);
@@ -1154,6 +1203,7 @@
         if (__builtin_amdgcn_readfirstlane(wave) == 0) {
             if (ragged) put(wr + b_lds1, XHD_PLANE_B, qb[1], sx);
         }
+        if constexpr (OCC) cue();
         load_slice(qa, qb);
         __syncthreads();
     };
@@ -1167,14 +1217,28 @@
     };
 
     unsigned short *buf0 = lds, *buf1 = lds + XHD_BUF;
-    load_slice(ra[0], rb[0]);
-    load_slice(ra[1], rb[1]);
-    store_slice(buf0, ra[0], rb[0]);
-    load_slice(ra[0], rb[0]);
-    __syncthreads();
-    for (int s = 0; s < n_slices; s += 2) {
-        half(buf0, buf1, ra[1], rb[1]);
-        half(buf1, buf0, ra[0], rb[0]);
+    auto refill = [&]() {
+        if constexpr (OCC) cue();
+        load_slice(ra[0], rb[0]);
+        if constexpr (OCC) cue();
+        load_slice(ra[1], rb[1]);
+        store_slice(buf0, ra[0], rb[0]);
+        if constexpr (OCC) cue();
+        load_slice(ra[0], rb[0]);
+        __syncthreads();
+    };
+    if constexpr (!OCC) {
+        refill();
+        for (int s = 0; s < n_slices; s += 2) {
+            half(buf0, buf1, ra[1], rb[1]);
+            half(buf1, buf0, ra[0], rb[0]);
+        }
+    } else {
+        refill();
+        for (int s = 0; s < issued; s += 2) {
+            half(buf0, buf1, ra[1], rb[1]);
+            half(buf1, buf0, ra[0], rb[0]);
+        }
     }
 
     if (do_bias) {
@@ -1442,7 +1506,7 @@
 
 static int bwd_weight_impl(const float *x, const float *gy, float *gw, float *gbias, int B, int H, int W, int Ci, int Co, int kh,
                            int kw, int stride, int pad, int dil, void *workspace, void *stream, int accumulate,
-                           const float *amax_x = nullptr, const float *amax_g = nullptr)
+                           const float *amax_x = nullptr, const float *amax_g = nullptr, const uint32_t *occ = nullptr)
 {
     HTD_REQUIRE(B > 0 && H > 0 && W > 0 && Ci > 0 && Co > 0 && kh > 0 && kw > 0 && stride > 0 && dil > 0 && pad >= 0,
                 "conv2d_bwd_weight: bad sizes");
@@ -1451,6 +1515,7 @@
     WgradParams p{};
     p.x = x; p.gy = gy;
     p.amax_x = amax_x; p.amax_g = amax_g;
+    p.occ = occ;
     const bool h2 = amax_x != nullptr && amax_g != nullptr;
     p.B = B; p.H = H; p.W = W; p.Ci = Ci; p.Co = Co; p.kh = kh; p.kw = kw; p.stride = stride; p.pad = pad; p.dil = dil;
     p.Ho = (H + 2 * pad - (dil * (kh - 1) + 1)) / stride + 1;
@@ -1482,8 +1547,13 @@
             if (tile64 && Co <= 64) {
                 p.mt = (int)htd::ceil_div(Co, 64);
                 const dim3 g64((unsigned)(p.mt * p.nt * 3 * p.splits));
-                if (h2) hipLaunchKernelGGL((conv_wgrad_x3hd_kernel<1, true>), g64, dim3(256), 0, s, p);
+                if (occ && h2) hipLaunchKernelGGL((conv_wgrad_x3hd_kernel<1, true, true>), g64, dim3(256), 0, s, p);
+                else if (occ) hipLaunchKernelGGL((conv_wgrad_x3hd_kernel<1, false, true>), g64, dim3(256), 0, s, p);
+                else if (h2) hipLaunchKernelGGL((conv_wgrad_x3hd_kernel<1, true>), g64, dim3(256), 0, s, p);
                 else hipLaunchKernelGGL((conv_wgrad_x3hd_kernel<1, false>), g64, dim3(256), 0, s, p);
+            } else if (occ) {
+                if (h2) hipLaunchKernelGGL((conv_wgrad_x3hd_kernel<2, true, true>), grid, dim3(256), 0, s, p);
+                else hipLaunchKernelGGL((conv_wgrad_x3hd_kernel<2, false, true>), grid, dim3(256), 0, s, p);
             } else if (h2) {
                 hipLaunchKernelGGL((conv_wgrad_x3hd_kernel<2, true>), grid, dim3(256), 0, s, p);
             } else {
@@ -1491,6 +1561,7 @@
             }
         }
         else {
+            HTD_REQUIRE(!occ, "conv2d_bwd_weight_occ: this 3x3 layer is not taken by conv_wgrad_x3hd_kernel (htd_conv2d_bwd_weight_occ_supported)");
             HTD_REQUIRE(!h2, "conv2d_bwd_weight_h2: this 3x3 layer is not taken by the H2 kernels (htd_conv2d_bwd_weight_h2_supported)");
             if (W + 1 >= XH_KS) hipLaunchKernelGGL(conv_wgrad_x3h_kernel<true>, grid, dim3(256), 0, s, p);
             else hipLaunchKernelGGL(conv_wgrad_x3h_kernel<false>, grid, dim3(256), 0, s, p);
@@ -1504,6 +1575,7 @@
         }
         return htd::check_launch("conv2d_bwd_weight");
     }
+    HTD_REQUIRE(!occ, "conv2d_bwd_weight_occ: layer not taken by conv_wgrad_x3hd_kernel (htd_conv2d_bwd_weight_occ_supported)");
     const Cfg c = choose(Co, p.Ntot, p.K);
     p.mt = c.mt; p.nt = c.nt; p.splits = c.splits;
     p.slices_per_split = htd::ceil_div(htd::ceil_div(p.K, BKW), c.splits);
@@ -1603,6 +1675,88 @@
                            amax_g);
 }
 
+namespace {
+
+__global__ __launch_bounds__(1024) void row_occupancy_kernel(const float *__restrict__ g, int64_t rows, int64_t V, int Wv, int C,
+                                                             uint32_t *__restrict__ bits)
+{
+    __shared__ unsigned part[16];
+    const int lane = threadIdx.x & 63, wave = threadIdx.x >> 6;
+    unsigned mine = 0u;
+#pragma unroll
+    for (int j = 0; j < 2; ++j) {
+        const int64_t v0 = ((int64_t)blockIdx.x * 32 + wave * 2 + j) * XH_KS;
+        const int64_t v1 = v0 + XH_KS;
+        const int64_t r0 = v0 < V ? v0 - v0 / Wv : rows, r1 = v1 < V ? v1 - v1 / Wv : rows;
+        const float4 *src = reinterpret_cast<const float4 *>(g + r0 * C);
+        const int n4 = (int)((r1 - r0) * C / 4);
+        bool any = false;
+        for (int i = lane; i < n4; i += 64) {
+            const float4 q = src[i];
+            any |= !(q.x == 0.f) | !(q.y == 0.f) | !(q.z == 0.f) | !(q.w == 0.f);
+        }
+        mine |= __ballot(any) != 0ull ? 1u << (wave * 2 + j) : 0u;
+    }
+    if (lane == 0) part[wave] = mine;
+    __syncthreads();
+    if (threadIdx.x == 0) {
+        unsigned w = 0u;
+        for (int i = 0; i < 16; ++i) w |= part[i];
+        bits[blockIdx.x] = w;
+    }
+}
+
+}
+
+extern "C" int64_t htd_row_occupancy_words(int B, int H, int W)
+{
+    if (B <= 0 || H <= 0 || W <= 0) return 0;
+    return htd::ceil_div(htd::ceil_div((int64_t)B * H * (W + 1), XH_KS), 32);
+}
+
+extern "C" int htd_row_occupancy(const float *g, int B, int H, int W, int C, uint32_t *bits, void *stream)
+{
+    HTD_REQUIRE(B > 0 && H > 0 && W > 0 && C > 0 && (C & 3) == 0, "row_occupancy: bad sizes (C=%d must be a multiple of 4)", C);
+    HTD_REQUIRE(g && bits && ((uintptr_t)g & 15) == 0, "row_occupancy: null or unaligned pointer");
+    const int64_t words = htd_row_occupancy_words(B, H, W);
+    HTD_REQUIRE(words < (1ll << 31), "row_occupancy: map too large");
+    hipLaunchKernelGGL(row_occupancy_kernel, dim3((unsigned)words), dim3(1024), 0, (hipStream_t)stream, g, (int64_t)B * H * W,
+                       (int64_t)B * H * (W + 1), W + 1, C, bits);
+    return htd::check_launch("row_occupancy");
+}
+
+extern "C" int htd_conv2d_bwd_weight_occ_supported(int B, int H, int W, int Ci, int Co, int kh, int kw, int stride, int pad, int dil)
+{
+    static const int math_env = getenv("HTD_CONV_MATH") ? atoi(getenv("HTD_CONV_MATH")) : 1;
+    static const bool d_on = !(getenv("HTD_WGRAD_X3D") && atoi(getenv("HTD_WGRAD_X3D")) == 0);
+    if (B <= 0 || H <= 0 || W <= 0 || Ci <= 0 || Co <= 0 || !d_on || (g_wgrad_math < 0 ? math_env : g_wgrad_math) != 1) return 0;
+    if (!x3h_takes(Ci, Co, kh, kw, stride, pad, dil) || XHD_KS / (W + 1) + 1 > H) return 0;
+    return ((int64_t)B * H * W * Ci * 4 < (1ll << 31) && (int64_t)B * H * W * Co * 4 < (1ll << 31)) ? 1 : 0;
+}
+
+extern "C" int htd_conv2d_bwd_weight_occ(const float *x, const float *gy, float *gw, float *gbias, int B, int H, int W, int Ci, int Co,
+                                         int kh, int kw, int stride, int pad, int dil, int accumulate, void *workspace,
+                                         void *stream, const uint32_t *occ)
+{
+    HTD_REQUIRE(occ, "conv2d_bwd_weight_occ: null occupancy map");
+    HTD_REQUIRE(htd_conv2d_bwd_weight_occ_supported(B, H, W, Ci, Co, kh, kw, stride, pad, dil) == 1,
+                "conv2d_bwd_weight_occ: layer not taken by conv_wgrad_x3hd_kernel");
+    return bwd_weight_impl(x, gy, gw, gbias, B, H, W, Ci, Co, kh, kw, stride, pad, dil, workspace, stream, accumulate ? 1 : 0,
+                           nullptr, nullptr, occ);
+}
+
+extern "C" int htd_conv2d_bwd_weight_h2_occ(const float *x, const float *gy, const float *amax_x, const float *amax_g, float *gw,
+                                            float *gbias, int B, int H, int W, int Ci, int Co, int kh, int kw, int stride, int pad,
+                                            int dil, int accumulate, void *workspace, void *stream, const uint32_t *occ)
+{
+    HTD_REQUIRE(amax_x && amax_g && occ, "conv2d_bwd_weight_h2_occ: null maximum or occupancy map");
+    HTD_REQUIRE(htd_conv2d_bwd_weight_h2_supported(B, H, W, Ci, Co, kh, kw, stride, pad, dil) == 1 &&
+                    htd_conv2d_bwd_weight_occ_supported(B, H, W, Ci, Co, kh, kw, stride, pad, dil) == 1,
+                "conv2d_bwd_weight_h2_occ: layer not taken by the H2 form of conv_wgrad_x3hd_kernel");
+    return bwd_weight_impl(x, gy, gw, gbias, B, H, W, Ci, Co, kh, kw, stride, pad, dil, workspace, stream, accumulate ? 1 : 0, amax_x,
+                           amax_g, occ);
+}
+
 static int bias_grad_relu_mask_impl(const float *g, const float *y, float *gm, float *gbias, int64_t rows, int C, void *workspace,
                                     float *amax_out, void *stream)
 {
diff --git a/htd_amd/csrc/conv_x3.hip b/htd_amd/csrc/conv_x3.hip
--- a/htd_amd/csrc/conv_x3.hip
+++ b/htd_amd/csrc/conv_x3.hip
@@ -115,6 +115,7 @@
     int64_t xp_rows, yp_rows;
     const float *amax, *wscale;
     float *amax_out;
+    const uint32_t *occ;
 };
 
 __device__ __forceinline__ void block_absmax_out(float mx, float *out, float *red, unsigned seen)
@@ -398,6 +399,26 @@
     const int64_t m0 = (int64_t)tile_m * BM;
     const int n0 = tile_n * BN;
 
+    bool empty = false;
+    if constexpr (H2 && KW > 1) {
+        if (p.occ != nullptr) {
+            unsigned any = 0u;
+            for (int dy = -1; dy <= 1; ++dy) {
+                const int64_t r0 = max((int64_t)0, m0 + dy * p.Wx - 1), r1 = min(p.M, m0 + dy * p.Wx + BM + 1);
+                if (r0 >= r1) continue;
+                const unsigned lo = (unsigned)r0, hi = (unsigned)r1 - 1u;
+                const unsigned k0 = (lo + lo / (unsigned)p.Wx) >> 5, k1 = (hi + hi / (unsigned)p.Wx) >> 5;
+                for (unsigned w = k0 >> 5; w <= k1 >> 5; ++w) {
+                    unsigned bits = (unsigned)__builtin_amdgcn_readfirstlane((int)p.occ[w]);
+                    if (w == k0 >> 5) bits &= ~0u << (k0 & 31);
+                    if (w == k1 >> 5) bits &= ~0u >> (31 - (k1 & 31));
+                    any |= bits;
+                }
+            }
+            empty = any == 0u;
+        }
+    }
+
     const int tid = threadIdx.x, lane = tid & 63, wave = tid >> 6;
     const int wm = wave / WGN, wn = wave % WGN;
     const int frow = lane & 31, fhalf = lane >> 5;
@@ -672,6 +693,7 @@
     if (++ky1 == p.kh) { ky1 = 0; ++cs1; }
     int cs2 = cs1, ky2 = ky1;
     if (++ky2 == p.kh) { ky2 = 0; ++cs2; }
+    if (!empty) {
 #pragma unroll
     for (int d = 0; d < DIST; ++d) issue_b();
     {
@@ -787,6 +809,9 @@
     wait_vm<0>();
 #pragma unroll
     for (int i = 0; i < 2 * NPT; ++i) landed(ra[i]);
+    } else {
+        lds_barrier();
+    }
 
     x3_epilogue<WGM, WGN, TM, TN, MF16>(p, acc, lds, m0, n0, part, region_b, split);
 }
@@ -1857,9 +1882,9 @@
     return launch_x3p(p, kw, (hipStream_t)stream, workspace);
 }
 
-extern "C" int htd_conv2d_bwd_data_x3h(const float *gy, const float *amax, const void *wplanesT, const float *mask_src,
-                                       const float *accum, float *gx, void *gxplanes, float *amax_out, int B, int H, int W,
-                                       int Ci, int Co, int kh, int kw, int pad, void *workspace, void *stream)
+static int bwd_data_x3h_impl(const float *gy, const float *amax, const void *wplanesT, const float *mask_src, const float *accum,
+                             float *gx, void *gxplanes, float *amax_out, int B, int H, int W, int Ci, int Co, int kh, int kw, int pad,
+                             void *workspace, void *stream, const uint32_t *occ)
 {
     HTD_REQUIRE(!gxplanes || Ci % XK == 0, "conv2d_bwd_data_x3h: output planes need Ci %% 16 == 0 (Ci=%d)", Ci);
     HTD_REQUIRE(gy && amax && wplanesT && gx && B > 0 && H > 0 && W > 0, "conv2d_bwd_data_x3h: bad arguments");
@@ -1875,8 +1900,26 @@
     p.wscale = reinterpret_cast<const float *>(p.wp + planes_vec(kh * kw, Co, p.Cop));
     p.yp = (uint4 *)gxplanes; p.yp_rows = act_rows(p.M);
     p.amax_out = amax_out;
+    p.occ = occ;
     HTD_REQUIRE((int64_t)B * H * W * Co < (1ll << 31), "conv2d_bwd_data_x3h: operand too large");
     return launch_x3p(p, kw, (hipStream_t)stream, workspace);
+}
+
+extern "C" int htd_conv2d_bwd_data_x3h(const float *gy, const float *amax, const void *wplanesT, const float *mask_src,
+                                       const float *accum, float *gx, void *gxplanes, float *amax_out, int B, int H, int W,
+                                       int Ci, int Co, int kh, int kw, int pad, void *workspace, void *stream)
+{
+    return bwd_data_x3h_impl(gy, amax, wplanesT, mask_src, accum, gx, gxplanes, amax_out, B, H, W, Ci, Co, kh, kw, pad, workspace,
+                             stream, nullptr);
+}
+
+extern "C" int htd_conv2d_bwd_data_x3h_occ(const float *gy, const float *amax, const void *wplanesT, const float *mask_src,
+                                           const float *accum, float *gx, void *gxplanes, float *amax_out, int B, int H, int W,
+                                           int Ci, int Co, int kh, int kw, int pad, void *workspace, void *stream, const uint32_t *occ)
+{
+    HTD_REQUIRE(occ && kh == 3 && kw == 3, "conv2d_bwd_data_x3h_occ: 3x3 layers with an occupancy map only");
+    return bwd_data_x3h_impl(gy, amax, wplanesT, mask_src, accum, gx, gxplanes, amax_out, B, H, W, Ci, Co, kh, kw, pad, workspace,
+                             stream, occ);
 }
 
 namespace {
diff --git a/htd_amd/dense.py b/htd_amd/dense.py
--- a/htd_amd/dense.py
+++ b/htd_amd/dense.py
@@ -597,14 +597,15 @@
     return gm
 
 
-def _dgrad_raw(g, weight, x_shape, stride, padding, dilation, mask_src=None, accum=None, wT=None, g_planes=None, emit=None):
-    gx = _dgrad_raw_(g, weight, x_shape, stride, padding, dilation, mask_src, accum, wT, g_planes, bool(emit))
+def _dgrad_raw(g, weight, x_shape, stride, padding, dilation, mask_src=None, accum=None, wT=None, g_planes=None, emit=None,
+               occ=None):
+    gx = _dgrad_raw_(g, weight, x_shape, stride, padding, dilation, mask_src, accum, wT, g_planes, bool(emit), occ)
     if emit is not None:
         return gx if isinstance(gx, tuple) else (gx, None)
     return gx
 
 
-def _dgrad_raw_(g, weight, x_shape, stride, padding, dilation, mask_src, accum, wT, g_planes, emit):
+def _dgrad_raw_(g, weight, x_shape, stride, padding, dilation, mask_src, accum, wT, g_planes, emit, occ=None):
     B, Ci, H, W = x_shape
     Co, _, kh, kw = weight.shape
     Ho, Wo = g.shape[2], g.shape[3]
@@ -626,9 +627,14 @@
                 _h2_trace('dgrad', g, weight)
             if am is None and kh * kw * Ci >= H2_ABSMAX_MIN_WORK and g.numel() >= H2_ABSMAX_MIN_ELEMS:
                 am = absmax(g)
-            if am is not None:
+            if am is not None and occ is not None and kh == 3 and kw == 3:
+                capi.call('htd_conv2d_bwd_data_x3h_occ', _P(g), _P(am), _P(x3_planes(weight, True, True)), _P(mask_src), _P(accum),
+                          _P(gx), _P(gxp), _P(out_slot), B, H, W, Ci, Co, kh, kw, padding, _P(ws), _S(), _P(occ),
+                          key='htd_conv2d_bwd_data_x3h', work=work)
+            elif am is not None:
                 capi.call('htd_conv2d_bwd_data_x3h', _P(g), _P(am), _P(x3_planes(weight, True, True)), _P(mask_src), _P(accum), _P(gx),
                           _P(gxp), _P(out_slot), B, H, W, Ci, Co, kh, kw, padding, _P(ws), _S(), work=work)
+            if am is not None:
                 tag_amax(gx, out_slot)
                 _h2_guard(am, out_slot)
                 return (gx, gxp) if emit else gx
@@ -714,17 +720,41 @@
     return (ax if ax is not None else absmax(x)), (ag if ag is not None else absmax(g))
 
 
-def _wgrad_launch(x, g, weight, stride, padding, dilation, bias, amax=None):
+RPN_OCC = os.environ.get('HTD_RPN_OCC', '1') != '0'
+
+
+def row_occupancy(g):
+    B, C, H, W = g.shape
+    bits = torch.empty(capi.lib().htd_row_occupancy_words(B, H, W), device=g.device, dtype=torch.int32)
+    capi.call('htd_row_occupancy', _P(g), B, H, W, C, _P(bits), _S(), work=('byte', 4.0 * g.numel()))
+    return bits
+
+
+def _wgrad_occ(x, g, amax, gw, gb, shape, accumulate, ws, occ, work):
+    if amax is not None:
+        capi.call('htd_conv2d_bwd_weight_h2_occ', _P(x), _P(g), _P(amax[0]), _P(amax[1]), _P(gw), _P(gb), *shape, accumulate, _P(ws),
+                  _S(), _P(occ), key='htd_conv2d_bwd_weight_h2', work=work)
+    else:
+        capi.call('htd_conv2d_bwd_weight_occ', _P(x), _P(g), _P(gw), _P(gb), *shape, accumulate, _P(ws), _S(), _P(occ),
+                  key='htd_conv2d_bwd_weight', work=work)
+
+
+def _wgrad_launch(x, g, weight, stride, padding, dilation, bias, amax=None, occ=None):
     B, Ci, H, W = x.shape
     Co, _, kh, kw = weight.shape
     Ho, Wo = g.shape[2], g.shape[3]
+    if occ is not None and not (B * Ho * Wo > 0 and
+                                capi.lib().htd_conv2d_bwd_weight_occ_supported(B, H, W, Ci, Co, kh, kw, stride, padding, dilation)):
+        occ = None
     aw = grad_sink_again(weight) if SINK_ACCUMULATE else None
     ab = grad_sink_again(bias) if (aw is not None and torch.is_tensor(bias)) else None
     if aw is not None and (bias is None or ab is not None) and B * Ho * Wo > 0:
         nbytes = capi.lib().htd_conv2d_wgrad_workspace_bytes(B, H, W, Ci, Co, kh, kw, stride, padding, dilation)
         ws = torch.empty(nbytes // 4 + 1, device=g.device, dtype=g.dtype)
         work = ('flop', 2.0 * B * Ho * Wo * Co * kh * kw * Ci, 4.0 * (x.numel() + g.numel() + aw.numel()))
-        if amax is not None:
+        if occ is not None:
+            _wgrad_occ(x, g, amax, aw, ab, (B, H, W, Ci, Co, kh, kw, stride, padding, dilation), 1, ws, occ, work)
+        elif amax is not None:
             capi.call('htd_conv2d_bwd_weight_h2', _P(x), _P(g), _P(amax[0]), _P(amax[1]), _P(aw), _P(ab), B, H, W, Ci, Co, kh, kw,
                       stride, padding, dilation, 1, _P(ws), _S(), work=work)
         else:
@@ -744,7 +774,9 @@
     nbytes = capi.lib().htd_conv2d_wgrad_workspace_bytes(B, H, W, Ci, Co, kh, kw, stride, padding, dilation)
     ws = torch.empty(nbytes // 4 + 1, device=g.device, dtype=g.dtype)
     work = ('flop', 2.0 * B * Ho * Wo * Co * kh * kw * Ci, 4.0 * (x.numel() + g.numel() + gw.numel()))
-    if amax is not None:
+    if occ is not None:
+        _wgrad_occ(x, g, amax, gw, gb, (B, H, W, Ci, Co, kh, kw, stride, padding, dilation), 0, ws, occ, work)
+    elif amax is not None:
         capi.call('htd_conv2d_bwd_weight_h2', _P(x), _P(g), _P(amax[0]), _P(amax[1]), _P(gw), _P(gb), B, H, W, Ci, Co, kh, kw,
                   stride, padding, dilation, 0, _P(ws), _S(), work=work)
     else:
@@ -753,18 +785,20 @@
     return gw, gb, sink_w and sink_b
 
 
-def _wgrad_raw(x, g, weight, stride, padding, dilation, bias=None, overlap=True):
+def _wgrad_raw(x, g, weight, stride, padding, dilation, bias=None, overlap=True, occ=None):
     amax = _wgrad_amax(x, g, weight, stride, padding, dilation)
     if not overlap or not OVERLAP_WGRAD or (capi.profiling() and not _OVERLAP_IN_PROFILE):
         if OVERLAP_WGRAD and _SIDE and SINK_ACCUMULATE and grad_sink_again(weight) is not None:
             torch.cuda.current_stream().wait_stream(side_stream(g.device))
-        return _wgrad_launch(x, g, weight, stride, padding, dilation, bias, amax)[:2]
+        return _wgrad_launch(x, g, weight, stride, padding, dilation, bias, amax, occ)[:2]
     main, side = torch.cuda.current_stream(), side_stream(g.device)
     side.wait_stream(main)
     x.record_stream(side)
     g.record_stream(side)
+    if occ is not None:
+        occ.record_stream(side)
     with torch.cuda.stream(side):
-        gw, gb, sinks = _wgrad_launch(x, g, weight, stride, padding, dilation, bias, amax)
+        gw, gb, sinks = _wgrad_launch(x, g, weight, stride, padding, dilation, bias, amax, occ)
     if not sinks and weight.data_ptr() not in _SIDE_CONSUMED:
         if gw is not None:
             gw.record_stream(main)
@@ -774,9 +808,10 @@
     return gw, gb
 
 
-def _dgrad_joined(galias, g, weight, x_shape, stride, padding, dilation):
+def _dgrad_joined(galias, g, weight, x_shape, stride, padding, dilation, occ=None):
     fuse = galias is not None and stride == 1 and galias.dtype == g.dtype and tuple(galias.shape) == tuple(x_shape)
-    gx = _dgrad_raw(g, weight, x_shape, stride, padding, dilation, accum=galias.contiguous(memory_format=CL) if fuse else None)
+    gx = _dgrad_raw(g, weight, x_shape, stride, padding, dilation, accum=galias.contiguous(memory_format=CL) if fuse else None,
+                    occ=occ)
     return gx if (galias is None or fuse) else gx + galias
 
 
@@ -830,6 +865,15 @@
         return gx, gw, (gb if (has_bias and need_b) else None), gr, None, None, None, None, None, None
 
 
+def _occ_kernels(x, w1, padding):
+    B, Ci, H, W = x.shape
+    Co, _, kh, kw = w1.shape
+    if kh != 3 or kw != 3 or x.dtype != torch.float32 or B * H * W == 0:
+        return False
+    return bool(capi.lib().htd_conv2d_bwd_weight_occ_supported(B, H, W, Ci, Co, kh, kw, 1, padding, 1)) or \
+        _x3h_ok(Co, Ci, kh, kw, 1, padding, 1, x.dtype)
+
+
 class ConvReluHeadFunction(Function):
 
     @staticmethod
@@ -861,11 +905,14 @@
         elif need_b2 and b2 is not None:
             gb2 = _colsum_raw(gy, None, b2)[1]
         gh = _dgrad_raw(gy, w2, h.shape, 1, 0, 1, mask_src=h)
+        occ = None
+        if RPN_OCC and (need_w1 or need_x) and _occ_kernels(x, w1, padding) and gy.size(1) % 4 == 0 and gy.numel() > 0:
+            occ = row_occupancy(gy)
         if need_w1:
-            gw1, gb1 = _wgrad_raw(x, gh, w1, 1, padding, 1, b1 if (need_b1 and b1 is not None) else None)
+            gw1, gb1 = _wgrad_raw(x, gh, w1, 1, padding, 1, b1 if (need_b1 and b1 is not None) else None, occ=occ)
         elif need_b1 and b1 is not None:
             gb1 = _colsum_raw(gh, None, b1)[1]
-        gx = _dgrad_joined(galias, gh, w1, x.shape, 1, padding, 1) if need_x else galias
+        gx = _dgrad_joined(galias, gh, w1, x.shape, 1, padding, 1, occ=occ) if need_x else galias
         return gx, gw1, gb1, gw2, gb2, None, None
 
 
diff --git a/include/htd_amd.h b/include/htd_amd.h
--- a/include/htd_amd.h
+++ b/include/htd_amd.h
@@ -174,6 +174,19 @@
                             const float *accum, float *gx, void *gxplanes, float *amax_out, int B, int H, int W,
                             int Ci, int Co, int kh, int kw, int pad, void *workspace, void *stream);
 
+int64_t htd_row_occupancy_words(int B, int H, int W);
+int htd_row_occupancy(const float *g, int B, int H, int W, int C, uint32_t *bits, void *stream);
+int htd_conv2d_bwd_weight_occ_supported(int B, int H, int W, int Ci, int Co, int kh, int kw, int stride, int pad, int dil);
+int htd_conv2d_bwd_weight_occ(const float *x, const float *gy, float *gw, float *gbias, int B, int H, int W, int Ci, int Co,
+                              int kh, int kw, int stride, int pad, int dil, int accumulate, void *workspace, void *stream,
+                              const uint32_t *occ);
+int htd_conv2d_bwd_weight_h2_occ(const float *x, const float *gy, const float *amax_x, const float *amax_g, float *gw,
+                                 float *gbias, int B, int H, int W, int Ci, int Co, int kh, int kw, int stride, int pad,
+                                 int dil, int accumulate, void *workspace, void *stream, const uint32_t *occ);
+int htd_conv2d_bwd_data_x3h_occ(const float *gy, const float *amax, const void *wplanesT, const float *mask_src,
+                                const float *accum, float *gx, void *gxplanes, float *amax_out, int B, int H, int W,
+                                int Ci, int Co, int kh, int kw, int pad, void *workspace, void *stream, const uint32_t *occ);
+
 int64_t htd_deform_columns_bytes(int B, int H, int W, int C, int kh, int kw, int stride, int pad, int dil);
 int htd_deform_im2col(const float *x, const float *offset, const float *mask, float *columns, int B,
                       int H, int W, int C, int kh, int kw, int stride, int pad, int dil,
```

Measured after the change: 126.0 images/sec (median of 6 runs). +2.2%, better.
